# alvgaona/heart-sounds-segmentation

Measured on AMD Instinct MI355X. Metric: PCG windows/sec FSST (1 kHz, 2000-sample), higher is better.
Workload: dtype f32

## Files before the change

### heart_sounds_segmentation_amd/csrc/fsst_canon128.hpp

```cpp
#pragma once
#include "fsst_mfma128.hpp"

namespace hssfsst {

using h8 = _Float16 __attribute__((ext_vector_type(8)));
using u2 = unsigned __attribute__((ext_vector_type(2)));
using u4 = unsigned __attribute__((ext_vector_type(4)));
using lds_u2 = __attribute__((address_space(3))) u2;
using lds_u4 = __attribute__((address_space(3))) u4;

#define HSS_RARE_VMEM_DONE() __builtin_amdgcn_s_waitcnt(0x0f70)
constexpr int kCanonTileFrames = 64;
constexpr int kCanonRecs = 192;
constexpr int kCanonOpFloats = 16 * 64 * 4;
constexpr int kCanonAtabFloats = kCanonOpFloats + 4 * 128;
constexpr int kCanonLdsTabFloats = kCanonAtabFloats + 4 * 33 * 2;
constexpr int kCanonErrMul = 4;
constexpr int kCanonFlagWords = 8;
constexpr int kCanonTieWords = 32;

template <int KLO, int KC>
struct CanonCfg {
    static_assert(KC % 2 == 0 && KC >= 2 && KC <= 24 && KLO >= 0 && KLO + KC <= 32, "even band of <= 24 rows inside rows 0..31");
    static constexpr int NWIN = 128;
// ... 279 lines not shown
            if (mb) db = canon_decide(kB, dnb.y, dnb.x, tile.R2s, tile.eoff());
            const bool la = ma && (da.tie || da.row != kA), lb = mb && (db.tie || db.row != kB);
            if (ma && da.tie) { __hip_atomic_fetch_or(tb + (kA >> 1), 1u << (((kA & 1) << 4) + j), __ATOMIC_RELAXED, __HIP_MEMORY_SCOPE_WORKGROUP); flag[1] = 1; }
            if (mb && db.tie) { __hip_atomic_fetch_or(tb + (kB >> 1), 1u << (((kB & 1) << 4) + j), __ATOMIC_RELAXED, __HIP_MEMORY_SCOPE_WORKGROUP); flag[1] = 1; }
            if constexpr (STA) { if (la) *cellA = f2{0.0f, 0.0f}; }
            if constexpr (STB) { if (lb) *cellB = f2{0.0f, 0.0f}; }
            if (la && !da.tie) { if (canon_put<KLO, KC, s>(row0, kA, da.row, f2{a1.x, a2.x})) defer |= 1u << (2 * s); }
            if (lb && !db.tie) { if (canon_put<KLO, KC, s>(row0, kB, db.row, f2{b1.x, b2.x})) defer |= 1u << (2 * s + 1); }
        }
        if constexpr (s == 3) {
            if (__builtin_expect(visited && __builtin_amdgcn_ballot_w64(defer != 0u) != 0ull, 0)) {
                static_for<3>([&](auto TT) {
                    constexpr int t = decltype(TT)::value;
                    if (__builtin_amdgcn_ballot_w64((defer >> (2 * t)) & 3u) != 0ull) {
                        const f2 QA = zb[NT - 1 - t], QB = za[NT - 1 - t];
                        const f2 c1 = mix_re(za[t], QA), c2 = mix_im(za[t], QA), e1 = mix_re(zb[t], QB), e2 = mix_im(zb[t], QB);
                        const f2 dc = dn_second(c2, dn_first(c1, tiny)), de = dn_second(e2, dn_first(e1, tiny));
                        if ((defer >> (2 * t)) & 1u) {
                            const CanonMove d = canon_decide(rAi + RQ * t, dc.y, dc.x, tile.R2s, tile.eoff());
                            (void)canon_put<KLO, KC, 3>(row0, rAi + RQ * t, d.row, f2{c1.x, c2.x});
                        }
                        if ((defer >> (2 * t + 1)) & 1u) {
                            const CanonMove d = canon_decide(rBi + RQ * t, de.y, de.x, tile.R2s, tile.eoff());
                            (void)canon_put<KLO, KC, 3>(row0, rBi + RQ * t, d.row, f2{e1.x, e2.x});
                        }
                    }
                });
            }
        }
    });
    wave_sync();
    int f_ties = 0;
    if (visited) f_ties = flag[1];
    asm volatile("" : "+v"(f_ties));
    auto signal_sample = [&](int i) -> double {
        const int gi = tg + i - NWIN / 2;
        const float* xs;
        if constexpr (__is_pointer(XSig)) xs = xsig; else xs = xsig();
        return (gi >= 0 && gi < n) ? static_cast<double>(xs[gi]) : 0.0;
    };
    bool exact = false;
    if (__builtin_expect(__builtin_amdgcn_ballot_w64(mx > kExactTheta2 * tile.R2s) == 0ull && tile.R2s > 0.0f, 0)) {
        float e2 = 0.0f;
#pragma unroll
        for (int k = 0; k < 3; ++k) {
            const int i = lane_o + 64 * k;
            const u2 r = xrec[min(i, 142)];
            const float v = static_cast<float>(__builtin_bit_cast(_Float16, static_cast<unsigned short>(r.x & 0xffffu))) +
                            static_cast<float>(__builtin_bit_cast(_Float16, static_cast<unsigned short>(r.y & 0xffffu)));
            e2 = fmaf(i < 143 ? v : 0.0f, v, e2);
        }
        const float R2g = tile.r2s * __int_as_float(__builtin_amdgcn_readfirstlane(__float_as_int(piece_sums(e2, 0.0f, 0.0f, 0.0f))));
        exact = __builtin_amdgcn_ballot_w64(mx > kExactTheta2 * R2g) == 0ull && R2g > 0.0f;
    }
    if (__builtin_expect(exact, 0)) {
        for (int i = lane_o; i < 16 * C::LD; i += 64) own_base[i] = f2{0.0f, 0.0f};
        if (lane_o == 0) flag[1] = 0;
        wave_sync();
        resolve_bitmap<NWIN, true, true, true>(reinterpret_cast<unsigned*>(tq), signal_sample, own_base, C::LD, flag, KLO, KC, own_base, C::LD,
                                               C::COV0, C::COV0 + C::COVN, wtab, tw_lds, 1.0 / static_cast<double>(tile.inv), lane_o);
        wave_sync();
        HSS_RARE_VMEM_DONE();
    } else
    if (__builtin_expect(__builtin_amdgcn_readfirstlane(f_ties) != 0, 0)) {
        resolve_bitmap<NWIN, false, true, true>(reinterpret_cast<unsigned*>(tq), signal_sample, own_base, C::LD, flag, KLO, KC, own_base, C::LD, C::COV0, C::COV0 + C::COVN, wtab, tw_lds, 1.0 / static_cast<double>(tile.inv), lane_o);
        wave_sync();
        HSS_RARE_VMEM_DONE();
    }
}
template <int KLO, int KC>
__device__ __forceinline__ float canon_stats(const f2* own_base, int nvalid, float inv, int lane_o, f2& piv_out)
{
    using C = CanonCfg<KLO, KC>;
    const int g = (lane_o >> 4) & 3, j = lane_o & 15;
    const f2* src = own_base + j * C::LD + C::KOFF + g;
    const f2 pv0 = own_base[C::KOFF], pv1 = own_base[C::KOFF + KC / 2], pv2 = own_base[C::KOFF + KC - 1];
    const f2 piv = f2{pivot_med3(pv0.x, pv1.x, pv2.x), pivot_med3(pv0.y, pv1.y, pv2.y)};
    constexpr int NU = (KC + 3) / 4, UF = KC / 4;
    f2 v[NU];
#pragma unroll
    for (int u = 0; u < NU; ++u) v[u] = src[4 * u];
    f2 st_s = {0.0f, 0.0f}, st_q = {0.0f, 0.0f};
    if (__builtin_expect(nvalid == 16, 1)) {
#pragma unroll
        for (int u = 0; u < NU; ++u) {
            f2 d = v[u] - piv;
            if (u >= UF) { const bool ok = g + 4 * u < KC; d = f2{ok ? d.x : 0.0f, ok ? d.y : 0.0f}; }
            st_s += d; st_q = pk_fma(d, d, st_q);
        }
    } else {
        asm volatile("");
        const bool jv = j < nvalid;
#pragma unroll
        for (int u = 0; u < NU; ++u) {
            f2 d = v[u] - piv;
            const bool ok = jv && (g + 4 * u < KC);
            d = f2{ok ? d.x : 0.0f, ok ? d.y : 0.0f};
            st_s += d; st_q = pk_fma(d, d, st_q);
        }
    }
    float w = piece_sums(st_s.x, st_q.x, st_s.y, st_q.y);
    w *= inv;
    if ((lane_o >> 4) & 1) w *= inv;
    piv_out = piv * f2{inv, inv};
    return w;
}

template <int KLO, int KC, class Sink>
__device__ __forceinline__ void canon_image_to(const f2* own_base, const unsigned* ppk, float inv, int lane_o, Sink sink)
{
    unsigned obase = static_cast<unsigned>(reinterpret_cast<size_t>((lds_float*)reinterpret_cast<const float*>(own_base)));
    asm volatile("" : "+s"(obase));
    const f2 sc = {inv, inv};
    static_for<3>([&](auto I) {
        constexpr int i = decltype(I)::value;
        const unsigned pk = ppk[i * 64 + lane_o];
        const lds_float* q0 = (const lds_float*)static_cast<size_t>(obase + (pk & 0xffffu));
        const lds_float* q1 = (const lds_float*)static_cast<size_t>(obase + (pk >> 16));
        const f2 lo = f2{q0[0], q0[2]} * sc, hi = f2{q1[0], q1[2]} * sc;
        sink(i, f4{lo.x, lo.y, hi.x, hi.y});
    });
}
template <int KLO, int KC>
__device__ __forceinline__ void canon_image(const f2* own_base, const unsigned* ppk, float inv, int lane_o, f4 (&o)[3])
{
    canon_image_to<KLO, KC>(own_base, ppk, inv, lane_o, [&](int i, f4 v) { o[i] = v; });
}

template <int KLO, int KC>
__device__ __forceinline__ unsigned canon_store_offsets(int f)
{
    using C = CanonCfg<KLO, KC>;
    constexpr int Q = KC / 2;
    const int jj = min(f / Q, 15), c = 4 * (f - (f / Q) * Q);
    const int rowb = jj * C::LD + C::KOFF;
    const unsigned p0 = (c < KC) ? (rowb + c) * 8 : (rowb + c - KC) * 8 + 4;
    const unsigned p1 = (c + 2 < KC) ? (rowb + c + 2) * 8 : (rowb + c + 2 - KC) * 8 + 4;
    return p0 | (p1 << 16);
}

struct CanonParams {
    const float* x;
    float* out;
    float* partials;
    const float* atab;
    const double* wtab;
    const double* twtab;
    float r2scale_s;
    float inv_c;
    int n, mode, nsig, col0, ncols;
    long long xstride;
    Core128Regions reg;
    unsigned* status;
    const unsigned* gate;
    unsigned gate_val;
    const RaggedSignal* rsig;
    const int2* rchunk;
    int rnchunks;
};

constexpr int kCanonCtlFloats = 16 + 192;
constexpr int kCanonCtlFusedFloats = kCtlFusedFloats;

__device__ __forceinline__ void canon_fetch(const float* xsig, int n, int t0, int lane_o, float (&sreg)[3])
{
    const __amdgpu_buffer_rsrc_t rs = __builtin_amdgcn_make_buffer_rsrc(const_cast<float*>(xsig), 0, n * 4, 0x00020000);
#pragma unroll
    for (int k = 0; k < 3; ++k)
        sreg[k] = __builtin_bit_cast(float, __builtin_amdgcn_raw_buffer_load_b32(rs, (t0 + lane_o + 64 * k - 64) * 4, 0, 0));
}

template <int KLO, int KC, bool FUSED, bool RAGGED = false>
__global__ __launch_bounds__(64 * 16, 4) void fsst_canon_kernel(CanonParams p)
{
    static_assert(!(RAGGED && FUSED), "ragged lists: the two-launch kernel");
    using C = CanonCfg<KLO, KC>;
    constexpr int WPB = 16, K = KC, GPCF = kCanonTileFrames / 16;
    constexpr int ATAB = kCanonLdsTabFloats;
    constexpr int CTL = FUSED ? kCanonCtlFusedFloats : kCanonCtlFloats;
    extern __shared__ __attribute__((aligned(16))) float smem[];
    if (p.gate != nullptr && *p.gate != p.gate_val) return;
    int n = p.n;
    const int lane = threadIdx.x & 63;
    const int wv = __builtin_amdgcn_readfirstlane(threadIdx.x >> 6);
    float* atab = smem;
    int* next_q = reinterpret_cast<int*>(smem + ATAB);
    unsigned* done_a = reinterpret_cast<unsigned*>(smem + ATAB) + 1;
    unsigned* dead = done_a + 2;
    unsigned* ready = dead + 1;
    float4* fin_stats = reinterpret_cast<float4*>(smem + ATAB + 272);
    unsigned* cls_lds = reinterpret_cast<unsigned*>(smem + ATAB + 16);
    unsigned* ppk_lds = reinterpret_cast<unsigned*>(smem + ATAB + (FUSED ? 80 : 16));
    float* part_lds = smem + ATAB + 288;
    float* wbase = smem + ATAB + CTL + wv * C::wave_floats();
    u2* xrec = reinterpret_cast<u2*>(wbase);
    f2* own_base = reinterpret_cast<f2*>(wbase + 2 * kCanonRecs);
    int* flag = reinterpret_cast<int*>(own_base + 16 * C::LD);
    int* tq = flag + kCanonFlagWords;

    for (int i = threadIdx.x; i < ATAB; i += 64 * WPB) atab[i] = p.atab[i];
    int ncols = p.ncols, cend = p.col0 + p.ncols;
    if (lane < kCanonFlagWords) flag[lane] = 0;
    if (lane < kCanonTieWords) tq[lane] = 0;
    if (threadIdx.x < (FUSED ? 8 : 1)) next_q[threadIdx.x] = 0;
    if (wv == 0) {
        unsigned cls = 0u;
#pragma unroll
        for (int i = 0; i < 3; ++i) {
            const unsigned c = (4u * static_cast<unsigned>(lane + 64 * i)) % static_cast<unsigned>(2 * K);
            cls |= (c >= static_cast<unsigned>(K) ? 1u : 0u) << (2 * i);
            cls |= (c + 2 >= static_cast<unsigned>(K) ? 1u : 0u) << (2 * i + 1);
            ppk_lds[i * 64 + lane] = canon_store_offsets<KLO, KC>(lane + 64 * i);
        }
        if constexpr (FUSED) cls_lds[lane] = cls;
    }
    __syncthreads();

    const int nc0 = p.nsig * p.reg.npc[0];
    const int nc1 = nc0 + p.nsig * p.reg.npc[1];
    const int nchunks = nc1 + p.nsig * p.reg.npc[2];
    int ngroups = (ncols + 15) >> 4;
    const int nk = (FUSED && p.nsig > static_cast<int>(blockIdx.x)) ? (p.nsig - static_cast<int>(blockIdx.x) + static_cast<int>(gridDim.x) - 1) / static_cast<int>(gridDim.x) : 0;
    const int NC = (ngroups + GPCF - 1) / GPCF;
    const int lead = min(8, NC);
    const int nwork = FUSED ? 2 * NC * nk : RAGGED ? p.rnchunks : nchunks;
    auto draw = [&]() -> int {
        int q = 0;
        if (lane == 0) q = __hip_atomic_fetch_add(next_q, 1, __ATOMIC_RELAXED, __HIP_MEMORY_SCOPE_WORKGROUP);
        q = __builtin_amdgcn_readfirstlane(q);
        if constexpr (FUSED) return q < nwork ? q : nwork;
        const long long c = static_cast<long long>(blockIdx.x) + static_cast<long long>(q) * gridDim.x;
        return c < nwork ? static_cast<int>(c) : nwork;
    };
    int chunk = draw();
    f2 tiny = {1.0e-37f, 0.0f};
    asm volatile("" : "+s"(tiny));
    while (chunk < nwork) {
    long long b;
    int grp0, ngrp;
    long long ksig = 0;
    bool zpass = false;
    long long rxo = 0, roo = 0, rpo = 0;
    if constexpr (FUSED) {
        int c;
        if (chunk < NC) {
            ksig = 0; c = chunk;
        } else {
            const int u = chunk - NC;
            const int kk = 1 + u / (2 * NC), v = u - (kk - 1) * (2 * NC);
            if (kk < nk) {
                const int npairs = NC - lead;
                if (v < lead) { ksig = kk; c = v; }
                else if (v - lead < 2 * npairs) {
                    const int w = v - lead;
                    if (w & 1) { ksig = kk; c = lead + (w >> 1); }
                    else { ksig = kk - 1; c = w >> 1; zpass = true; }
                } else { ksig = kk - 1; c = npairs + (v - lead - 2 * npairs); zpass = true; }
            } else { ksig = nk - 1; c = v; zpass = true; }
        }
        b = static_cast<long long>(blockIdx.x) + ksig * gridDim.x;
        grp0 = c * GPCF;
        ngrp = min(GPCF, ngroups - grp0);
    } else if constexpr (RAGGED) {
        const int2 cd = p.rchunk[chunk];
        const RaggedSignal* rs = p.rsig + cd.x;
        rxo = rs->xoff; roo = rs->ooff; rpo = rs->poff;
        n = rs->n; ncols = n; cend = n; ngroups = (n + 15) >> 4;
        b = 0;
        grp0 = cd.y & ((1 << kRaggedGroupBits) - 1);
        ngrp = (cd.y >> kRaggedGroupBits) + 1;
    } else {
        const int rg = (chunk < nc0) ? 0 : (chunk < nc1) ? 1 : 2;
        const int local = chunk - ((rg == 0) ? 0 : (rg == 1) ? nc0 : nc1);
        const int npc = p.reg.npc[rg], gpc = p.reg.gpc[rg];
        b = local / npc;
        const int cidx = local - static_cast<int>(b) * npc;
        grp0 = p.reg.g0[rg] + cidx * gpc;
        ngrp = min(gpc, ngroups - grp0);
    }
    int lane_o = lane;
    asm volatile("" : "+v"(lane_o));
    if (FUSED && zpass) {
        const int sl = static_cast<int>(ksig) & 3;
        const unsigned epoch = static_cast<unsigned>(ksig) + 1u;
        constexpr int CC = 2 * K;
        float4* d4 = reinterpret_cast<float4*>(p.out + (b * static_cast<long long>(ncols) + grp0 * 16) * CC) + lane_o;
        constexpr int per = 8 * K;
        for (unsigned spins = 0;; ++spins) {
            unsigned have = 0;
            if (lane == 0) have = __hip_atomic_load(ready + sl, __ATOMIC_ACQUIRE, __HIP_MEMORY_SCOPE_WORKGROUP);
            if (__builtin_amdgcn_readfirstlane(have) == epoch) break;
            if (spins >= kSpinLimit || __hip_atomic_load(dead, __ATOMIC_RELAXED, __HIP_MEMORY_SCOPE_WORKGROUP)) {
                if (lane == 0) {
                    __hip_atomic_store((gu32*)(p.status), 2u, __ATOMIC_RELAXED, __HIP_MEMORY_SCOPE_SYSTEM);
                    __hip_atomic_store(dead, 1u, __ATOMIC_RELAXED, __HIP_MEMORY_SCOPE_WORKGROUP);
                }
                break;
            }
            __builtin_amdgcn_s_sleep(4);
        }
        __builtin_amdgcn_fence(__ATOMIC_ACQUIRE, "workgroup");
        const float4 st = fin_stats[sl];
        const unsigned cls = cls_lds[lane_o];
        const float4* base0 = reinterpret_cast<const float4*>(p.out + (b * static_cast<long long>(ncols) + grp0 * 16) * CC);
        auto glim = [&](int q) { return (q < ngrp) ? min(16, ncols - (grp0 + q) * 16) * (K >> 1) : 0; };
        {
            f4 o[GPCF][3];
#pragma unroll
            for (int q = 0; q < GPCF; ++q) {
                const int lim = glim(q);
#pragma unroll
                for (int i = 0; i < 3; ++i) {
                    const float4* src = (lane_o + 64 * i < lim) ? (d4 + q * per + 64 * i) : base0;
                    o[q][i] = __builtin_nontemporal_load(reinterpret_cast<const f4*>(src));
                }
            }
            f2 mu[3][2], rs[3][2];
#pragma unroll
            for (int i = 0; i < 3; ++i) {
                const bool im0 = (cls >> (2 * i)) & 1u, im1 = (cls >> (2 * i + 1)) & 1u;
                const float m0 = im0 ? st.z : st.x, r0 = im0 ? st.w : st.y;
                const float m1 = im1 ? st.z : st.x, r1 = im1 ? st.w : st.y;
                mu[i][0] = f2{m0, m0}; rs[i][0] = f2{r0, r0};
                mu[i][1] = f2{m1, m1}; rs[i][1] = f2{r1, r1};
            }
#pragma unroll
            for (int q = 0; q < GPCF; ++q) {
                const int lim = glim(q);
#pragma unroll
                for (int i = 0; i < 3; ++i) {
                    if (lane_o + 64 * i < lim) {
                        const f2 lo = (f2{o[q][i].x, o[q][i].y} - mu[i][0]) * rs[i][0];
                        const f2 hi = (f2{o[q][i].z, o[q][i].w} - mu[i][1]) * rs[i][1];
                        __builtin_nontemporal_store(f4{lo.x, lo.y, hi.x, hi.y}, reinterpret_cast<f4*>(d4 + q * per + 64 * i));
// ... 79 lines not shown
```

### heart_sounds_segmentation_amd/csrc/fsst_half.hpp

```cpp
#pragma once

#include "fsst_kernels.hpp"
#include "fsst_mfma128.hpp"

namespace hssfsst {

template <class OT>
__device__ __forceinline__ void half_store4(OT* dst, float a, float b, float c, float d)
{
    using o2 = OT __attribute__((ext_vector_type(2)));
    using w2 = unsigned __attribute__((ext_vector_type(2)));
    const w2 w = {__builtin_bit_cast(unsigned, __builtin_convertvector(f2{a, b}, o2)), __builtin_bit_cast(unsigned, __builtin_convertvector(f2{c, d}, o2))};
    *reinterpret_cast<w2*>(dst) = w;
}

template <class OT>
__global__ __launch_bounds__(256) void fsst_normalize_to_kernel(const float* in, OT* out, const float4* stats, const float* partials,
                                                                int nblk, int fpp, int n, int K, int nsignals, int slices,
                                                                const unsigned* gate = nullptr, unsigned gate_val = 0u)
{
    static_assert(sizeof(OT) == 2, "2-byte output elements");
    if (gate != nullptr && *gate != gate_val) return;
    __shared__ float4 st_sh;
    const int tid = threadIdx.x;
    const int C = 2 * K;
    const int total = n * C;
    const bool vec = (total & 3) == 0 && (reinterpret_cast<uintptr_t>(out) & 7) == 0;
    for (int unit = blockIdx.x; unit < nsignals * slices; unit += gridDim.x) {
        const int sig = unit / slices, sl = unit - sig * slices;
        float4 st;
        if (partials != nullptr) {
            if (tid < 64) {
                const float4 r = signal_stats(partials + static_cast<long long>(sig) * nblk * kPartFloats, nblk, fpp, n, K, tid);
                if (tid == 0) st_sh = r;
            }
            __syncthreads();
            st = st_sh;
            __syncthreads();
        } else {
            st = stats[sig];
        }
        const float m_re = st.x, i_re = st.y, m_im = st.z, i_im = st.w;
        const float* src = in + static_cast<long long>(sig) * total;
        OT* dst = out + static_cast<long long>(sig) * total;
        if (vec) {
            const float4* s4 = reinterpret_cast<const float4*>(src);
            const int tot4 = total >> 2;
            const int i0 = static_cast<int>(static_cast<long long>(tot4) * sl / slices);
            const int i1 = static_cast<int>(static_cast<long long>(tot4) * (sl + 1) / slices);
            int c = static_cast<int>((static_cast<unsigned>(i0 + tid) * 4u) % static_cast<unsigned>(C));
            const int dc = static_cast<int>(1024u % static_cast<unsigned>(C));
            const bool rowwrap = (C & 3) != 0;
#pragma unroll 4
            for (int i = i0 + tid; i < i1; i += 256) {
                const float4 v = s4[i];
                int c1 = c + 1, c2 = c + 2, c3 = c + 3;
                if (rowwrap) {
                    if (c1 >= C) c1 -= C;
                    if (c2 >= C) c2 -= C;
                    if (c3 >= C) c3 -= C;
                }
                half_store4<OT>(dst + 4ll * i,
                                (c < K) ? (v.x - m_re) * i_re : (v.x - m_im) * i_im,
                                (c1 < K) ? (v.y - m_re) * i_re : (v.y - m_im) * i_im,
                                (c2 < K) ? (v.z - m_re) * i_re : (v.z - m_im) * i_im,
                                (c3 < K) ? (v.w - m_re) * i_re : (v.w - m_im) * i_im);
                c += dc;
                if (c >= C) c -= C;
            }
        } else {
            const int i0 = static_cast<int>(static_cast<long long>(total) * sl / slices);
            const int i1 = static_cast<int>(static_cast<long long>(total) * (sl + 1) / slices);
            for (int i = i0 + tid; i < i1; i += 256) {
                const int c = i % C;
                const float v = src[i];
                dst[i] = static_cast<OT>((c < K) ? (v - m_re) * i_re : (v - m_im) * i_im);
            }
        }
    }
}

template <class OT>
__global__ __launch_bounds__(256) void fsst_ragged_normalize_to_kernel(const float* in, OT* out, const RaggedSignal* sig, const int* unit0,
                                                                       const float4* stats, int nsig, int K)
{
    static_assert(sizeof(OT) == 2, "2-byte output elements");
    const int tid = threadIdx.x;
    const int C = 2 * K;
    const bool vec = (reinterpret_cast<uintptr_t>(out) & 7) == 0;
    const int nunits = unit0[nsig];
    for (int u = blockIdx.x; u < nunits; u += gridDim.x) {
        int lo = 0, hi = nsig;
        while (hi - lo > 1) {
            const int mid = (lo + hi) >> 1;
            if (unit0[mid] <= u) lo = mid; else hi = mid;
        }
        const int s = lo;
        const RaggedSignal rs = sig[s];
        const float4 st = stats[s];
        const float m_re = st.x, i_re = st.y, m_im = st.z, i_im = st.w;
        const int a = static_cast<int>(rs.ooff & 3);
        const float* src = in + (rs.ooff - a);
        OT* dst = out + (rs.ooff - a);
        const int total = rs.n * C;
        const int q = static_cast<int>((static_cast<long long>(a) + total + 3) >> 2);
        const int slices = unit0[s + 1] - unit0[s], sl = u - unit0[s];
        const int i0 = static_cast<int>(static_cast<long long>(q) * sl / slices);
        const int i1 = static_cast<int>(static_cast<long long>(q) * (sl + 1) / slices);
        long long e = 4ll * (i0 + tid) - a;
        int c = static_cast<int>(e % C);
        if (c < 0) c += C;
        const int dc = 1024 % C;
        auto zs = [&](float v, int col) -> float { return (col < K) ? (v - m_re) * i_re : (v - m_im) * i_im; };
        auto wrap = [&](int col) -> int { if (col >= C) col -= C; if (col >= C) col -= C; return col; };
        for (int i = i0 + tid; i < i1; i += 256) {
            if (vec && e >= 0 && e + 4 <= total) {
                const float4 v = reinterpret_cast<const float4*>(src)[i];
                half_store4<OT>(dst + 4ll * i, zs(v.x, c), zs(v.y, wrap(c + 1)), zs(v.z, wrap(c + 2)), zs(v.w, wrap(c + 3)));
            } else {
                for (int k = 0; k < 4; ++k)
                    if (e + k >= 0 && e + k < total) dst[4ll * i + k] = static_cast<OT>(zs(src[4ll * i + k], wrap(c + k)));
            }
            e += 1024;
            c = wrap(c + dc);
        }
    }
}

}
```

### heart_sounds_segmentation_amd/csrc/fsst_kernels.hpp

```cpp
#pragma once
#include <hip/hip_runtime.h>

#include <utility>

namespace hssfsst {

constexpr int kModeRaw = 0, kModeAbs = 1, kModeStack = 2, kModeStackUnnorm = 3;

struct CoreParams {
    const float* x;
    float* out;
    float* partials;
    const float* ctab;
    int n;
    int klo;
    int K;
    int mode;
    int nblk;
    int col0;
    int ncols;
    int oneplane;
    const double* wtab;
    const double* twtab;
    float r2scale;
// ... 246 lines not shown
        const auto r = __builtin_amdgcn_permlane16_swap(v, v, false, false);
        const auto ri = __builtin_amdgcn_permlane16_swap(id, id, false, false);
        return ri[0] == (id ^ 16u) ? r[0] : r[1];
    } else {
        const auto r = __builtin_amdgcn_permlane32_swap(v, v, false, false);
        const auto ri = __builtin_amdgcn_permlane32_swap(id, id, false, false);
        return ri[0] == (id ^ 32u) ? r[0] : r[1];
    }
}
template <int OFF>
__device__ __forceinline__ double xor_lane_f64(double v, int lane)
{
    const long long b = __double_as_longlong(v);
    const unsigned lo = xor_lane_u32<OFF>(static_cast<unsigned>(b & 0xffffffffll), lane);
    const unsigned hi = xor_lane_u32<OFF>(static_cast<unsigned>(static_cast<unsigned long long>(b) >> 32), lane);
    return __longlong_as_double(static_cast<long long>((static_cast<unsigned long long>(hi) << 32) | lo));
}
__device__ __forceinline__ float4 stats_finish_pre(double acc, double it, double it1, int lane)
{
    { const double o = xor_lane_f64<4>(acc, lane);  acc = (lane & 4) ? (o + acc) : (acc + o); }
    { const double o = xor_lane_f64<8>(acc, lane);  acc = (lane & 8) ? (o + acc) : (acc + o); }
    { const double o = xor_lane_f64<16>(acc, lane); acc = (lane & 16) ? (o + acc) : (acc + o); }
    { const double o = xor_lane_f64<32>(acc, lane); acc = (lane & 32) ? (o + acc) : (acc + o); }
    auto from_lane = [&](int l) {
        const long long b = __double_as_longlong(acc);
        const int lo = __builtin_amdgcn_readlane(static_cast<int>(b & 0xffffffffll), l);
        const int hi = __builtin_amdgcn_readlane(static_cast<int>(b >> 32), l);
        return __longlong_as_double((static_cast<long long>(hi) << 32) | static_cast<unsigned>(lo));
    };
    const double sx_re = from_lane(0), sxx_re = from_lane(1), sx_im = from_lane(2), sxx_im = from_lane(3);
    const double mr = sx_re * it, mi = sx_im * it;
    const double vr = fma(-sx_re, mr, sxx_re) * it1, vi = fma(-sx_im, mi, sxx_im) * it1;
    return make_float4(static_cast<float>(mr), 1.0f / sqrtf(static_cast<float>(vr)),
                       static_cast<float>(mi), 1.0f / sqrtf(static_cast<float>(vi)));
}
__device__ __forceinline__ float4 stats_finish_lead(double acc, double it, double it1, int lane)
{
    auto halves = [](double v, unsigned& lo, unsigned& hi) {
        const unsigned long long b = static_cast<unsigned long long>(__double_as_longlong(v));
        lo = static_cast<unsigned>(b); hi = static_cast<unsigned>(b >> 32);
    };
    auto join = [](unsigned lo, unsigned hi) { return __longlong_as_double(static_cast<long long>((static_cast<unsigned long long>(hi) << 32) | lo)); };
    unsigned lo, hi;
    {
        const int from = __builtin_amdgcn_readfirstlane(__builtin_amdgcn_update_dpp(0, lane, 0x124, 0xf, 0xf, false));
        halves(acc, lo, hi);
        unsigned plo, phi;
        if (from == 4) {
            plo = static_cast<unsigned>(__builtin_amdgcn_update_dpp(0, static_cast<int>(lo), 0x124, 0xf, 0xf, false));
            phi = static_cast<unsigned>(__builtin_amdgcn_update_dpp(0, static_cast<int>(hi), 0x124, 0xf, 0xf, false));
        } else {
            plo = static_cast<unsigned>(__builtin_amdgcn_update_dpp(0, static_cast<int>(lo), 0x12c, 0xf, 0xf, false));
            phi = static_cast<unsigned>(__builtin_amdgcn_update_dpp(0, static_cast<int>(hi), 0x12c, 0xf, 0xf, false));
        }
        acc = acc + join(plo, phi);
    }
    {
        halves(acc, lo, hi);
        const unsigned plo = static_cast<unsigned>(__builtin_amdgcn_update_dpp(0, static_cast<int>(lo), 0x128, 0xf, 0xf, false));
        const unsigned phi = static_cast<unsigned>(__builtin_amdgcn_update_dpp(0, static_cast<int>(hi), 0x128, 0xf, 0xf, false));
        acc = acc + join(plo, phi);
    }
    {
        halves(acc, lo, hi);
        const auto rl = __builtin_amdgcn_permlane16_swap(lo, lo, false, false);
        const auto rh = __builtin_amdgcn_permlane16_swap(hi, hi, false, false);
        acc = acc + join(rl[1], rh[1]);
    }
    {
        halves(acc, lo, hi);
        const auto rl = __builtin_amdgcn_permlane32_swap(lo, lo, false, false);
        const auto rh = __builtin_amdgcn_permlane32_swap(hi, hi, false, false);
        acc = acc + join(rl[1], rh[1]);
    }
    auto from_lane = [&](int l) {
        const long long b = __double_as_longlong(acc);
        const int l0 = __builtin_amdgcn_readlane(static_cast<int>(b & 0xffffffffll), l);
        const int h0 = __builtin_amdgcn_readlane(static_cast<int>(b >> 32), l);
        return __longlong_as_double((static_cast<long long>(h0) << 32) | static_cast<unsigned>(l0));
    };
    const double sx_re = from_lane(0), sxx_re = from_lane(1), sx_im = from_lane(2), sxx_im = from_lane(3);
    const double mr = sx_re * it, mi = sx_im * it;
    const double vr = fma(-sx_re, mr, sxx_re) * it1, vi = fma(-sx_im, mi, sxx_im) * it1;
    return make_float4(static_cast<float>(mr), 1.0f / sqrtf(static_cast<float>(vr)),
                       static_cast<float>(mi), 1.0f / sqrtf(static_cast<float>(vi)));
}
__device__ __forceinline__ float4 stats_finish(double acc, double total, int lane)
{
    return stats_finish_pre(acc, 1.0 / total, 1.0 / (total - 1.0), lane);
}
template <class BlockSum>
__device__ __forceinline__ float4 stats_from_blocks(int nblocks, double total, BlockSum block_sum, int lane)
{
    const int q = lane & 3;
    double acc = 0.0;
    for (int blk = lane >> 2; blk < nblocks; blk += 16) acc += block_sum(blk, q);
    return stats_finish(acc, total, lane);
}

template <int STRIDE = kPartFloats>
__device__ __forceinline__ float4 signal_stats(const float* part, int nparts, int fpp, int ncols, int K, int lane)
{
    const int nblocks = (nparts + kStatBlock - 1) / kStatBlock;
    return stats_from_blocks(nblocks, static_cast<double>(K) * static_cast<double>(ncols), [&](int blk, int q) {
        double s = 0.0;
        const int g1 = min(nparts, (blk + 1) * kStatBlock);
        for (int g = blk * kStatBlock; g < g1; ++g) {
            const float* pp = part + static_cast<long long>(g) * STRIDE;
            const double cnt = static_cast<double>(min(fpp, ncols - fpp * g)) * static_cast<double>(K);
            const int h = q >> 1;
            s += piece_moment(q, static_cast<double>(pp[2 * h]), static_cast<double>(pp[2 * h + 1]),
                              static_cast<double>(pp[4 + h]), cnt);
        }
        return s;
    }, lane);
}

__device__ __forceinline__ float piece_sums(float s_re, float q_re, float s_im, float q_im)
{
    const auto r1 = __builtin_amdgcn_permlane32_swap(__float_as_uint(s_re), __float_as_uint(s_im), false, false);
    const float u = __uint_as_float(r1[0]) + __uint_as_float(r1[1]);
    const auto r2 = __builtin_amdgcn_permlane32_swap(__float_as_uint(q_re), __float_as_uint(q_im), false, false);
    const float v = __uint_as_float(r2[0]) + __uint_as_float(r2[1]);
    const auto r3 = __builtin_amdgcn_permlane16_swap(__float_as_uint(u), __float_as_uint(v), false, false);
    float w = __uint_as_float(r3[0]) + __uint_as_float(r3[1]);
    w += __uint_as_float(__builtin_amdgcn_update_dpp(0, __float_as_uint(w), 0x128, 0xf, 0xf, false));
    w += __uint_as_float(__builtin_amdgcn_update_dpp(0, __float_as_uint(w), 0x124, 0xf, 0xf, false));
    w += __uint_as_float(__builtin_amdgcn_update_dpp(0, __float_as_uint(w), 0x122, 0xf, 0xf, false));
    w += __uint_as_float(__builtin_amdgcn_update_dpp(0, __float_as_uint(w), 0x121, 0xf, 0xf, false));
    return w;
}

__device__ __forceinline__ float pivot_med3(float a, float b, float c) { return __builtin_amdgcn_fmed3f(a, b, c); }

__device__ __forceinline__ void store_partial(float* part, float w, float p_re, float p_im)
{
    const int lane = threadIdx.x & 63;
    part[lane >> 4] = w;
    part[4 + (lane & 1)] = (lane & 1) ? p_im : p_re;
}

constexpr float kDcTheta = 0.99f;
struct TileEnergy { float E, S1, C; bool dcdom; };
__device__ __forceinline__ TileEnergy tile_energy(float e2, float s1, float cnt)
{
    const float w = piece_sums(e2, s1, cnt, 0.0f);
    const float E = __int_as_float(__builtin_amdgcn_readlane(__float_as_int(w), 0));
    const float S1 = __int_as_float(__builtin_amdgcn_readlane(__float_as_int(w), 16));
    const float C = __int_as_float(__builtin_amdgcn_readlane(__float_as_int(w), 32));
    return TileEnergy{E, S1, C, E > 0.0f && S1 * S1 >= kDcTheta * C * E};
}

__global__ __launch_bounds__(64) void fsst_stats_kernel(const float* partials, float4* stats, int nparts, int fpp,
                                                        int n, int K, const unsigned* gate = nullptr, unsigned gate_val = 0u)
{
    if (gate != nullptr && *gate != gate_val) return;
    const long long b = blockIdx.x;
    const float4 st = signal_stats(partials + b * nparts * kPartFloats, nparts, fpp, n, K, threadIdx.x & 63);
    if (threadIdx.x == 0) stats[b] = st;
}

template <int R, int TILE>
__global__ __launch_bounds__(TILE, 2) void fsst_core_kernel(CoreParams p)
{
    constexpr int NWIN = 32 * R;
    constexpr int XS = ((TILE + NWIN - 1 + 3) / 4) * 4;
    constexpr int LD = TILE + 1;
    extern __shared__ __attribute__((aligned(16))) float smem[];
    float* xs = smem;
    float* own = smem + XS;

    const int tid = threadIdx.x;
    const int blk = blockIdx.x % p.nblk;
    const long long b = blockIdx.x / p.nblk;
    const int t0 = p.col0 + blk * TILE;
    const int n = p.n;
    const int ncols = p.ncols, tr0 = t0 - p.col0;
    const int K = p.K;
    const float* xsig = p.x + b * p.xstride;

    float e2 = 0.0f, s1 = 0.0f, cnt = 0.0f;
    for (int i = tid; i < TILE + NWIN - 1; i += TILE) {
        const int g = t0 + i - NWIN / 2;
        const bool in = (g >= 0 && g < n);
        const float v = in ? xsig[g] : 0.0f;
        xs[i] = v;
        e2 = fmaf(v, v, e2); s1 += v; cnt += in ? 1.0f : 0.0f;
    }
    static_assert(TILE == 64, "tile_energy reduces one wave");
    const TileEnergy te = tile_energy(e2, s1, cnt);
    const float R2 = p.r2scale * te.E;
    const bool oneplane = p.oneplane != 0;
    float* disp = oneplane ? own : own + 2 * K * LD;
    for (int c = 0; c < 2 * K; ++c) disp[c * LD + tid] = 0.0f;
    __syncthreads();

    const Scatter<LD> sc{own + tid, disp + tid, p.klo, K, oneplane, xs + tid, p.wtab, p.twtab, R2};
    const float* myx = xs + tid;
    ctab_ptr tab = (ctab_ptr)p.ctab;
    packed_class<R, false, LD>(tab, myx, sc);
    if constexpr (R >= 2) packed_class<R, true, LD>(tab + (R / 2) * 32 * 4 * R, myx, sc);
    if constexpr (R >= 4 && R <= 8) {
        static_for<R / 2 - 1>([&](auto RR) {
            constexpr int r = decltype(RR)::value + 1;
            pair_class<R, LD>(tab + r * 32 * 4 * R, r, myx, sc);
        });
    } else if constexpr (R > 8) {
        for (int r = 1; r < R / 2; ++r) pair_class<R, LD>(tab + r * 32 * 4 * R, r, myx, sc);
    }
    __syncthreads();
    if (!oneplane) {
        for (int c = 0; c < 2 * K; ++c) own[c * LD + tid] += disp[c * LD + tid];
    }
    __syncthreads();
    float* acc = own;
    {
        float mxc = 0.0f;
        for (int k = 0; k < K; ++k) { const float re = acc[k * LD + tid], im = acc[(K + k) * LD + tid]; mxc = fmaxf(mxc, fmaf(re, re, im * im)); }
        if ((__builtin_amdgcn_ballot_w64(mxc > 1.0e-4f * R2) == 0ull || te.dcdom) && R2 > 0.0f) {
            for (int c = 0; c < 2 * K; ++c) acc[c * LD + tid] = 0.0f;
            const int klo = p.klo;
            for (int kp = 0; kp <= NWIN / 2; ++kp) {
                double vr = 0.0, vi = 0.0, dr = 0.0, di = 0.0;
#pragma unroll 4
                for (int nn = 0; nn < NWIN; ++nn) {
                    const double x = static_cast<double>(xs[tid + nn]);
                    const double2 wd = reinterpret_cast<const double2*>(p.wtab)[nn];
                    const double2 cs = reinterpret_cast<const double2*>(p.twtab)[(kp * nn) & (NWIN - 1)];
                    const double xw = x * wd.x, xd = x * wd.y;
                    vr = fma(xw, cs.x, vr); vi = fma(-xw, cs.y, vi);
                    dr = fma(xd, cs.x, dr); di = fma(-xd, cs.y, di);
                }
                double shift = (dr * vi - di * vr) / (vr * vr + vi * vi);
                if (!(fabs(shift) <= 1.0e6)) shift = 0.0;
                const double a = static_cast<double>(kp) + shift;
                const double r = (a >= 0.0) ? floor(a + 0.5) : -floor(0.5 - a);
                const int row = static_cast<int>(static_cast<long long>(r)) & (NWIN - 1);
                const double sg = (kp & 1) ? -1.0 : 1.0;
                const float re = static_cast<float>(vr * sg), im = static_cast<float>(vi * sg);
                const int idx = row - klo;
                if (static_cast<unsigned>(idx) < static_cast<unsigned>(K)) { acc[idx * LD + tid] += re; acc[(K + idx) * LD + tid] += im; }
                if (kp != 0 && kp != NWIN / 2) {
                    const int idm = ((NWIN - row) & (NWIN - 1)) - klo;
                    if (static_cast<unsigned>(idm) < static_cast<unsigned>(K)) { acc[idm * LD + tid] += re; acc[(K + idm) * LD + tid] -= im; }
                }
            }
        }
    }

    const int valid = min(TILE, p.col0 + ncols - t0);
    if (p.mode == kModeRaw) {
        if (tid < valid) {
            float2* dst = reinterpret_cast<float2*>(p.out) + (b * K) * static_cast<long long>(ncols) + tr0 + tid;
            for (int k = 0; k < K; ++k)
                dst[static_cast<long long>(k) * ncols] = make_float2(acc[k * LD + tid], acc[(K + k) * LD + tid]);
        }
        return;
    }
    const int C = (p.mode == kModeAbs) ? K : 2 * K;
    float* dst = p.out + (b * static_cast<long long>(ncols) + tr0) * C;
    const int total = valid * C;
    int tt = tid / C, c = tid - tt * C;
    const int dtt = TILE / C, dc = TILE - dtt * C;
    static_assert(TILE == 64, "one wave per tile: the statistics partial is a single-wave reduction");
    const float p_re = pivot_med3(acc[0], acc[(K >> 1) * LD], acc[(K - 1) * LD]);
    const float p_im = pivot_med3(acc[K * LD], acc[(K + (K >> 1)) * LD], acc[(2 * K - 1) * LD]);
    float s_re = 0.0f, q_re = 0.0f, s_im = 0.0f, q_im = 0.0f;
    for (int e = tid; e < total; e += TILE) {
        float val;
        if (p.mode == kModeAbs) {
            const float re = acc[c * LD + tt], im = acc[(K + c) * LD + tt];
            val = sqrtf(fmaf(re, re, im * im));
        } else {
            val = acc[c * LD + tt];
            if (c < K) { const float d = val - p_re; s_re += d; q_re = fmaf(d, d, q_re); }
            else       { const float d = val - p_im; s_im += d; q_im = fmaf(d, d, q_im); }
        }
        dst[e] = val;
        c += dc; tt += dtt;
        if (c >= C) { c -= C; ++tt; }
    }
    if (p.mode != kModeStack) return;
    const float w = piece_sums(s_re, q_re, s_im, q_im);
    store_partial(p.partials + (b * p.nblk + blk) * kPartFloats, w, p_re, p_im);
}

__global__ __launch_bounds__(256) void fsst_normalize_kernel(float* out, const float4* stats, const float* partials,
                                                             int nblk, int fpp, int n, int K, int nsignals, int slices,
                                                             const unsigned* gate = nullptr, unsigned gate_val = 0u)
{
    if (gate != nullptr && *gate != gate_val) return;
    __shared__ float4 st_sh;
    const int tid = threadIdx.x;
    const int C = 2 * K;
    const int total = n * C;
    for (int unit = blockIdx.x; unit < nsignals * slices; unit += gridDim.x) {
        const int sig = unit / slices, sl = unit - sig * slices;
        float4 st;
        if (partials != nullptr) {
            if (tid < 64) {
                const float4 r = signal_stats(partials + static_cast<long long>(sig) * nblk * kPartFloats, nblk, fpp, n, K, tid);
                if (tid == 0) st_sh = r;
            }
            __syncthreads();
            st = st_sh;
            __syncthreads();
        } else {
            st = stats[sig];
        }
        const float m_re = st.x, i_re = st.y, m_im = st.z, i_im = st.w;
        float* base = out + static_cast<long long>(sig) * total;
        if ((total & 3) == 0) {
            float4* b4 = reinterpret_cast<float4*>(base);
            const int tot4 = total >> 2;
            const int i0 = static_cast<int>(static_cast<long long>(tot4) * sl / slices);
            const int i1 = static_cast<int>(static_cast<long long>(tot4) * (sl + 1) / slices);
            int c = static_cast<int>((static_cast<unsigned>(i0 + tid) * 4u) % static_cast<unsigned>(C));
            const int dc = static_cast<int>(1024u % static_cast<unsigned>(C));
            const bool rowwrap = (C & 3) != 0;
#pragma unroll 4
            for (int i = i0 + tid; i < i1; i += 256) {
                float4 v = b4[i];
                int c1 = c + 1, c2 = c + 2, c3 = c + 3;
                if (rowwrap) {
                    if (c1 >= C) c1 -= C;
                    if (c2 >= C) c2 -= C;
                    if (c3 >= C) c3 -= C;
                }
                v.x = (c < K) ? (v.x - m_re) * i_re : (v.x - m_im) * i_im;
                v.y = (c1 < K) ? (v.y - m_re) * i_re : (v.y - m_im) * i_im;
                v.z = (c2 < K) ? (v.z - m_re) * i_re : (v.z - m_im) * i_im;
                v.w = (c3 < K) ? (v.w - m_re) * i_re : (v.w - m_im) * i_im;
                b4[i] = v;
                c += dc;
                if (c >= C) c -= C;
            }
        } else {
            const int i0 = static_cast<int>(static_cast<long long>(total) * sl / slices);
            const int i1 = static_cast<int>(static_cast<long long>(total) * (sl + 1) / slices);
            for (int i = i0 + tid; i < i1; i += 256) {
                const int c = i % C;
                const float v = base[i];
                base[i] = (c < K) ? (v - m_re) * i_re : (v - m_im) * i_im;
            }
        }
    }
}

constexpr int kMomThreads = 1024;
constexpr int kMomPieceFrames = 16;
struct PlainLoad4 { __device__ float4 operator()(const float4* q) const { return *q; } };
struct AgentLoad4 {
    __device__ float4 operator()(const float4* q) const
    {
        const unsigned long long* u = reinterpret_cast<const unsigned long long*>(q);
        const unsigned long long a = __hip_atomic_load(u, __ATOMIC_RELAXED, __HIP_MEMORY_SCOPE_AGENT);
        const unsigned long long b = __hip_atomic_load(u + 1, __ATOMIC_RELAXED, __HIP_MEMORY_SCOPE_AGENT);
        return make_float4(__uint_as_float(static_cast<unsigned>(a)), __uint_as_float(static_cast<unsigned>(a >> 32)),
                           __uint_as_float(static_cast<unsigned>(b)), __uint_as_float(static_cast<unsigned>(b >> 32)));
    }
};
__device__ __forceinline__ void mom_acc(double (&a)[4], float f, bool imag)
{
    const double v = static_cast<double>(f);
    if (imag) { a[2] += v; a[3] = fma(v, v, a[3]); } else { a[0] += v; a[1] = fma(v, v, a[1]); }
}
__device__ __forceinline__ void mom_acc4(double (&a)[4], float4 v, int f, int C, int K)
{
    int c = static_cast<int>((4u * static_cast<unsigned>(f)) % static_cast<unsigned>(C));
    int c1 = c + 1, c2 = c + 2, c3 = c + 3;
    if (c1 >= C) c1 -= C;
    if (c2 >= C) c2 -= C;
    if (c3 >= C) c3 -= C;
    mom_acc(a, v.x, c >= K); mom_acc(a, v.y, c1 >= K); mom_acc(a, v.z, c2 >= K); mom_acc(a, v.w, c3 >= K);
}
__device__ inline void piece_moments(const float* pb, int L, int C, int K, int lane, double (&t)[4])
{
    double a[4] = {0.0, 0.0, 0.0, 0.0};
    const bool wide = (reinterpret_cast<uintptr_t>(pb) & 15) == 0;
    for (int f = lane; 4 * f < L; f += 64) {
        if (wide && 4 * f + 3 < L) mom_acc4(a, *reinterpret_cast<const float4*>(pb + 4 * f), f, C, K);
        else
            for (int u = 0; u < 4; ++u) {
                const int e = 4 * f + u;
                if (e < L) mom_acc(a, pb[e], (e % C) >= K);
            }
    }
#pragma unroll
    for (int e = 0; e < 4; ++e) t[e] = wave_sum(a[e]);
}
template <class Piece>
__device__ inline void moments_from_pieces(int npieces, int lane, Piece piece, double (&out)[4])
{
    double a[4] = {0.0, 0.0, 0.0, 0.0};
    for (int q = lane; q < npieces; q += 64)
#pragma unroll
        for (int e = 0; e < 4; ++e) a[e] += piece(q, e);
#pragma unroll
    for (int e = 0; e < 4; ++e) out[e] = wave_sum(a[e]);
}
__device__ inline void chunk_moments(const float* base, int n, int C, int K, int tid, double (*sh)[4], double out[4])
{
    const int lane = tid & 63, w = tid >> 6;
    const int npieces = (n + kMomPieceFrames - 1) / kMomPieceFrames;
    double a[4] = {0.0, 0.0, 0.0, 0.0};
    for (int q = w; q < npieces; q += kMomThreads / 64) {
        double t[4];
        piece_moments(base + static_cast<long long>(q) * kMomPieceFrames * C, min(kMomPieceFrames, n - q * kMomPieceFrames) * C, C, K, lane, t);
        if (lane == (q & 63))
#pragma unroll
            for (int e = 0; e < 4; ++e) a[e] += t[e];
    }
    if ((lane & 15) == w)
#pragma unroll
        for (int e = 0; e < 4; ++e) sh[lane][e] = a[e];
    __syncthreads();
#pragma unroll
    for (int e = 0; e < 4; ++e) out[e] = wave_sum(sh[lane][e]);
}

__device__ inline float2 merge_state(double* st, double s, double q, double nb)
{
    const double mean_b = s / nb;
    const double m2_b = q - s * mean_b;
    const double na = st[0], mean_a = st[1], m2_a = st[2];
    const double nn = na + nb;
    const double delta = mean_b - mean_a;
    const double mean_n = mean_a + delta * (nb / nn);
    const double m2_n = m2_a + m2_b + delta * delta * (na * nb / nn);
    st[0] = nn; st[1] = mean_n; st[2] = m2_n;
    return make_float2(static_cast<float>(mean_n), 1.0f / static_cast<float>(sqrt(m2_n / (nn - 1.0))));
}

__global__ __launch_bounds__(kMomThreads) void fsst_moments_merge_kernel(const float* feats, double* state, int n, int K)
{
    __shared__ double sh[64][4];
    const long long b = blockIdx.x;
    const int tid = threadIdx.x;
    const int total = n * 2 * K;
    double m[4];
    chunk_moments(feats + b * static_cast<long long>(total), n, 2 * K, K, tid, sh, m);
    if (tid < 2) merge_state(state + b * 6 + tid * 3, m[2 * tid], m[2 * tid + 1], static_cast<double>(K) * static_cast<double>(n));
}

// ... 112 lines not shown
```

### heart_sounds_segmentation_amd/csrc/fsst_team16.hpp

```cpp
#pragma once
#include "fsst_mfma128.hpp"
#include "fsst_canon128.hpp"

namespace hssfsst {

using gu64 = __attribute__((address_space(1))) unsigned long long;

constexpr int kT16PartFloats = 6;
constexpr int kT16BlockWords = 8;
constexpr int kT16MaxBlocks = kFusedMaxGroups / kStatBlock;
constexpr int kT16SlotWords = kT16MaxBlocks * kT16BlockWords;
constexpr int kT16MaxCpc = 8;
constexpr int kT16MaxSlots = 64;
constexpr int kT16StatFloats = 12;
constexpr int t16_ctl_base(int slots) { return 16 + 64 + 192 + 2 * slots + kT16StatFloats * slots; }
constexpr int t16_ctl_floats(int pslots, int slots) { return t16_ctl_base(slots) + pslots * (kT16MaxCpc * kT16PartFloats + 2); }
template <int KLO, int KC>
constexpr int t16_room() { return 160 * 1024 / 4 - kCanonLdsTabFloats - 16 * CanonCfg<KLO, KC>::wave_floats(); }
template <int KLO, int KC>
constexpr int t16_slots() { return t16_room<KLO, KC>() >= t16_ctl_floats(16, kT16MaxSlots) ? kT16MaxSlots : kT16MaxSlots / 2; }
template <int KLO, int KC>
constexpr int t16_pslots()
{
    constexpr int room = t16_room<KLO, KC>(), sl = t16_slots<KLO, KC>();
    return room >= t16_ctl_floats(32, sl) ? 32 : room >= t16_ctl_floats(16, sl) ? 16 : 0;
}

struct Team16Params {
    const float* x;
    float* out;
    const float* atab;
    const double* wtab;
    const double* twtab;
    unsigned long long* mail;
    unsigned* status;
    float r2scale_s;
    float inv_c;
    int n, nsig, col0, ncols;
    long long xstride;
    int team;
    int cpc_shift;
    int slots;
    unsigned seq;
    unsigned spin_ticks;
    unsigned* arrive;
    unsigned arrive_base;
    unsigned* abort_word;
    unsigned* fallbacks;
    unsigned launch;
    unsigned* done;
    unsigned done_base;
    unsigned* host_done;
    double inv_total, inv_total1;
};


constexpr int kT16HeldBase = 104;
#define HSS_T16_PAIRS(X) X(0, 104, 105) X(1, 106, 107) X(2, 108, 109) X(3, 110, 111) X(4, 112, 113) X(5, 114, 115) \
                         X(6, 116, 117) X(7, 118, 119) X(8, 120, 121) X(9, 122, 123) X(10, 124, 125) X(11, 126, 127)
template <int P>
__device__ __forceinline__ void held_put(f2 a, f2 b)
{
#define HSS_T16_PUT(N, LO, HI) if constexpr (P == N) asm volatile("v_pk_mul_f32 v[" #LO ":" #HI "], %0, %1" :: "v"(a), "v"(b) : "v" #LO, "v" #HI);
    HSS_T16_PAIRS(HSS_T16_PUT)
#undef HSS_T16_PUT
}
template <int P>
__device__ __forceinline__ f2 held_zscore(f2 m)
{
    f2 d, e;
#define HSS_T16_ZS(N, LO, HI) if constexpr (P == N) asm volatile("v_pk_add_f32 %0, v[" #LO ":" #HI "], %1 op_sel:[0,0] op_sel_hi:[1,0] neg_lo:[0,1] neg_hi:[0,1]" : "=v"(d) : "v"(m));
    HSS_T16_PAIRS(HSS_T16_ZS)
#undef HSS_T16_ZS
    asm("v_pk_mul_f32 %0, %1, %2 op_sel:[0,1] op_sel_hi:[1,1]" : "=v"(e) : "v"(d), "v"(m));
    return e;
}

template <class OT>
__device__ __forceinline__ void team16_store4(char* dst, f2 lo, f2 hi)
{
    static_assert(sizeof(OT) == 2, "2-byte output elements");
    using o2 = OT __attribute__((ext_vector_type(2)));
    using w2 = unsigned __attribute__((ext_vector_type(2)));
    const w2 w = {__builtin_bit_cast(unsigned, __builtin_convertvector(lo, o2)), __builtin_bit_cast(unsigned, __builtin_convertvector(hi, o2))};
    __builtin_nontemporal_store(w, reinterpret_cast<w2*>(dst));
}

template <int KLO, int KC, int WPB, int DEPTH, class OT = float>
__global__ __launch_bounds__(64 * WPB, WPB / 4) __attribute__((amdgpu_num_vgpr(52))) void fsst_team16_kernel(Team16Params p)
{
    constexpr int OB = static_cast<int>(sizeof(OT));
    using C = CanonCfg<KLO, KC>;
    static_assert(WPB % 4 == 0 && DEPTH >= 1 && DEPTH <= 2, "whole waves per SIMD; two held groups (v104 .. v127)");
    static_assert(DEPTH == 2, "the kernel is compiled for 104 allocatable registers + 24 fixed ones");
    constexpr int K = KC, ATAB = kCanonLdsTabFloats;
    extern __shared__ __attribute__((aligned(16))) float smem[];
    const int n = p.n;
    const int lane = threadIdx.x & 63;
    const int wv = __builtin_amdgcn_readfirstlane(threadIdx.x >> 6);
    float* atab = smem;
    int* next_q = reinterpret_cast<int*>(smem + ATAB);
    unsigned* dead = reinterpret_cast<unsigned*>(smem + ATAB) + 1;
    unsigned* cls_lds = reinterpret_cast<unsigned*>(smem + ATAB + 16);
    unsigned* ppk_lds = reinterpret_cast<unsigned*>(smem + ATAB + 80);
    unsigned* ready = reinterpret_cast<unsigned*>(smem + ATAB + 272);
    constexpr int MS = t16_slots<KLO, KC>(), PSLOTS = t16_pslots<KLO, KC>();
    unsigned* claim = ready + MS;
    float4* fin = reinterpret_cast<float4*>(smem + ATAB + 272 + 2 * MS);
    static_assert(PSLOTS >= 16, "the CU's own partials need LDS beside the wave regions");
    float* part_lds = smem + ATAB + t16_ctl_base(MS);
    int* pcnt_lds = reinterpret_cast<int*>(part_lds + PSLOTS * kT16MaxCpc * kT16PartFloats);
    float* wbase = smem + ATAB + t16_ctl_floats(PSLOTS, MS) + wv * C::wave_floats();
    u2* xrec = reinterpret_cast<u2*>(wbase);
    f2* own_base = reinterpret_cast<f2*>(wbase + 2 * kCanonRecs);
    int* flag = reinterpret_cast<int*>(own_base + 16 * C::LD);
    int* tq = flag + kCanonFlagWords;

    unsigned arrived = 0u;
    if (threadIdx.x == 64) arrived = __hip_atomic_fetch_add(p.arrive, 1u, __ATOMIC_RELAXED, __HIP_MEMORY_SCOPE_AGENT) - p.arrive_base;
    for (int i = threadIdx.x; i < ATAB; i += 64 * WPB) atab[i] = p.atab[i];
    if (lane < kCanonFlagWords) flag[lane] = 0;
    if (lane < kCanonTieWords) tq[lane] = 0;
    if (threadIdx.x < 16 && threadIdx.x != 2) next_q[threadIdx.x] = 0;
    for (int i = threadIdx.x; i < 2 * MS; i += 64 * WPB) ready[i] = 0u;
    if (threadIdx.x < 2 * PSLOTS) pcnt_lds[threadIdx.x] = 0;
    if (threadIdx.x == 64) next_q[2] = static_cast<int>(arrived);
    if (wv == 0) {
        unsigned cofs = 0u;
#pragma unroll
        for (int i = 0; i < 3; ++i) {
            const unsigned c = (4u * static_cast<unsigned>(lane + 64 * i)) % static_cast<unsigned>(2 * K);
            const unsigned nim = (c >= static_cast<unsigned>(K) ? 1u : 0u) + (c + 2 >= static_cast<unsigned>(K) ? 1u : 0u);
            cofs |= (16u * nim) << (8 * i);
            ppk_lds[i * 64 + lane] = canon_store_offsets<KLO, KC>(lane + 64 * i);
        }
        cls_lds[lane] = cofs;
    }
    __syncthreads();

    using kparams = const __attribute__((address_space(4))) Team16Params;
    kparams* const kp_ = (kparams*)__builtin_amdgcn_kernarg_segment_ptr();
    auto P = [&]() -> kparams* { kparams* q = kp_; asm volatile("" : "+s"(q)); return q; };

    auto aborted = [&]() -> bool {
        return __hip_atomic_load(P()->abort_word, __ATOMIC_RELAXED, __HIP_MEMORY_SCOPE_AGENT) == P()->launch;
    };
    auto gave_up = [&]() {
        if (lane == 0) {
            __hip_atomic_store(P()->abort_word, P()->launch, __ATOMIC_RELAXED, __HIP_MEMORY_SCOPE_AGENT);
            __hip_atomic_store((gu32*)(P()->fallbacks), P()->launch, __ATOMIC_RELAXED, __HIP_MEMORY_SCOPE_SYSTEM);
            __hip_atomic_store(dead, 1u, __ATOMIC_RELAXED, __HIP_MEMORY_SCOPE_WORKGROUP);
        }
    };
    auto is_dead = [&]() -> bool { return __hip_atomic_load(dead, __ATOMIC_RELAXED, __HIP_MEMORY_SCOPE_WORKGROUP) != 0u; };
    auto leave = [&]() { asm volatile("s_endpgm" ::: "memory"); };
    auto expired = [&](unsigned since) -> bool {
        return static_cast<unsigned>(wall_clock64()) - since > P()->spin_ticks || is_dead() || aborted();
    };

    const int virt = __builtin_amdgcn_readfirstlane(next_q[2]);
    if (static_cast<unsigned>(virt) >= gridDim.x) { gave_up(); return; }
    const unsigned abort_seen = __hip_atomic_load(P()->abort_word, __ATOMIC_RELAXED, __HIP_MEMORY_SCOPE_AGENT);
    const int T = p.team, cpcs = p.cpc_shift, cpc = 1 << cpcs;
    const int member = virt & (T - 1), team = virt / T;
    const int nteams = static_cast<int>(gridDim.x) / T;
    const int nk = (p.nsig > team) ? (p.nsig - team + nteams - 1) / nteams : 0;
    const int nwork = nk << cpcs;
    const int ncols = p.ncols, cend = p.col0 + p.ncols;
    const int G = (ncols + 15) >> 4;
    const int cg0 = p.col0 >> 4;
    const int smask = p.slots - 1;
    constexpr int nwords = kT16SlotWords;
    gu64* mail = (gu64*)(p.mail) + static_cast<size_t>(team) * static_cast<size_t>(p.slots) * nwords;
    const int nblocks = (G + kStatBlock - 1) / kStatBlock;
    const unsigned sig_bytes = static_cast<unsigned>(ncols) * (2 * K * OB);

    f2 tiny = {1.0e-37f, 0.0f};
    asm volatile("" : "+s"(tiny));

    float sreg[3];
    bool d_valid = false, saw_dead = false;
    int ko_d = 0, g_d = 0, q_last = -1;
    int ask_qi = 0x7fffffff;
    unsigned ask_dd = 0u;
    auto draw_ask = [&](int after_ko) {
        ask_qi = 0x7fffffff;
        ask_dd = 0u;
        const bool known = after_ko < 0 || ((q_last + 1) >> cpcs) > after_ko;
        if (lane == 0) {
            const bool go = known || (__hip_atomic_load(next_q, __ATOMIC_RELAXED, __HIP_MEMORY_SCOPE_WORKGROUP) >> cpcs) > after_ko;
            if (go) ask_qi = __hip_atomic_fetch_add(next_q, 1, __ATOMIC_RELAXED, __HIP_MEMORY_SCOPE_WORKGROUP);
            ask_dd = __hip_atomic_load(dead, __ATOMIC_RELAXED, __HIP_MEMORY_SCOPE_WORKGROUP);
        }
    };
    auto draw_take = [&]() {
        int qi = __builtin_amdgcn_readfirstlane(ask_qi);
        const unsigned dd = ask_dd;
        saw_dead = __builtin_amdgcn_readfirstlane(dd) != 0u;
        d_valid = false;
        while (qi < nwork) {
            q_last = qi;
            ko_d = qi >> cpcs;
            g_d = (((member + ko_d) & (T - 1)) << cpcs) + (qi & (cpc - 1));
            if (g_d < G) { d_valid = true; break; }
            if (lane == 0) qi = __hip_atomic_fetch_add(next_q, 1, __ATOMIC_RELAXED, __HIP_MEMORY_SCOPE_WORKGROUP);
            qi = __builtin_amdgcn_readfirstlane(qi);
        }
        if (d_valid) {
            int lane_o = lane;
            asm volatile("" : "+v"(lane_o));
            const float* xsig = P()->x + static_cast<unsigned long long>(static_cast<unsigned>(team + ko_d * nteams)) * static_cast<unsigned>(P()->xstride);
            canon_fetch(xsig, n, ((g_d + cg0) & ~3) * 16, lane_o, sreg);
        }
    };
    auto draw = [&](int after_ko) { draw_ask(after_ko); draw_take(); };

    auto stats_ready = [&](int ko) -> bool {
        unsigned have = 0u;
        if (lane == 0) have = __hip_atomic_load(ready + (ko & smask), __ATOMIC_ACQUIRE, __HIP_MEMORY_SCOPE_WORKGROUP);
        return static_cast<unsigned>(__builtin_amdgcn_readfirstlane(have)) == static_cast<unsigned>(ko) + 1u;
    };
    auto try_claim = [&](int ko) -> bool {
        unsigned mine = 0u;
        const unsigned epoch = static_cast<unsigned>(ko) + 1u;
        if (lane == 0) mine = __hip_atomic_fetch_max(claim + (ko & smask), epoch, __ATOMIC_RELAXED, __HIP_MEMORY_SCOPE_WORKGROUP) < epoch ? 1u : 0u;
        return __builtin_amdgcn_readfirstlane(mine) != 0u;
    };

    auto blocks_to_stats = [&](int ko, unsigned t0, int lane_r) __attribute__((always_inline)) -> float4 {
        const unsigned tag = (P()->seq << 16) | (static_cast<unsigned>(ko) & 0xffffu);
        const gu64* slot = mail + static_cast<size_t>(ko & smask) * nwords;
        const int blk0 = lane_r >> 2;
        unsigned need = (blk0 < nblocks ? 1u : 0u) | (blk0 + 16 < nblocks ? 2u : 0u);
        double sb[2] = {0.0, 0.0};
        for (unsigned polls = 0;; ++polls) {
#pragma unroll
            for (int rb = 0; rb < 2; ++rb)
                if ((need >> rb) & 1u) {
                    const gu64* q = slot + 2 * (lane_r + 64 * rb);
                    const unsigned long long hi = __hip_atomic_load(q, __ATOMIC_RELAXED, __HIP_MEMORY_SCOPE_AGENT);
                    const unsigned long long lo = __hip_atomic_load(q + 1, __ATOMIC_RELAXED, __HIP_MEMORY_SCOPE_AGENT);
                    if (static_cast<unsigned>(hi >> 32) == tag && static_cast<unsigned>(lo >> 32) == tag) {
                        sb[rb] = __longlong_as_double(static_cast<long long>((hi << 32) | (lo & 0xffffffffull)));
                        need &= ~(1u << rb);
                    }
                }
            if (__builtin_amdgcn_ballot_w64(need != 0u) == 0ull) break;
            if ((polls & 7u) == 7u && expired(t0)) { gave_up(); leave(); }
            __builtin_amdgcn_s_sleep(8);
        }
        double acc = 0.0;
        if (blk0 < nblocks) acc += sb[0];
        if (blk0 + 16 < nblocks) acc += sb[1];
        static_assert(kT16MaxBlocks <= 32, "a lane sums at most two blocks");
        return stats_finish_lead(acc, P()->inv_total, P()->inv_total1, lane_r);
    };
    auto resolve_owned = [&](int ko, unsigned t0, int lane_r) __attribute__((always_inline)) {
        __builtin_amdgcn_s_setprio(3);
        float4 r;
        r = blocks_to_stats(ko, t0, lane_r);
        if (lane == 0) {
            float4* f3 = fin + 3 * (ko & smask);
            f3[0] = make_float4(r.x, r.y, r.x, r.y);
            f3[1] = make_float4(r.x, r.y, r.z, r.w);
            f3[2] = make_float4(r.z, r.w, r.z, r.w);
            __hip_atomic_store(ready + (ko & smask), static_cast<unsigned>(ko) + 1u, __ATOMIC_RELEASE, __HIP_MEMORY_SCOPE_WORKGROUP);
        }
        wave_sync();
        __builtin_amdgcn_s_setprio(0);
    };
    auto signal_statistics = [&](int ko) {
        if (stats_ready(ko)) return;
        int lane_r = lane;
        asm volatile("" : "+v"(lane_r));
        const unsigned t0 = static_cast<unsigned>(wall_clock64());
        for (unsigned spins = 0;; ++spins) {
            if ((spins & 15u) == 0u && try_claim(ko)) {
                resolve_owned(ko, t0, lane_r); return;
            }
            if ((spins & 31u) == 31u && expired(t0)) { gave_up(); leave(); }
            if (is_dead()) leave();
            __builtin_amdgcn_s_sleep(4);
            if (stats_ready(ko)) return;
        }
    };

    auto emit_held = [&](auto SL, int ko_h, int g_h) {
        constexpr int sl = decltype(SL)::value;
        int lane_r = lane;
        asm volatile("" : "+v"(lane_r));
        __builtin_amdgcn_fence(__ATOMIC_ACQUIRE, "workgroup");
        const unsigned cofs = cls_lds[lane_r];
        const char* tb = reinterpret_cast<const char*>(fin + 3 * (ko_h & smask));
        char* obase = reinterpret_cast<char*>(P()->out) + static_cast<unsigned long long>(static_cast<unsigned>(team + ko_h * nteams)) * sig_bytes +
                      static_cast<unsigned>(g_h * (16 * 2 * K * OB));
        const unsigned voff = static_cast<unsigned>(lane_r) * (4u * OB);
        const int nvalid = min(16, ncols - g_h * 16);
        auto put = [&](auto I) {
            constexpr int i = decltype(I)::value;
            const float4 tt = *reinterpret_cast<const float4*>(tb + ((cofs >> (8 * i)) & 0xffu));
            const f2 lo = held_zscore<6 * sl + 2 * i>(f2{tt.x, tt.y});
            const f2 hi = held_zscore<6 * sl + 2 * i + 1>(f2{tt.z, tt.w});
            if constexpr (OB == 4) __builtin_nontemporal_store(f4{lo.x, lo.y, hi.x, hi.y}, reinterpret_cast<f4*>(obase + (voff + 1024u * static_cast<unsigned>(i))));
            else team16_store4<OT>(obase + (voff + (256u * OB) * static_cast<unsigned>(i)), lo, hi);
        };
        if (__builtin_expect(nvalid == 16, 1)) {
            static_for<3>([&](auto I) {
                constexpr int i = decltype(I)::value;
                if constexpr (64 * (i + 1) <= 8 * K) put(I);
                else if constexpr (64 * i < 8 * K) { if (lane_r + 64 * i < 8 * K) put(I); }
            });
        } else {
            asm volatile("");
            const int lim = nvalid * (K >> 1);
            static_for<3>([&](auto I) { if (lane_r + 64 * decltype(I)::value < lim) put(I); });
        }
    };

// ... 29 lines not shown
        {
            const int lag = (d_valid ? ko_d : ko + 2) - ko;
            if (lag >= 2) __builtin_amdgcn_s_setprio(2); else if (lag == 1) __builtin_amdgcn_s_setprio(1); else __builtin_amdgcn_s_setprio(0);
        }
        canon_group<KLO, KC, 2, true>(xrec + ((g + cg0) & 3) * 16, atab, own_base, flag, tq, P()->wtab, P()->twtab, tile, tiny, lane_o,
                                           [&]() -> const float* { return P()->x + static_cast<unsigned long long>(b) * static_cast<unsigned>(P()->xstride); }, n, tg, P()->atab + kCanonAtabFloats);
        const float inv_cur = tile.inv;
        const int ko_cur = ko, g_cur = g;
        c_valid = false;
        HSS_RARE_VMEM_DONE();
        if (d_valid) land();
        {
            const int nvalid = min(16, cend - tg);
            f2 piv;
            const float w = canon_stats<KLO, KC>(own_base, nvalid, inv_cur, lane_o, piv);
            const int pos = g_cur & (cpc - 1);
            const int ps = ko_cur & (PSLOTS - 1);
            float* pe = part_lds + (ps * kT16MaxCpc + pos) * kT16PartFloats;
            const unsigned pa = static_cast<unsigned>(reinterpret_cast<size_t>((lds_float*)pe)) + (static_cast<unsigned>(lane_o) >> 4) * 4u;
            const unsigned pcnt_a = static_cast<unsigned>(reinterpret_cast<size_t>((__attribute__((address_space(3))) int*)(pcnt_lds + 2 * ps + (pos >> 2))));
            int before = 0;
            const bool known = ((q_last + 1) >> cpcs) > ko_cur;
            if (__builtin_expect(known, 1)) {
                const unsigned nq_a = static_cast<unsigned>(reinterpret_cast<size_t>((__attribute__((address_space(3))) int*)next_q));
                unsigned one = 1u, before_v, qi_v, dd_v;
                unsigned long long keep;
                asm volatile("s_mov_b64 %0, exec\n\ts_mov_b32 exec_lo, 0x00010001\n\ts_mov_b32 exec_hi, 0x00010001\n\tds_write_b32 %4, %5\n\t"
                             "s_mov_b64 exec, 1\n\tds_write_b64 %4, %6 offset:16\n\t"
                             "ds_add_rtn_u32 %1, %7, %9\n\tds_add_rtn_u32 %2, %8, %9\n\tds_read_b32 %3, %8 offset:4\n\t"
                             "s_mov_b64 exec, %0\n\ts_waitcnt lgkmcnt(0)"
                             : "=&s"(keep), "=&v"(before_v), "=&v"(qi_v), "=&v"(dd_v)
                             : "v"(pa), "v"(w), "v"(piv), "v"(pcnt_a), "v"(nq_a), "v"(one) : "memory");
                before = static_cast<int>(before_v);
                ask_qi = static_cast<int>(qi_v);
                ask_dd = dd_v;
                wave_sync();
            } else {
                unsigned long long keep;
                asm volatile("s_mov_b64 %0, exec\n\ts_mov_b32 exec_lo, 0x00010001\n\ts_mov_b32 exec_hi, 0x00010001\n\tds_write_b32 %1, %2\n\t"
                             "s_mov_b64 exec, 1\n\tds_write_b64 %1, %3 offset:16\n\ts_mov_b64 exec, %0"
                             : "=&s"(keep) : "v"(pa), "v"(w), "v"(piv) : "memory");
                wave_sync();
                if (lane == 0) before = __hip_atomic_fetch_add(pcnt_lds + 2 * ps + (pos >> 2), 1, __ATOMIC_RELAXED, __HIP_MEMORY_SCOPE_WORKGROUP);
                draw_ask(ko_cur);
            }
            const int blk = g_cur >> 2, bfirst = blk << 2;
            const int expect = min(kStatBlock, G - bfirst);
            if (__builtin_amdgcn_readfirstlane(before) + 1 == expect) {
                __builtin_amdgcn_s_setprio(3);
                if (lane == 0) __hip_atomic_store(pcnt_lds + 2 * ps + (pos >> 2), 0, __ATOMIC_RELAXED, __HIP_MEMORY_SCOPE_WORKGROUP);
                wave_sync();
                int lane_b = lane;
                asm volatile("" : "+v"(lane_b));
                const int q = lane_b & 3, h = q >> 1, pc = (lane_b >> 2) & 3;
                const float* pb = part_lds + (ps * kT16MaxCpc + (pos & ~3) + pc) * kT16PartFloats;
                const double cnt = static_cast<double>(min(16, ncols - 16 * (bfirst + pc))) * static_cast<double>(K);
                const double mom = piece_moment(q, static_cast<double>(pb[2 * h]), static_cast<double>(pb[2 * h + 1]), static_cast<double>(pb[4 + h]), cnt);
                auto from_row = [&](int ctrl) -> double {
                    const long long b = __double_as_longlong(mom);
                    unsigned lo, hi;
                    if (ctrl == 4) { lo = __builtin_amdgcn_update_dpp(0u, static_cast<unsigned>(b), 0x104, 0xf, 0xf, true); hi = __builtin_amdgcn_update_dpp(0u, static_cast<unsigned>(b >> 32), 0x104, 0xf, 0xf, true); }
                    else if (ctrl == 8) { lo = __builtin_amdgcn_update_dpp(0u, static_cast<unsigned>(b), 0x108, 0xf, 0xf, true); hi = __builtin_amdgcn_update_dpp(0u, static_cast<unsigned>(b >> 32), 0x108, 0xf, 0xf, true); }
                    else { lo = __builtin_amdgcn_update_dpp(0u, static_cast<unsigned>(b), 0x10c, 0xf, 0xf, true); hi = __builtin_amdgcn_update_dpp(0u, static_cast<unsigned>(b >> 32), 0x10c, 0xf, 0xf, true); }
                    return __longlong_as_double(static_cast<long long>((static_cast<unsigned long long>(hi) << 32) | lo));
                };
                double sbk = 0.0;
                sbk += mom;
                if (expect > 1) sbk += from_row(4);
                if (expect > 2) sbk += from_row(8);
                if (expect > 3) sbk += from_row(12);
                const unsigned tag = (P()->seq << 16) | (static_cast<unsigned>(ko_cur) & 0xffffu);
                const unsigned long long bits = static_cast<unsigned long long>(__double_as_longlong(sbk));
                gu64* e = mail + static_cast<size_t>(ko_cur & smask) * nwords + (blk * 4 + q) * 2;
                if (lane_b < 4) {
                    __hip_atomic_store(e, (static_cast<unsigned long long>(tag) << 32) | (bits >> 32), __ATOMIC_RELAXED, __HIP_MEMORY_SCOPE_AGENT);
                    __hip_atomic_store(e + 1, (static_cast<unsigned long long>(tag) << 32) | (bits & 0xffffffffull), __ATOMIC_RELAXED, __HIP_MEMORY_SCOPE_AGENT);
                }
                __builtin_amdgcn_s_setprio(0);
            }
        }
        draw_take();
        auto move_in = [&](const f2* src_plane, float inv_src, int ko_src, int g_src) {
            int ko_o = 0, g_o = 0;
            static_for<DEPTH>([&](auto S) { if (slot == decltype(S)::value) { ko_o = ko_hs[decltype(S)::value]; g_o = g_hs[decltype(S)::value]; } });
            const bool full = nheld == DEPTH;
            int lane_r = lane;
            asm volatile("" : "+v"(lane_r));
            const unsigned cofs = cls_lds[lane_r];
            const unsigned pk0 = ppk_lds[lane_r], pk1 = ppk_lds[64 + lane_r], pk2 = ppk_lds[128 + lane_r];
            const unsigned have = __hip_atomic_load(ready + (ko_o & smask), __ATOMIC_RELAXED, __HIP_MEMORY_SCOPE_WORKGROUP);
            if (full) {
                if (static_cast<unsigned>(__builtin_amdgcn_readfirstlane(static_cast<int>(have))) != static_cast<unsigned>(ko_o) + 1u) signal_statistics(ko_o);
            } else ++nheld;
            __builtin_amdgcn_fence(__ATOMIC_ACQUIRE, "workgroup");
            unsigned obase = static_cast<unsigned>(reinterpret_cast<size_t>((lds_float*)reinterpret_cast<const float*>(src_plane)));
            asm volatile("" : "+s"(obase));
            auto cell = [&](unsigned off) -> f2 {
                const lds_float* q = (const lds_float*)static_cast<size_t>(obase + off);
                return f2{q[0], q[2]};
            };
            const f2 lo0 = cell(pk0 & 0xffffu), hi0 = cell(pk0 >> 16), lo1 = cell(pk1 & 0xffffu), hi1 = cell(pk1 >> 16),
                     lo2 = cell(pk2 & 0xffffu), hi2 = cell(pk2 >> 16);
            const f2 sc = {inv_src, inv_src};
            static_for<DEPTH>([&](auto S) {
                constexpr int sl = decltype(S)::value;
                if (slot == sl) {
                    if (full) {
                        const char* tb = reinterpret_cast<const char*>(fin + 3 * (ko_o & smask));
                        const float4 t0 = *reinterpret_cast<const float4*>(tb + (cofs & 0xffu));
                        const float4 t1 = *reinterpret_cast<const float4*>(tb + ((cofs >> 8) & 0xffu));
                        const float4 t2 = *reinterpret_cast<const float4*>(tb + ((cofs >> 16) & 0xffu));
                        char* ob = reinterpret_cast<char*>(P()->out) + static_cast<unsigned long long>(static_cast<unsigned>(team + ko_o * nteams)) * sig_bytes +
                                   static_cast<unsigned>(g_o * (16 * 2 * K * OB));
                        const unsigned voff = static_cast<unsigned>(lane_r) * (4u * OB);
                        const int nvalid = min(16, ncols - g_o * 16);
                        auto put = [&](auto I, float4 tt) {
                            constexpr int i = decltype(I)::value;
                            const f2 l = held_zscore<6 * sl + 2 * i>(f2{tt.x, tt.y});
                            const f2 h = held_zscore<6 * sl + 2 * i + 1>(f2{tt.z, tt.w});
                            if constexpr (OB == 4) __builtin_nontemporal_store(f4{l.x, l.y, h.x, h.y}, reinterpret_cast<f4*>(ob + (voff + 1024u * static_cast<unsigned>(i))));
                            else team16_store4<OT>(ob + (voff + (256u * OB) * static_cast<unsigned>(i)), l, h);
                        };
                        const float4 tts[3] = {t0, t1, t2};
                        if (__builtin_expect(nvalid == 16, 1)) {
                            static_for<3>([&](auto I) {
                                constexpr int i = decltype(I)::value;
                                if constexpr (64 * (i + 1) <= 8 * K) put(I, tts[i]);
                                else if constexpr (64 * i < 8 * K) { if (lane_r + 64 * i < 8 * K) put(I, tts[i]); }
                            });
                        } else {
                            asm volatile("");
                            const int lim = nvalid * (K >> 1);
                            static_for<3>([&](auto I) { if (lane_r + 64 * decltype(I)::value < lim) put(I, tts[decltype(I)::value]); });
                        }
                    }
                    held_put<6 * sl + 0>(lo0, sc); held_put<6 * sl + 1>(hi0, sc);
                    held_put<6 * sl + 2>(lo1, sc); held_put<6 * sl + 3>(hi1, sc);
                    held_put<6 * sl + 4>(lo2, sc); held_put<6 * sl + 5>(hi2, sc);
                    ko_hs[sl] = ko_src; g_hs[sl] = g_src;
                }
            });
            slot = (slot + 1 == DEPTH) ? 0 : slot + 1;
        };
        move_in(own_base, inv_cur, ko_cur, g_cur);
        wave_sync();
    }
    for (int i = 0; i < nheld; ++i) {
        const int so = (slot + DEPTH - nheld + i) % DEPTH;
        static_for<DEPTH>([&](auto S) {
            constexpr int sl = decltype(S)::value;
            if (so == sl) { signal_statistics(ko_hs[sl]); emit_held(S, ko_hs[sl], g_hs[sl]); }
        });
    }
    if (P()->host_done != nullptr) {
        __builtin_amdgcn_fence(__ATOMIC_RELEASE, "workgroup");
        unsigned last = 0u;
        if (lane == 0) last = __hip_atomic_fetch_add(next_q + 3, 1, __ATOMIC_RELAXED, __HIP_MEMORY_SCOPE_WORKGROUP) == WPB - 1 ? 1u : 0u;
        if (__builtin_amdgcn_readfirstlane(last) != 0u) {
            __builtin_amdgcn_fence(__ATOMIC_ACQUIRE, "workgroup");
            __builtin_amdgcn_fence(__ATOMIC_RELEASE, "");
            if (lane == 0) {
                const unsigned before = __hip_atomic_fetch_add(P()->done, 1u, __ATOMIC_RELAXED, __HIP_MEMORY_SCOPE_AGENT) - P()->done_base;
                if (before + 1u == gridDim.x) {
                    __builtin_amdgcn_fence(__ATOMIC_SEQ_CST, "");
                    __hip_atomic_store((gu32*)(P()->host_done), P()->launch, __ATOMIC_RELAXED, __HIP_MEMORY_SCOPE_SYSTEM);
                }
            }
        }
    }
}

}
```

### heart_sounds_segmentation_amd/csrc/hssfsst.hip

```cpp
#include "../../include/hssfsst.h"

#include <hip/hip_runtime.h>

#include <algorithm>
#include <cmath>
#include <cstdarg>
#include <cstdio>
#include <cstring>
#include <chrono>
#include <mutex>
#include <dlfcn.h>
#include <cstdlib>
#include <array>
#include <atomic>
#include <memory>
#include <new>
#include <thread>
#include <vector>
#include <type_traits>

#include "fsst_kernels.hpp"
#include "fsst_mfma128.hpp"
#include "fsst_canon128.hpp"
#include "fsst_team16.hpp"
// ... 94 lines not shown
    if (device < 0 || device >= ndev) return fail(HSSFSST_EINVAL, "%s: device %d out of range [0,%d)", what, device, ndev);
    return 0;
}

int spline_knot_slopes(const double* w, int n, double* s)
{
    if (n < 1) return HSSFSST_EINVAL;
    if (n == 1) { s[0] = 0.0; return 0; }
    if (n == 2) { s[0] = s[1] = w[1] - w[0]; return 0; }
    if (n == 3) {
        const double d0 = w[1] - w[0], d1 = w[2] - w[1];
        s[0] = d0 - 0.5 * (d1 - d0); s[1] = 0.5 * (d0 + d1); s[2] = d1 + 0.5 * (d1 - d0);
        return 0;
    }
    std::vector<double> dl(n, 0.0), d(n, 0.0), du(n, 0.0), du2(n, 0.0), b(n, 0.0);
    d[0] = 1.0; du[0] = 2.0; b[0] = (5.0 * (w[1] - w[0]) + (w[2] - w[1])) / 2.0;
    for (int i = 1; i < n - 1; ++i) {
        dl[i] = 1.0; d[i] = 4.0; du[i] = 1.0; b[i] = 3.0 * (w[i + 1] - w[i - 1]);
    }
    dl[n - 1] = 2.0; d[n - 1] = 1.0;
    b[n - 1] = (5.0 * (w[n - 1] - w[n - 2]) + (w[n - 2] - w[n - 3])) / 2.0;
    for (int i = 0; i < n - 1; ++i) {
        if (std::fabs(d[i]) >= std::fabs(dl[i + 1])) {
            if (d[i] == 0.0) return HSSFSST_EINVAL;
            const double f = dl[i + 1] / d[i];
            d[i + 1] -= f * du[i];
            if (i + 2 < n) du[i + 1] -= f * du2[i];
            b[i + 1] -= f * b[i];
        } else {
            const double f = d[i] / dl[i + 1];
            const double di = dl[i + 1], dui = d[i + 1], du2i = (i + 2 < n) ? du[i + 1] : 0.0;
            const double bi = b[i + 1];
            d[i + 1] = du[i] - f * dui;
            if (i + 2 < n) du[i + 1] = du2[i] - f * du2i;
            b[i + 1] = b[i] - f * bi;
            d[i] = di; du[i] = dui; du2[i] = du2i; b[i] = bi;
        }
    }
    if (d[n - 1] == 0.0) return HSSFSST_EINVAL;
    s[n - 1] = b[n - 1] / d[n - 1];
    s[n - 2] = (b[n - 2] - du[n - 2] * s[n - 1]) / d[n - 2];
    for (int i = n - 3; i >= 0; --i) s[i] = (b[i] - du[i] * s[i + 1] - du2[i] * s[i + 2]) / d[i];
    return 0;
}

void band_rows(int nwin, double fs, double f_lo, double f_hi, int* klo, int* K)
{
    const int nf = nwin / 2 + 1;
    const double res = fs / static_cast<double>(nwin);
    int first = -1, cnt = 0;
    for (int k = 0; k < nf; ++k) {
        double fk = res * k;
        if ((nwin % 2) == 0 && k == nwin / 2) fk = fs / 2.0;
        const float f32 = static_cast<float>(fk);
        if (f32 >= static_cast<float>(f_lo) && f32 <= static_cast<float>(f_hi)) {
            if (first < 0) first = k;
            ++cnt;
        }
    }
    *klo = first < 0 ? 0 : first;
    *K = cnt;
}

constexpr int kTile = 64;
constexpr int kFpw128 = 64;

template <class T>
struct DevBuf {
    T* p = nullptr;
    size_t cap = 0;
    DevBuf() = default;
    DevBuf(const DevBuf&) = delete;
    DevBuf& operator=(const DevBuf&) = delete;
    ~DevBuf() { if (p) (void)hipFree(p); }
    T* get() const { return p; }
    int grow(size_t need)
    {
        if (need <= cap) return 0;
        if (p) { HIP_TRY(hipFree(p)); p = nullptr; cap = 0; }
        void* v = nullptr;
        const hipError_t e = hipMalloc(&v, need * sizeof(T));
        if (e != hipSuccess) return fail(HSSFSST_ENOMEM, "hipMalloc(%zu B): %s", need * sizeof(T), hipGetErrorString(e));
        p = static_cast<T*>(v);
        cap = need;
        return 0;
    }
    int upload(const T* host, size_t n)
    {
        if (int rc = grow(n)) return rc;
        HIP_TRY(hipMemcpy(p, host, n * sizeof(T), hipMemcpyHostToDevice));
        return 0;
    }
};

template <class T>
struct PinnedBuf {
    T* h = nullptr;
    T* d = nullptr;
    size_t cap = 0;
    bool mapped = true;
    PinnedBuf() = default;
    explicit PinnedBuf(bool mapped_) : mapped(mapped_) {}
    PinnedBuf(const PinnedBuf&) = delete;
    PinnedBuf& operator=(const PinnedBuf&) = delete;
    ~PinnedBuf() { if (h) (void)hipHostFree(h); }
    int grow(size_t need, size_t es)
    {
        if (need <= cap) return 0;
        if (h) { HIP_TRY(hipHostFree(h)); h = nullptr; d = nullptr; cap = 0; }
        size_t c = need + need / 2;
        if (mapped) for (c = size_t(1) << 12; c < need; c *= 2) {}
        void* hp = nullptr;
        HIP_TRY(hipHostMalloc(&hp, c * es, mapped ? hipHostMallocMapped : hipHostMallocDefault));
        void* dp = nullptr;
        const hipError_t e = mapped ? hipHostGetDevicePointer(&dp, hp, 0) : hipSuccess;
        if (e != hipSuccess) {
            (void)hipHostFree(hp);
            return fail(HSSFSST_EHIP, "hipHostGetDevicePointer: %s", hipGetErrorString(e));
        }
        h = static_cast<T*>(hp); d = static_cast<T*>(dp); cap = c;
        return 0;
    }
};

constexpr size_t kPinPoolMax = 64;

}

struct hssfsst_plan {
    int device = -1;
    int nwin = 0, R = 0, nf = 0, klo = 0, K = 0, mode = 0;
    int out_dtype = HSSFSST_DTYPE_F32;
    size_t out_es = sizeof(float);
    DevBuf<float> d_f32;
    double fs = 0.0;
    DevBuf<float> d_ctab;
    DevBuf<float> d_dtab;
    int dft = 0;
    float r2scale = 0.0f;
    DevBuf<double> d_wtab;
    DevBuf<float> d_atab;
    int rq = 0;
    DevBuf<float> d_atab16;
    float canon_inv_c = 0.0f;
    float canon_r2s = 0.0f;
    int canon_slots = 0;
    int nt = 16;
    DevBuf<float> d_partials;
    unsigned* d_status = nullptr;
    volatile unsigned* h_status = nullptr;
    DevBuf<unsigned long long> d_mail;
    unsigned team_seq = 0;
    DevBuf<unsigned> d_arrive; unsigned arrive_total = 0;
    unsigned done_total = 0;
    unsigned team_launch = 0;
    volatile unsigned* h_fallback = nullptr; unsigned* d_fallback = nullptr;
    unsigned seen_fallback = 0; int fallbacks = 0;
    int giveups_in_a_row = 0, team_pause = 0;
    int team16_cus = 0;
    char last_kernel[112] = "";
    int last_fused = 0;
    int zpath_pref = 0;
    int last_zpath = 0;
    int core128_slots = 0;
    int ragged_slots = 0;
    int stream_slots = 0;
    DevBuf<unsigned> d_stream_arrive;
    DevBuf<double> d_stream_pieces;
    int fused_slots = 0;
    DevBuf<float> d_stats;
    DevBuf<float> d_xstage, d_ostage;
    PinnedBuf<float> xpin, opin;
    struct PoolBuf { PinnedBuf<float> buf; bool used = false; };
    std::array<PoolBuf, kPinPoolMax> pin_pool;
    std::mutex pin_mu;
    DevBuf<long long> d_starts;
    DevBuf<float> d_frames;
    DevBuf<unsigned char> d_rtab;
    PinnedBuf<unsigned char> h_rtab{false};
    size_t rtab_bytes = 0;
    std::vector<long long> rkey;
    size_t rtab_unit = 0, rtab_chunk = 0;
    long long rtab_nchunks = 0, rtab_nunits = 0;
    hipEvent_t rtab_ev = nullptr;
    int timing_every = 0;
    unsigned timing_seq = 0;
    std::vector<hipEvent_t> ev;
    size_t ev_used = 0;
    std::vector<int> ev_chunks;
};

namespace {

constexpr int kMaxLdsBytes = 160 * 1024;
template <class Kern>
int allow_full_lds(Kern kern, int device, std::atomic<unsigned long long>& done)
{
    const unsigned long long bit = 1ull << (device & 63);
    if (done.load(std::memory_order_acquire) & bit) return 0;
    HIP_TRY(hipFuncSetAttribute(reinterpret_cast<const void*>(kern), hipFuncAttributeMaxDynamicSharedMemorySize, kMaxLdsBytes));
    done.fetch_or(bit, std::memory_order_release);
    return 0;
}

template <class Kern>
int resident_blocks(const hssfsst_plan* pl, int& cache, Kern kern, int threads, size_t lds, bool whole_cus)
{
    if (cache != 0) return 0;
    int per_cu = 0, cus = 0;
    HIP_TRY(hipOccupancyMaxActiveBlocksPerMultiprocessor(&per_cu, reinterpret_cast<const void*>(kern), threads, lds));
    HIP_TRY(hipDeviceGetAttribute(&cus, hipDeviceAttributeMultiprocessorCount, pl->device));
    cache = whole_cus ? ((per_cu >= 1 && cus >= 1) ? cus : -1) : std::max(per_cu, 1) * std::max(cus, 1);
    return 0;
}

struct ExecCtx {
    hipStream_t st = nullptr;
    int zpref = HSSFSST_ZPATH_AUTO;
    bool host_waits = false;
    bool want_done_word = false;
    const unsigned* gate = nullptr; unsigned gate_val = 0;
    unsigned team_launch = 0;
    unsigned flagged_launch = 0;
    bool fused = false;
    int zpath = 0;
    char kernel[sizeof(hssfsst_plan::last_kernel)] = "";
    bool timing = false;
    bool timing_closed = false;
};

void name_kernel(char (&name)[sizeof(hssfsst_plan::last_kernel)], int waves, long long grid, const char* fmt, ...)
{
    va_list ap;
    va_start(ap, fmt);
    const int k = vsnprintf(name, sizeof(name), fmt, ap);
    va_end(ap);
    if (k > 0 && static_cast<size_t>(k) < sizeof(name))
        snprintf(name + k, sizeof(name) - static_cast<size_t>(k), " [%d waves/block, grid %lld]", waves, grid);
}

void exec_report(hssfsst_plan* p, const ExecCtx& cx)
{
    std::memcpy(p->last_kernel, cx.kernel, sizeof(p->last_kernel));
    p->last_fused = (cx.fused || cx.team_launch != 0u) ? 1 : 0;
    p->last_zpath = cx.zpath;
}

int out_floats_per_sample(const hssfsst_plan* p) { return p->mode == HSSFSST_MODE_ABS ? p->K : 2 * p->K; }

template <int R>
int launch_core(hssfsst_plan* pl, ExecCtx& cx, hssfsst::CoreParams cp, long long nblocks)
{
    constexpr int NWIN = 32 * R;
    constexpr int XS = ((kTile + NWIN - 1 + 3) / 4) * 4;
    size_t lds = (static_cast<size_t>(XS) + static_cast<size_t>(4 * pl->K) * (kTile + 1)) * sizeof(float);
    cp.oneplane = 0;
    if (lds > 40 * 1024) {
        lds = (static_cast<size_t>(XS) + static_cast<size_t>(2 * pl->K) * (kTile + 1)) * sizeof(float);
        cp.oneplane = 1;
    }
    if (lds > 160 * 1024) return fail(HSSFSST_EUNSUPPORTED, "LDS request %zu B exceeds 160 KiB", lds);
    auto kern = hssfsst::fsst_core_kernel<R, kTile>;
    static std::atomic<unsigned long long> lds_ok{0};
    if (int rc = allow_full_lds(kern, pl->device, lds_ok)) return rc;
    name_kernel(cx.kernel, 1, nblocks, "fsst_core_kernel<%d, %d>", R, kTile);
    hipLaunchKernelGGL(kern, dim3(static_cast<unsigned>(nblocks)), dim3(kTile), lds, cx.st, cp);
    HIP_TRY(hipGetLastError());
    return 0;
}

inline size_t core128_lds_bytes(const hssfsst_plan* pl, int rq, int nt, int wpb, bool pair)
{
    const size_t regions = pair ? wpb / 2 : wpb;
    return (hssfsst::core128_atab_floats(rq, nt) + hssfsst::kCtlFloats + regions *
            (static_cast<size_t>(hssfsst::wave_lds_floats(kFpw128, pl->klo, pl->K, rq, nt)) + (pair ? hssfsst::kPairFloats : 0))) * sizeof(float);
}

int ensure_status(hssfsst_plan* pl);
template <int NT, int RQ, bool FAST, int WPB, int S1C = -1, bool PAIR = false, bool RAGGED = false>
int launch_core128_wpb(hssfsst_plan* pl, ExecCtx& cx, const hssfsst::Core128Params& cp, int64_t nchunks)
{
    size_t lds = core128_lds_bytes(pl, RQ, NT, WPB, PAIR);
    auto kern = hssfsst::fsst_core128_kernel<NT, RQ, kFpw128, FAST, WPB, S1C, false, false, PAIR, RAGGED>;
    static std::atomic<unsigned long long> lds_ok{0};
    if (int rc = allow_full_lds(kern, pl->device, lds_ok)) return rc;
    int& slots = RAGGED ? pl->ragged_slots : pl->core128_slots;
    if (int rc = resident_blocks(pl, slots, kern, 64 * WPB, lds, false)) return rc;
    int64_t blocks = nchunks;
    if (blocks > slots) blocks = slots;
    name_kernel(cx.kernel, WPB, blocks, "fsst_core128_kernel<%d, %d, %d, %s, %d, %d, false%s%s>", NT, RQ, kFpw128, FAST ? "true" : "false", WPB, S1C,
                PAIR ? ", pairs" : "", RAGGED ? ", ragged" : "");
    if constexpr (PAIR) {
        if (int rcs = ensure_status(pl)) return rcs;
        hssfsst::Core128Params cq = cp;
        cq.status = pl->d_status;
        hipLaunchKernelGGL(kern, dim3(static_cast<unsigned>(blocks)), dim3(64 * WPB), lds, cx.st, cq);
    } else
    hipLaunchKernelGGL(kern, dim3(static_cast<unsigned>(blocks)), dim3(64 * WPB), lds, cx.st, cp);
    HIP_TRY(hipGetLastError());
    return 0;
}

template <int NT, int RQ, int WPB, bool PAIR>
int launch_stream(hssfsst_plan* pl, float* tape_at, long long tape_len, const float* x_new_dev, long long x_stride, int channels, int chunk,
                  float* out, double* state, float* mirror, hipStream_t st)
{
    const int ngroups = (chunk + 15) / 16;
    const hssfsst::Core128Regions reg = hssfsst::core128_regions(ngroups, channels);
    if (!(reg.npc[0] == 0 && reg.npc[1] == 0 && reg.gpc[2] == 1)) return 0;
    const size_t lds = core128_lds_bytes(pl, RQ, NT, WPB, PAIR);
    if (lds > kMaxLdsBytes) return 0;
    auto kern = hssfsst::fsst_core128_kernel<NT, RQ, kFpw128, true, WPB, -1, false, true, PAIR>;
    static std::atomic<unsigned long long> lds_ok{0};
    if (int rc = allow_full_lds(kern, pl->device, lds_ok)) return rc;
    if (int rc = resident_blocks(pl, pl->stream_slots, kern, 64 * WPB, lds, false)) return rc;
    if (state && pl->d_stream_arrive.cap < static_cast<size_t>(channels)) {
        if (int rc = pl->d_stream_arrive.grow(static_cast<size_t>(channels))) return rc;
        HIP_TRY(hipMemsetAsync(pl->d_stream_arrive.get(), 0, static_cast<size_t>(channels) * sizeof(unsigned), st));
    }
    if (state) {
        if (int rc = pl->d_stream_pieces.grow(static_cast<size_t>(channels) * ngroups * 4)) return rc;
    }
    if (int rcs = ensure_status(pl)) return rcs;
    int bpc = pl->stream_slots / channels;
    if (bpc > ngroups) bpc = ngroups;
    if (bpc < 1) bpc = 1;
    hssfsst::Core128Params cp{};
    cp.x = tape_at; cp.xstride = tape_len; cp.out = out; cp.partials = nullptr; cp.atab = pl->d_atab.get();
    cp.wtab = pl->d_wtab.get(); cp.twtab = pl->d_wtab.get() + 2 * pl->nwin; cp.r2scale = pl->r2scale;
    cp.n = pl->nwin - 1 + chunk; cp.klo = pl->klo; cp.K = pl->K; cp.mode = pl->mode; cp.nsig = channels;
    cp.col0 = pl->nwin / 2; cp.ncols = chunk; cp.reg = reg;
    cp.xnew = x_new_dev; cp.xnew_stride = x_stride; cp.hist = pl->nwin - 1; cp.bpc = bpc; cp.state = state; cp.arrive = pl->d_stream_arrive.get(); cp.pieces = pl->d_stream_pieces.get(); cp.mirror = mirror;
    const long long grid = static_cast<long long>(channels) * bpc;
    cp.status = pl->d_status;
    name_kernel(pl->last_kernel, WPB, grid, "fsst_core128_kernel<%d, %d, %d, true, %d, -1, false, stream%s>", NT, RQ, kFpw128, WPB, PAIR ? ", pairs" : "");
    hipLaunchKernelGGL(kern, dim3(static_cast<unsigned>(grid)), dim3(64 * WPB), lds, st, cp);
    HIP_TRY(hipGetLastError());
    return 1;
}

template <int S1C>
int launch_fused128(hssfsst_plan* pl, ExecCtx& cx, hssfsst::Core128Params cp, int64_t batch, int ngroups)
{
    constexpr int WPB = 16;
    if (ngroups > hssfsst::kFusedMaxGroups || (ngroups + kFpw128 / 16 - 1) / (kFpw128 / 16) < hssfsst::kFusedMinChunks) return 0;
    const size_t lds = (hssfsst::core128_atab_floats(8, 16) + hssfsst::kCtlFusedFloats + static_cast<size_t>(WPB) *
                        hssfsst::wave_lds_floats(kFpw128, pl->klo, pl->K, 8, 16)) * sizeof(float);
    if (lds > static_cast<size_t>(kMaxLdsBytes)) return 0;
    auto kern = hssfsst::fsst_core128_kernel<16, 8, kFpw128, true, WPB, S1C, true>;
    static std::atomic<unsigned long long> lds_ok{0};
    if (int rc = allow_full_lds(kern, pl->device, lds_ok)) return rc;
    if (int rc = resident_blocks(pl, pl->fused_slots, kern, 64 * WPB, lds, true)) return rc;
    if (pl->fused_slots < 1) return 0;
    const int64_t grid = pl->fused_slots;
    const int64_t rounds = (batch + grid - 1) / grid;
    if (batch < grid || rounds * grid * 100 > batch * 112) return 0;
    if (int rcs = ensure_status(pl)) return rcs;
    cp.status = pl->d_status;
    name_kernel(cx.kernel, WPB, grid, "fsst_core128_kernel<16, 8, %d, true, %d, %d, true>", kFpw128, WPB, S1C);
    hipLaunchKernelGGL(kern, dim3(static_cast<unsigned>(grid)), dim3(64 * WPB), lds, cx.st, cp);
    HIP_TRY(hipGetLastError());
    return 1;
}

template <int NT, int RQ, int WPB, int S1C>
int launch_fused_general(hssfsst_plan* pl, ExecCtx& cx, hssfsst::Core128Params cp, int64_t batch, int ngroups)
{
    if (ngroups > hssfsst::kFusedMaxGroups || (ngroups + kFpw128 / 16 - 1) / (kFpw128 / 16) < hssfsst::kFusedMinChunks) return 0;
    if (((static_cast<long long>(cp.ncols) * 2 * pl->K) & 3) != 0 || (reinterpret_cast<uintptr_t>(cp.out) & 15) != 0) return 0;
    const size_t lds = (hssfsst::core128_atab_floats(RQ, NT) + hssfsst::kCtlFloats + static_cast<size_t>(WPB) *
                        hssfsst::wave_lds_floats(kFpw128, pl->klo, pl->K, RQ, NT)) * sizeof(float);
    if (lds > static_cast<size_t>(kMaxLdsBytes)) return 0;
    auto kern = hssfsst::fsst_core128_kernel<NT, RQ, kFpw128, false, WPB, S1C, true>;
    static std::atomic<unsigned long long> lds_ok{0};
    if (int rc = allow_full_lds(kern, pl->device, lds_ok)) return rc;
    if (int rc = resident_blocks(pl, pl->fused_slots, kern, 64 * WPB, lds, true)) return rc;
    if (pl->fused_slots < 1) return 0;
    const int64_t grid = pl->fused_slots;
    const int64_t rounds = (batch + grid - 1) / grid;
    if (batch < grid || rounds * grid * 100 > batch * 112) return 0;
    if (int rcs = ensure_status(pl)) return rcs;
    cp.status = pl->d_status;
    name_kernel(cx.kernel, WPB, grid, "fsst_core128_kernel<%d, %d, %d, false, %d, %d, true>", NT, RQ, kFpw128, WPB, S1C);
    hipLaunchKernelGGL(kern, dim3(static_cast<unsigned>(grid)), dim3(64 * WPB), lds, cx.st, cp);
    HIP_TRY(hipGetLastError());
    return 1;
}

int ensure_status(hssfsst_plan* pl)
{
    if (pl->d_status) return 0;
    void* h = nullptr;
    HIP_TRY(hipHostMalloc(&h, sizeof(unsigned), hipHostMallocMapped));
    *static_cast<volatile unsigned*>(h) = 0u;
    void* d = nullptr;
    HIP_TRY(hipHostGetDevicePointer(&d, h, 0));
    pl->h_status = static_cast<volatile unsigned*>(h);
    pl->d_status = static_cast<unsigned*>(d);
    return 0;
}

int ensure_team_words(hssfsst_plan* pl, hipStream_t st)
{
    if (pl->d_arrive.get()) return 0;
    if (int rc = pl->d_arrive.grow(4)) return rc;
    HIP_TRY(hipMemsetAsync(pl->d_arrive.get(), 0, 4 * sizeof(unsigned), st));
    pl->arrive_total = 0;
    pl->done_total = 0;
    void* h = nullptr;
    HIP_TRY(hipHostMalloc(&h, 4 * sizeof(unsigned), hipHostMallocMapped));
    for (int i = 0; i < 4; ++i) static_cast<volatile unsigned*>(h)[i] = 0u;
    void* d = nullptr;
    HIP_TRY(hipHostGetDevicePointer(&d, h, 0));
    pl->h_fallback = static_cast<volatile unsigned*>(h);
    pl->d_fallback = static_cast<unsigned*>(d);
    return 0;
}

template <int KLO, int KC, int WPB, int DEPTH, class OT>
constexpr auto team16_kernel()
{
    return &hssfsst::fsst_team16_kernel<KLO, KC, WPB, DEPTH, OT>;
}
template <class OT>
constexpr const char* out_type_suffix() { return sizeof(OT) == 4 ? "" : std::is_same<OT, _Float16>::value ? ", f16" : ", bf16"; }

template <int KLO, int KC, int WPB, int DEPTH, class OT = float>
int launch_team16(hssfsst_plan* pl, ExecCtx& cx, const hssfsst::Core128Params& cp, int64_t batch, int ngroups, void* hout = nullptr)
{
    using namespace hssfsst;
    hipStream_t st = cx.st;
    if constexpr (sizeof(OT) == 2) {
        if (hout == nullptr || (reinterpret_cast<uintptr_t>(hout) & 7) != 0) return 0;
    }
    const int G = ngroups;
    if (G < 1 || G > kFusedMaxGroups) return 0;
    constexpr int PSLOTS = t16_pslots<KLO, KC>();
    constexpr int MS = t16_slots<KLO, KC>();
    size_t lds = (kCanonLdsTabFloats + t16_ctl_floats(PSLOTS, MS) + static_cast<size_t>(WPB) * CanonCfg<KLO, KC>::wave_floats()) * sizeof(float);
    if (lds > static_cast<size_t>(kMaxLdsBytes)) return 0;
    if (lds < 84 * 1024) lds = 84 * 1024;
    auto kern = team16_kernel<KLO, KC, WPB, DEPTH, OT>();
    static std::atomic<unsigned long long> lds_ok{0};
    if (int rc = allow_full_lds(kern, pl->device, lds_ok)) return rc;
    if (int rc = resident_blocks(pl, pl->team16_cus, kern, 64 * WPB, lds, true)) return rc;
    if (pl->team16_cus < 1) return 0;
    int T = 1;
    while ((WPB / 2) * T < G) T *= 2;
    if (T > pl->team16_cus || T > 64) return 0;
    int cpc = 1, cpc_shift = 0;
    while (cpc * T < G) { cpc *= 2; ++cpc_shift; }
    if (cpc > WPB || cpc > kT16MaxCpc || G / T < 1) return 0;
    if (cpc < 4 && T > 1) return 0;
    int nteams = pl->team16_cus / T;
    if (batch < nteams) nteams = static_cast<int>(batch);
    const int grid = nteams * T;
    if ((batch + nteams - 1) / nteams > 65535) return 0;
    if (cp.xstride < 1 || cp.xstride > 0x7fffffffLL || batch > 0x7fffffffLL) return 0;
    const int held_pos = WPB * (DEPTH + 3);
    const int lead = (held_pos + G / T - 1) / (G / T) + 1;
    int slots = 8;
    while (slots < 2 * lead + 2) slots *= 2;
    if (slots > MS) return 0;
    if (lead + 1 > PSLOTS) return 0;
    int rc;
    if ((rc = ensure_status(pl)) != 0) return rc;
    const size_t words = static_cast<size_t>(nteams) * slots * kT16SlotWords;
    if (words > pl->d_mail.cap) {
        if ((rc = pl->d_mail.grow(words)) != 0) return rc;
        HIP_TRY(hipMemsetAsync(pl->d_mail.get(), 0, pl->d_mail.cap * sizeof(unsigned long long), st));
        pl->team_seq = 0;
    }
    if (++pl->team_seq > 0xffffu) {
        HIP_TRY(hipMemsetAsync(pl->d_mail.get(), 0, pl->d_mail.cap * sizeof(unsigned long long), st));
        pl->team_seq = 1;
    }
    Team16Params tp{};
    tp.x = cp.x; tp.out = sizeof(OT) == 4 ? cp.out : static_cast<float*>(hout); tp.atab = pl->d_atab16.get(); tp.wtab = cp.wtab; tp.twtab = cp.twtab;
    tp.mail = pl->d_mail.get(); tp.status = pl->d_status; tp.r2scale_s = pl->canon_r2s; tp.inv_c = pl->canon_inv_c;
    tp.n = cp.n; tp.nsig = cp.nsig; tp.col0 = cp.col0; tp.ncols = cp.ncols; tp.xstride = cp.xstride;
    tp.team = T; tp.cpc_shift = cpc_shift; tp.slots = slots; tp.seq = pl->team_seq;
    {
        const double total = static_cast<double>(KC) * static_cast<double>(cp.ncols);
        tp.inv_total = 1.0 / total; tp.inv_total1 = 1.0 / (total - 1.0);
    }
    tp.spin_ticks = 500u * 100u;
    if ((rc = ensure_team_words(pl, st)) != 0) return rc;
    if (++pl->team_launch == 0u) pl->team_launch = 1u;
    tp.abort_word = pl->d_arrive.get() + 1; tp.fallbacks = pl->d_fallback; tp.launch = pl->team_launch;
    const bool force_fallback = debug_switches().team_force_fallback;
    if (force_fallback) {
        HIP_TRY(hipMemcpyAsync(pl->d_arrive.get() + 1, &pl->team_launch, sizeof(unsigned), hipMemcpyHostToDevice, st));
        HIP_TRY(hipMemcpyAsync(pl->d_fallback, &pl->team_launch, sizeof(unsigned), hipMemcpyHostToDevice, st));
    }
    tp.arrive = pl->d_arrive.get(); tp.arrive_base = pl->arrive_total;
    pl->arrive_total += static_cast<unsigned>(grid);
    if (cx.want_done_word && !force_fallback) {
        tp.done = pl->d_arrive.get() + 2; tp.done_base = pl->done_total; tp.host_done = pl->d_fallback + 2;
        pl->done_total += static_cast<unsigned>(grid);
        cx.flagged_launch = pl->team_launch;
    }
    name_kernel(cx.kernel, WPB, grid, "fsst_team16_kernel<%d, %d, %d, %d%s> teams of %d", KLO, KC, WPB, DEPTH, out_type_suffix<OT>(), T);
    hipLaunchKernelGGL(kern, dim3(static_cast<unsigned>(grid)), dim3(64 * WPB), lds, st, tp);
    HIP_TRY(hipGetLastError());
    cx.team_launch = pl->team_launch;
    return 1;
}

constexpr int kCanonBands[][2] = {{4, 22}, {2, 24}};
constexpr int kCanonKlo = kCanonBands[0][0], kCanonK = kCanonBands[0][1];

int canon_band(const hssfsst_plan* pl)
{
    if (debug_switches().no_canon || !pl->d_atab16.get() || pl->nwin != 128) return -1;
    if (!(pl->mode == HSSFSST_MODE_STACK || pl->mode == HSSFSST_MODE_STACK_UNNORM)) return -1;
    for (int i = 0; i < static_cast<int>(sizeof(kCanonBands) / sizeof(kCanonBands[0])); ++i)
        if (pl->klo == kCanonBands[i][0] && pl->K == kCanonBands[i][1]) return i;
    return -1;
}
bool plan_is_canon(const hssfsst_plan* pl) { return canon_band(pl) >= 0; }
template <class F>
int canon_dispatch(const hssfsst_plan* pl, F&& f)
{
    switch (canon_band(pl)) {
    case 0: return f(std::integral_constant<int, kCanonBands[0][0]>{}, std::integral_constant<int, kCanonBands[0][1]>{});
    case 1: return f(std::integral_constant<int, kCanonBands[1][0]>{}, std::integral_constant<int, kCanonBands[1][1]>{});
    default: return fail(HSSFSST_EINVAL, "canon_dispatch: not a canonical-class plan");
    }
}

hssfsst::CanonParams canon_params(const hssfsst_plan* pl, const ExecCtx& cx, const hssfsst::Core128Params& cp)
{
    hssfsst::CanonParams q{};
    q.x = cp.x; q.out = cp.out; q.partials = cp.partials; q.atab = pl->d_atab16.get(); q.wtab = cp.wtab; q.twtab = cp.twtab;
    q.r2scale_s = pl->canon_r2s; q.inv_c = pl->canon_inv_c;
    q.n = cp.n; q.mode = cp.mode; q.nsig = cp.nsig; q.col0 = cp.col0; q.ncols = cp.ncols; q.xstride = cp.xstride; q.reg = cp.reg;
    q.status = cp.status;
    q.gate = cx.gate; q.gate_val = cx.gate_val;
    return q;
}

template <int KLO, int KC, bool RAGGED = false>
int launch_canon_band(hssfsst_plan* pl, ExecCtx& cx, const hssfsst::Core128Params& cp, int64_t nchunks)
{
    constexpr int WPB = 16;
    const size_t lds = (hssfsst::kCanonLdsTabFloats + hssfsst::kCanonCtlFloats + static_cast<size_t>(WPB) * hssfsst::CanonCfg<KLO, KC>::wave_floats()) * sizeof(float);
    static_assert((hssfsst::kCanonLdsTabFloats + hssfsst::kCanonCtlFloats + 16 * hssfsst::CanonCfg<KLO, KC>::wave_floats()) * sizeof(float) <= 160 * 1024, "16 wave regions must fit");
    auto kern = hssfsst::fsst_canon_kernel<KLO, KC, false, RAGGED>;
    static std::atomic<unsigned long long> lds_ok{0};
    if (int rc = allow_full_lds(kern, pl->device, lds_ok)) return rc;
    int& slots = RAGGED ? pl->ragged_slots : pl->canon_slots;
    if (int rc = resident_blocks(pl, slots, kern, 64 * WPB, lds, false)) return rc;
    int64_t blocks = nchunks < slots ? nchunks : slots;
    if (cx.gate != nullptr && blocks > 64) blocks = 64;
    if (cx.gate == nullptr) name_kernel(cx.kernel, WPB, blocks, "fsst_canon_kernel<%d, %d, false%s>", KLO, KC, RAGGED ? ", ragged" : "");
    hssfsst::CanonParams q = canon_params(pl, cx, cp);
    if constexpr (RAGGED) { q.rsig = cp.rsig; q.rchunk = cp.rchunk; q.rnchunks = cp.rnchunks; }
    hipLaunchKernelGGL(kern, dim3(static_cast<unsigned>(blocks)), dim3(64 * WPB), lds, cx.st, q);
    HIP_TRY(hipGetLastError());
    return 0;
}
int launch_canon(hssfsst_plan* pl, ExecCtx& cx, const hssfsst::Core128Params& cp, int64_t nchunks)
{
    return canon_dispatch(pl, [&](auto KL, auto KN) { return launch_canon_band<decltype(KL)::value, decltype(KN)::value>(pl, cx, cp, nchunks); });
}

template <int KLO, int KC>
int launch_canon_fused_band(hssfsst_plan* pl, ExecCtx& cx, hssfsst::Core128Params cp, int64_t batch, int ngroups)
{
    const bool gated = cx.gate != nullptr;
    constexpr int WPB = 16, GPC = hssfsst::kCanonTileFrames / 16;
    if (ngroups > hssfsst::kFusedMaxGroups || (ngroups + GPC - 1) / GPC < hssfsst::kFusedMinChunks) return 0;
    constexpr size_t lds = (hssfsst::kCanonLdsTabFloats + hssfsst::kCanonCtlFusedFloats + static_cast<size_t>(WPB) * hssfsst::CanonCfg<KLO, KC>::wave_floats()) * sizeof(float);
    if constexpr (lds > static_cast<size_t>(kMaxLdsBytes)) return 0;
    else {
    auto kern = hssfsst::fsst_canon_kernel<KLO, KC, true>;
    static std::atomic<unsigned long long> lds_ok{0};
    if (int rc = allow_full_lds(kern, pl->device, lds_ok)) return rc;
    if (int rc = resident_blocks(pl, pl->fused_slots, kern, 64 * WPB, lds, true)) return rc;
    if (pl->fused_slots < 1) return 0;
    int64_t grid = pl->fused_slots;
    const int64_t rounds = (batch + grid - 1) / grid;
    if (gated) grid = batch < 64 ? batch : 64;
    else if (batch < grid || rounds * grid * 100 > batch * 112) return 0;
    if (int rcs = ensure_status(pl)) return rcs;
    cp.status = pl->d_status;
    if (!gated) name_kernel(cx.kernel, WPB, grid, "fsst_canon_kernel<%d, %d, true>", KLO, KC);
    hipLaunchKernelGGL(kern, dim3(static_cast<unsigned>(grid)), dim3(64 * WPB), lds, cx.st, canon_params(pl, cx, cp));
    HIP_TRY(hipGetLastError());
    return 1;
    }
}
int launch_canon_fused(hssfsst_plan* pl, ExecCtx& cx, const hssfsst::Core128Params& cp, int64_t batch, int ngroups)
{
    return canon_dispatch(pl, [&](auto KL, auto KN) { return launch_canon_fused_band<decltype(KL)::value, decltype(KN)::value>(pl, cx, cp, batch, ngroups); });
}

constexpr int kTeamGiveUps = 4, kTeamPause = 256;
void note_team_outcome(hssfsst_plan* p, bool gave_up)
{
    if (!gave_up) { p->giveups_in_a_row = 0; return; }
    if (++p->giveups_in_a_row >= kTeamGiveUps) { p->giveups_in_a_row = 0; p->team_pause = kTeamPause; }
}

int plan_next_event(hssfsst_plan* p, hipEvent_t* out_ev)
{
    if (p->ev.size() <= p->ev_used) {
        hipEvent_t e2 = nullptr;
        HIP_TRY(hipEventCreate(&e2));
        p->ev.push_back(e2);
    }
    *out_ev = p->ev[p->ev_used++];
    return 0;
}

void timing_begin(hssfsst_plan* p, ExecCtx& cx)
{
    cx.timing = p->timing_every > 0 && (p->timing_seq++ % static_cast<unsigned>(p->timing_every)) == 0u;
}
int timing_event(hssfsst_plan* p, const ExecCtx& cx)
{
    if (!cx.timing) return 0;
    hipEvent_t evt = nullptr;
    if (int rc = plan_next_event(p, &evt)) return rc;
    HIP_TRY(hipEventRecord(evt, cx.st));
    return 0;
}
int timing_core_done(hssfsst_plan* p, const ExecCtx& cx)
{
    return cx.timing_closed ? 0 : timing_event(p, cx);
}
int timing_end(hssfsst_plan* p, const ExecCtx& cx, bool one_kernel)
{
    if (!cx.timing) return 0;
    if (!one_kernel)
        if (int rc = timing_event(p, cx)) return rc;
    p->ev_chunks.push_back(one_kernel ? -1 : 1);
    return 0;
}

template <class F>
void half_dispatch(const hssfsst_plan* p, void* out, F&& f)
{
    if (p->out_dtype == HSSFSST_DTYPE_F16) f(static_cast<_Float16*>(out));
    else f(static_cast<__bf16*>(out));
}

template <bool RAGGED>
int launch_core128_plain(hssfsst_plan* pl, ExecCtx& cx, const hssfsst::Core128Params& cp, int64_t nchunks, bool fast, bool canon)
{
    const int rq = pl->rq, nt = pl->nt;
    const size_t fixed = (hssfsst::core128_atab_floats(rq, nt) + hssfsst::kCtlFloats) * sizeof(float);
    const size_t per_wave = static_cast<size_t>(hssfsst::wave_lds_floats(kFpw128, pl->klo, pl->K, rq, nt)) * sizeof(float);
    const size_t room = 160 * 1024;
    if (nt == 16 && rq == 8) {
        if (fast && canon) return launch_core128_wpb<16, 8, true, 16, 3, false, RAGGED>(pl, cx, cp, nchunks);
        if (fast) return launch_core128_wpb<16, 8, true, 16, -1, false, RAGGED>(pl, cx, cp, nchunks);
        if (fixed + 16 * per_wave <= room) return launch_core128_wpb<16, 8, false, 16, -1, false, RAGGED>(pl, cx, cp, nchunks);
        if (fixed + 8 * per_wave <= room) return launch_core128_wpb<16, 8, false, 8, -1, false, RAGGED>(pl, cx, cp, nchunks);
        if (fixed + 4 * per_wave <= room) return launch_core128_wpb<16, 8, false, 4, -1, false, RAGGED>(pl, cx, cp, nchunks);
    } else if (nt == 16 && rq == 16) {
        if (fast && fixed + 8 * per_wave <= room) return launch_core128_wpb<16, 16, true, 8, -1, false, RAGGED>(pl, cx, cp, nchunks);
        if (!fast && canon && fixed + 8 * per_wave <= room) return launch_core128_wpb<16, 16, false, 8, 3, false, RAGGED>(pl, cx, cp, nchunks);
        if (!fast && fixed + 8 * per_wave <= room) return launch_core128_wpb<16, 16, false, 8, -1, false, RAGGED>(pl, cx, cp, nchunks);
        if (!fast && fixed + 4 * per_wave <= room) return launch_core128_wpb<16, 16, false, 4, -1, false, RAGGED>(pl, cx, cp, nchunks);
        if (fast && fixed + 4 * per_wave <= room) return launch_core128_wpb<16, 16, true, 4, -1, false, RAGGED>(pl, cx, cp, nchunks);
    } else {
        if (!debug_switches().no_pair) {
            if (fast && core128_lds_bytes(pl, 16, 32, 8, true) <= room) return launch_core128_wpb<32, 16, true, 8, -1, true, RAGGED>(pl, cx, cp, nchunks);
            if (!fast && core128_lds_bytes(pl, 16, 32, 8, true) <= room) return launch_core128_wpb<32, 16, false, 8, -1, true, RAGGED>(pl, cx, cp, nchunks);
            if (!fast && core128_lds_bytes(pl, 16, 32, 6, true) <= room) return launch_core128_wpb<32, 16, false, 6, -1, true, RAGGED>(pl, cx, cp, nchunks);
            if (!fast && core128_lds_bytes(pl, 16, 32, 4, true) <= room) return launch_core128_wpb<32, 16, false, 4, -1, true, RAGGED>(pl, cx, cp, nchunks);
        }
        if (fast && fixed + 8 * per_wave <= room) return launch_core128_wpb<32, 16, true, 8, -1, false, RAGGED>(pl, cx, cp, nchunks);
        if (!fast && fixed + 8 * per_wave <= room) return launch_core128_wpb<32, 16, false, 8, -1, false, RAGGED>(pl, cx, cp, nchunks);
        if (!fast && fixed + 6 * per_wave <= room) return launch_core128_wpb<32, 16, false, 6, -1, false, RAGGED>(pl, cx, cp, nchunks);
        if (fast && fixed + 4 * per_wave <= room) return launch_core128_wpb<32, 16, true, 4, -1, false, RAGGED>(pl, cx, cp, nchunks);
        if (!fast && fixed + 4 * per_wave <= room) return launch_core128_wpb<32, 16, false, 4, -1, false, RAGGED>(pl, cx, cp, nchunks);
        if (!fast && fixed + 3 * per_wave <= room) return launch_core128_wpb<32, 16, false, 3, -1, false, RAGGED>(pl, cx, cp, nchunks);
        if (!fast && fixed + 2 * per_wave <= room) return launch_core128_wpb<32, 16, false, 2, -1, false, RAGGED>(pl, cx, cp, nchunks);
        if (fast && fixed + 2 * per_wave <= room) return launch_core128_wpb<32, 16, true, 2, -1, false, RAGGED>(pl, cx, cp, nchunks);
    }
    return fail(HSSFSST_EUNSUPPORTED, "LDS request %zu B per wave exceeds the 160 KiB budget", per_wave);
}

enum class Team { No, Paused, Yes };
Team team_wanted(const hssfsst_plan* pl, int zpref, int col0, int ncols, bool team_only)
{
    if (!plan_is_canon(pl) || (col0 & 15) != 0 || debug_switches().no_team || zpref == HSSFSST_ZPATH_ONE_CU || zpref == HSSFSST_ZPATH_TWO_LAUNCH)
        return Team::No;
    if (pl->team_pause > 0 && !team_only) return Team::Paused;
    return (ncols + 15) / 16 <= hssfsst::kFusedMaxGroups ? Team::Yes : Team::No;
}

int launch_core128(hssfsst_plan* pl, ExecCtx& cx, const float* dx, long long xstride, float* dout, float* partials, int n, int col0,
                   int ncols, int64_t batch, bool try_fused, void* hout = nullptr)
{
    const bool half = hout != nullptr;
    hssfsst::Core128Params cp{};
    cp.xstride = xstride;
    cp.x = dx; cp.out = dout; cp.partials = partials; cp.atab = pl->d_atab.get();
    cp.wtab = pl->d_wtab.get(); cp.twtab = pl->d_wtab.get() + 2 * pl->nwin; cp.r2scale = pl->r2scale;
    cp.n = n; cp.klo = pl->klo; cp.K = pl->K; cp.mode = pl->mode; cp.nsig = static_cast<int>(batch);
    cp.col0 = col0; cp.ncols = ncols;
    cp.reg = hssfsst::core128_regions((ncols + 15) / 16, batch);
    const int64_t nchunks = batch * hssfsst::core128_chunks_per_signal(cp.reg);
    const bool fast = (pl->mode == HSSFSST_MODE_STACK || pl->mode == HSSFSST_MODE_STACK_UNNORM) &&
                      (pl->K & 1) == 0 && pl->K <= 24;
    const int rq = pl->rq, nt = pl->nt;
    const size_t fixed = (hssfsst::core128_atab_floats(rq, nt) + hssfsst::kCtlFloats) * sizeof(float);
    const size_t per_wave = static_cast<size_t>(hssfsst::wave_lds_floats(kFpw128, pl->klo, pl->K, rq, nt)) * sizeof(float);
    const size_t room = 160 * 1024;
    const bool canon = hssfsst::own_s0(pl->klo, rq) == 0 && hssfsst::own_s1(pl->klo, pl->K, rq) == 3;
    const bool canon16 = fast && nt == 16 && rq == 8 && plan_is_canon(pl) && (col0 & 15) == 0;
    if (try_fused && fast && nt == 16 && rq == 8 && pl->mode == HSSFSST_MODE_STACK) {
        const int ngroups = (ncols + 15) / 16;
        const bool team_only = debug_switches().team_only || cx.zpref == HSSFSST_ZPATH_TEAM;
        int rc = 0;
        const Team team = team_wanted(pl, cx.zpref, col0, ncols, team_only);
        if (team == Team::Paused) --pl->team_pause;
        if (team == Team::Yes) {
            rc = canon_dispatch(pl, [&](auto KL, auto KN) {
                constexpr int kl = decltype(KL)::value, kn = decltype(KN)::value;
                if (pl->out_dtype == HSSFSST_DTYPE_F16) return launch_team16<kl, kn, 16, 2, _Float16>(pl, cx, cp, batch, ngroups, hout);
                if (pl->out_dtype == HSSFSST_DTYPE_BF16) return launch_team16<kl, kn, 16, 2, __bf16>(pl, cx, cp, batch, ngroups, hout);
                return launch_team16<kl, kn, 16, 2>(pl, cx, cp, batch, ngroups);
            });
            if (rc == 1) {
                cx.zpath = 2;
                if (int rce = timing_event(pl, cx)) return rce;
                cx.timing_closed = cx.timing;
                if (cx.host_waits) {
                    cx.fused = true;
                    return 0;
                }
                cx.gate = pl->d_arrive.get() + 1; cx.gate_val = cx.team_launch;
                const int rc1 = half ? 0 : launch_canon_fused(pl, cx, cp, batch, ngroups);
                if (rc1 < 0) return rc1;
                if (rc1 == 1) { cx.fused = true; return 0; }
                return launch_canon(pl, cx, cp, nchunks);
            }
            if (rc < 0) return rc;
        }
        if (!team_only && !half) {
            rc = canon16 ? launch_canon_fused(pl, cx, cp, batch, ngroups)
                 : canon ? launch_fused128<3>(pl, cx, cp, batch, ngroups) : launch_fused128<-1>(pl, cx, cp, batch, ngroups);
        }
        if (rc < 0) return rc;
        if (rc == 1) { cx.fused = true; cx.zpath = 1; return 0; }
    }
    if (try_fused && !half && !fast && rq == 8 && nt == 16 && pl->mode == HSSFSST_MODE_STACK && cx.zpref != HSSFSST_ZPATH_TEAM &&
        fixed + 16 * per_wave <= room) {
        const int rc = launch_fused_general<16, 8, 16, -1>(pl, cx, cp, batch, (ncols + 15) / 16);
        if (rc < 0) return rc;
        if (rc == 1) { cx.fused = true; cx.zpath = 1; return 0; }
    }
    if (try_fused && !half && !fast && rq == 16 && pl->mode == HSSFSST_MODE_STACK && cx.zpref != HSSFSST_ZPATH_TEAM) {
        const int ngroups = (ncols + 15) / 16;
        int rc = 0;
        if (nt == 16 && fixed + 8 * per_wave <= room)
            rc = canon ? launch_fused_general<16, 16, 8, 3>(pl, cx, cp, batch, ngroups) : launch_fused_general<16, 16, 8, -1>(pl, cx, cp, batch, ngroups);
        if (rc < 0) return rc;
        if (rc == 1) { cx.fused = true; cx.zpath = 1; return 0; }
    }
    if (canon16) return launch_canon(pl, cx, cp, nchunks);
    return launch_core128_plain<false>(pl, cx, cp, nchunks, fast, canon);
}

}

extern "C" {

int hssfsst_version(void) { return HSSFSST_VERSION; }
const char* hssfsst_last_error(void) { return g_err; }

int hssfsst_device_count(void)
{
    int n = 0;
    if (hipGetDeviceCount(&n) != hipSuccess) { (void)hipGetLastError(); return 0; }
    return n;
}

int hssfsst_dtwin(const double* window, int nwin, double fs, double* dwindow)
{
    if (!window || !dwindow || nwin < 1 || !(fs > 0.0)) return fail(HSSFSST_EINVAL, "hssfsst_dtwin: bad argument");
    const int rc = spline_knot_slopes(window, nwin, dwindow);
    if (rc != 0) return fail(rc, "hssfsst_dtwin: singular spline system");
    const double scale = fs / (2.0 * M_PI);
    for (int i = 0; i < nwin; ++i) dwindow[i] *= scale;
    return 0;
}

int hssfsst_band(int nwin, double fs, double f_lo, double f_hi, int* klo, int* K)
{
    if (nwin < 1 || !(fs > 0.0) || !klo || !K) return fail(HSSFSST_EINVAL, "hssfsst_band: bad argument");
    band_rows(nwin, fs, f_lo, f_hi, klo, K);
    return 0;
}

double hssfsst_update_mean(double m, double x, int64_t k) { return m + (x - m) / static_cast<double>(k); }

double hssfsst_update_variance(double x, double m, double var, int64_t k)
{
    const double delta = x - m;
    return var + delta * (x - (m + delta / static_cast<double>(k)));
}

int hssfsst_plan_create(hssfsst_plan** out, int device, int nwin, const double* window, double fs,
                        int has_band, double f_lo, double f_hi, int mode)
{
    return hssfsst_plan_create_ex(out, device, nwin, window, fs, has_band, f_lo, f_hi, mode, HSSFSST_DTYPE_F32);
}

int hssfsst_plan_create_ex(hssfsst_plan** out, int device, int nwin, const double* window, double fs,
                           int has_band, double f_lo, double f_hi, int mode, int out_dtype)
{
    if (!out) return fail(HSSFSST_EINVAL, "plan_create: out is NULL");
    *out = nullptr;
    if (!window || nwin < 1 || !(fs > 0.0) || mode < 0 || mode > HSSFSST_MODE_STACK_UNNORM)
        return fail(HSSFSST_EINVAL, "plan_create: bad argument (nwin=%d fs=%g mode=%d)", nwin, fs, mode);
    if (out_dtype != HSSFSST_DTYPE_F32 && out_dtype != HSSFSST_DTYPE_F16 && out_dtype != HSSFSST_DTYPE_BF16)
        return fail(HSSFSST_EINVAL, "plan_create: output dtype %d is not HSSFSST_DTYPE_F32 / F16 / BF16", out_dtype);
    if (out_dtype != HSSFSST_DTYPE_F32 && mode != HSSFSST_MODE_STACK)
        return fail(HSSFSST_EINVAL, "plan_create: half-precision output (dtype %d) is for HSSFSST_MODE_STACK only, not mode %d", out_dtype, mode);
    if (nwin > 65535) return fail(HSSFSST_EUNSUPPORTED, "plan_create: window length %d exceeds 65535", nwin);
    const bool force_dft = debug_switches().force_dft;
    const bool radix_len = nwin == 32 || nwin == 64 || nwin == 128 || nwin == 256 || nwin == 512;
    if (int rc = check_device("plan_create", device)) return rc;
    DEVICE_SCOPE(device);

    std::unique_ptr<hssfsst_plan> p(new (std::nothrow) hssfsst_plan());
    if (!p) return fail(HSSFSST_ENOMEM, "plan_create: host allocation failed");
    p->device = device; p->nwin = nwin; p->R = nwin / 32; p->nf = nwin / 2 + 1; p->mode = mode; p->fs = fs;
    p->out_dtype = out_dtype; p->out_es = out_dtype == HSSFSST_DTYPE_F32 ? sizeof(float) : 2;
    if (has_band) band_rows(nwin, fs, f_lo, f_hi, &p->klo, &p->K);
    else { p->klo = 0; p->K = p->nf; }

    std::vector<double> dwb(nwin);
    int rc = spline_knot_slopes(window, nwin, dwb.data());
    if (rc != 0) return fail(rc, "plan_create: singular spline system");
    for (int i = 0; i < nwin; ++i) dwb[i] *= static_cast<double>(nwin) / (2.0 * M_PI);

    p->dft = (!radix_len || force_dft) ? 1 : 0;
    const int R = p->dft ? 2 : p->R;
    const int ncls = R / 2 + 1;
    std::vector<float> tab(static_cast<size_t>(ncls) * 32 * 4 * R, 0.0f);
    if (!p->dft)
    for (int r = 0; r < ncls; ++r) {
        const bool packed = (r == 0) || (2 * r == R);
        for (int n = 0; n < 32; ++n) {
            float* row = tab.data() + (static_cast<size_t>(r) * 32 + n) * 4 * R;
            for (int q = 0; q < R; ++q) {
                const double ang = -2.0 * M_PI * (static_cast<double>(r) * q / R + static_cast<double>(r) * n / nwin);
                const double c = std::cos(ang), s = std::sin(ang);
                const double wv = window[n + 32 * q], dv = dwb[n + 32 * q];
                if (packed) {
                    row[q] = static_cast<float>(0.5 * (wv * c - dv * s));
                    row[R + q] = static_cast<float>(0.5 * (wv * s + dv * c));
                } else {
                    row[q] = static_cast<float>(wv * c);
                    row[R + q] = static_cast<float>(wv * s);
                    row[2 * R + q] = static_cast<float>(dv * c);
                    row[3 * R + q] = static_cast<float>(dv * s);
                }
            }
        }
    }
    if ((rc = p->d_ctab.upload(tab.data(), tab.size())) != 0) return rc;
    {
        std::vector<double> wt(static_cast<size_t>(4) * nwin);
        double cmax2 = 0.0;
        for (int i = 0; i < nwin; ++i) cmax2 = std::fmax(cmax2, 0.25 * (window[i] * window[i] + dwb[i] * dwb[i]));
        p->r2scale = static_cast<float>(4.0 * nwin * cmax2);
        for (int i = 0; i < nwin; ++i) {
            wt[2 * i] = window[i]; wt[2 * i + 1] = dwb[i];
            const double ang = 2.0 * M_PI * static_cast<double>(i) / static_cast<double>(nwin);
            wt[2 * nwin + 2 * i] = std::cos(ang); wt[2 * nwin + 2 * i + 1] = std::sin(ang);
        }
        if (nwin == 128 || nwin == 256 || nwin == 512) {
            const int nt = (nwin == 512) ? 32 : 16, rq = nwin / nt, npass = rq / 8, kst = rq / 4;
            wt.resize(static_cast<size_t>(4) * nwin + static_cast<size_t>(hssfsst::fold64_doubles(rq, nt)));
            for (int pz = 0; pz < npass; ++pz)
                for (int n = 0; n < nt; ++n)
                    for (int ks = 0; ks < kst; ++ks)
                        for (int l = 0; l < 64; ++l) {
                            const int i = l & 15, q = (l >> 4) + 4 * ks;
                            const int gg = i & 3, sub = i >> 2, m = 4 * pz + gg;
                            const int r = (sub < 2) ? m : (m ? rq - m : rq / 2);
                            const double ang = -2.0 * M_PI * (static_cast<double>(r) * q / rq + static_cast<double>(r) * n / nwin);
                            const double c = std::cos(ang), sn = std::sin(ang);
                            const double sg = (r & 1) ? -0.5 : 0.5;
                            const double wv = window[n + nt * q], dv = dwb[n + nt * q];
                            wt[static_cast<size_t>(4) * nwin + (((pz * nt + n) * kst) + ks) * 64 + l] =
// ... 386 lines not shown
        const size_t pw = static_cast<size_t>(hssfsst::dft_wave_lds_floats(dp.nk4, p->K, cand)) * sizeof(float);
        int w = static_cast<int>(static_cast<size_t>(kMaxLdsBytes) / pw);
        if (w > 8) w = 8;
        if (w < 1) continue;
        int per_cu = static_cast<int>(static_cast<size_t>(kMaxLdsBytes) / (pw * w)) * w;
        if (per_cu > 32) per_cu = 32;
        if (per_cu >= 16) { G = cand; best_waves = per_cu; break; }
        if (per_cu > best_waves) { G = cand; best_waves = per_cu; }
    }
    if (ncols <= 16) G = 1;
    const size_t per_wave = static_cast<size_t>(hssfsst::dft_wave_lds_floats(dp.nk4, p->K, G)) * sizeof(float);
    int waves = static_cast<int>(static_cast<size_t>(kMaxLdsBytes) / per_wave);
    if (waves > 8) waves = 8;
    if (waves < 1) return fail(HSSFSST_EUNSUPPORTED, "exec: LDS request %zu B per wave exceeds 160 KiB", per_wave);
    const int ntiles = (ncols + 16 * G - 1) / (16 * G);
    dp.nitems = static_cast<long long>(batch) * ntiles;
    long long blocks = (dp.nitems + waves - 1) / waves;
    if (blocks > 256 * 64) blocks = 256 * 64;
    auto launch = [&](auto kern) -> int {
        static std::atomic<unsigned long long> lds_ok{0};
        if (int r2 = allow_full_lds(kern, p->device, lds_ok)) return r2;
        name_kernel(cx.kernel, waves, blocks, "fsst_dft_kernel<%d>", G);
        hipLaunchKernelGGL(kern, dim3(static_cast<unsigned>(blocks)), dim3(64 * waves), per_wave * waves, cx.st, dp);
        return (hipGetLastError() == hipSuccess) ? 0 : fail(HSSFSST_EHIP, "exec: fsst_dft_kernel launch failed");
    };
    return (G == 4) ? launch(hssfsst::fsst_dft_kernel<4>) : (G == 2) ? launch(hssfsst::fsst_dft_kernel<2>) : launch(hssfsst::fsst_dft_kernel<1>);
}

static int finish_pinned_exec(hssfsst_plan* p, const ExecCtx& cx, bool* redo)
{
    bool seen = false;
    const unsigned fl = cx.flagged_launch;
    if (fl != 0u && p->h_fallback) {
        const auto t0 = std::chrono::steady_clock::now();
        for (unsigned it = 0;; ++it) {
            if (p->h_fallback[2] == fl) { seen = true; break; }
            if (p->h_fallback[0] == fl) break;
            if ((it & 255u) == 255u && std::chrono::steady_clock::now() - t0 > std::chrono::microseconds(2000)) break;
            __builtin_ia32_pause();
        }
        std::atomic_thread_fence(std::memory_order_acquire);
    }
    if (!seen) {
        HIP_TRY(hipStreamSynchronize(cx.st));
        if (fl != 0u) {
            HIP_TRY(hipMemsetAsync(p->d_arrive.get() + 2, 0, sizeof(unsigned), cx.st));
            p->done_total = 0;
        }
    }
    if (cx.host_waits && cx.team_launch != 0u) {
        const bool gave = p->h_fallback && p->h_fallback[0] == cx.team_launch;
        note_team_outcome(p, gave);
        if (gave) { *redo = true; return 0; }
    }
    if (seen) {
        if (p->h_status && *p->h_status != 0u) {
            const unsigned code = *p->h_status;
            *p->h_status = 0u;
            return fail(HSSFSST_EHIP, "fused z-score: a wait inside the kernel gave up (code %u); results of that exec are invalid", code);
        }
    } else if (p->d_status) return hssfsst_plan_check(p);
    return 0;
}

static int exec_impl(hssfsst_plan* p, const float* x, int64_t batch, int n, int64_t x_stride, const long long* d_starts,
                     size_t x_len, int col0, int ncols, int x_on_device, float* out, int out_on_device, void* stream, float* pin_d = nullptr,
                     bool redo = false)
{
    if (!p || !x || !out || batch < 0 || n < 1 || col0 < 0 || ncols < 1 || col0 > n - ncols || x_stride < 1)
        return fail(HSSFSST_EINVAL, "exec: bad argument (batch=%lld n=%d stride=%lld col0=%d ncols=%d)",
                    static_cast<long long>(batch), n, static_cast<long long>(x_stride), col0, ncols);
    if (batch == 0 || p->K == 0) return 0;
    hipStream_t st = static_cast<hipStream_t>(stream);
    DEVICE_SCOPE(p->device);
    int rc;
    if ((rc = take_pending_status(p, "exec")) != 0) return rc;
    ExecCtx cx;
    cx.st = st;
    cx.zpref = redo ? HSSFSST_ZPATH_ONE_CU : p->zpath_pref;
    const int ofps = out_floats_per_sample(p);
    const bool use128 = (p->d_atab.get() != nullptr);
    const int fpp = (use128 || p->dft) ? 16 : kTile;
    const int nblk = (ncols + fpp - 1) / fpp;
    const long long nblocks = static_cast<long long>(batch) * nblk;
    if (nblocks > 0x7fffffffLL) return fail(HSSFSST_EINVAL, "exec: batch*tiles = %lld exceeds the grid limit; split the batch", nblocks);
    if (static_cast<long long>(n) * 2 * p->nf >= 0x7fffffffLL) return fail(HSSFSST_EINVAL, "exec: signal too long (n = %d)", n);
    const size_t nx = d_starts ? x_len : static_cast<size_t>(batch > 0 ? batch - 1 : 0) * static_cast<size_t>(x_stride) + n;
    const size_t no = static_cast<size_t>(batch) * ncols * ofps;
    const size_t es = p->out_es, no_f = (no * es + sizeof(float) - 1) / sizeof(float);
    const bool half = es != sizeof(float);

    const float* dx = x;
    float* dout = out;
    const bool tiny_in = !x_on_device && nx <= (static_cast<size_t>(1) << 16);
    const bool tiny_out = tiny_in && !out_on_device && no_f <= (static_cast<size_t>(1) << 21) &&
                          (p->mode != HSSFSST_MODE_STACK || team_wanted(p, cx.zpref, col0, ncols, cx.zpref == HSSFSST_ZPATH_TEAM) == Team::Yes);
    auto pin = [&](PinnedBuf<float>& b, size_t need) -> int {
        if (b.h && b.cap < need) HIP_TRY(hipStreamSynchronize(st));
        return b.grow(need, sizeof(float));
    };
    if (tiny_in) {
        if ((rc = pin(p->xpin, nx)) != 0) return rc;
        std::memcpy(p->xpin.h, x, nx * sizeof(float));
        dx = p->xpin.d;
    } else if (!x_on_device) {
        if ((rc = stage_input(p, x, nx, &dx, st)) != 0) return rc;
    }
    if (d_starts) {
        const size_t nd = static_cast<size_t>(batch) * n;
        if ((rc = p->d_frames.grow(nd)) != 0) return rc;
        const long long quads = (static_cast<long long>(n) + 3) / 4;
        long long blocks = (static_cast<long long>(batch) * quads + 255) / 256;
        if (blocks > 65536) blocks = 65536;
        hipLaunchKernelGGL(hssfsst::fsst_gather_frames_kernel, dim3(static_cast<unsigned>(blocks)), dim3(256), 0, st,
                           dx, d_starts, p->d_frames.get(), static_cast<long long>(batch), n);
        HIP_TRY(hipGetLastError());
        dx = p->d_frames.get();
        x_stride = n;
    }
    if (pin_d && !tiny_out) return 1;
    if (tiny_out) {
        if (pin_d) dout = pin_d;
        else {
            if ((rc = pin(p->opin, no_f)) != 0) return rc;
            dout = p->opin.d;
        }
        cx.host_waits = cx.zpref != HSSFSST_ZPATH_ONE_CU && !d_starts;
    }
    float* kout = nullptr;
    if ((rc = exec_buffers(p, no, !tiny_out && !out_on_device, static_cast<size_t>(nblocks), batch, &dout, &kout)) != 0) return rc;

    timing_begin(p, cx);
    cx.want_done_word = cx.host_waits && !cx.timing;
    hssfsst::CoreParams cp;
    cp.x = dx; cp.out = kout; cp.partials = p->d_partials.get(); cp.ctab = p->d_ctab.get();
    cp.n = n; cp.klo = p->klo; cp.K = p->K; cp.mode = p->mode; cp.nblk = nblk; cp.col0 = col0; cp.ncols = ncols; cp.xstride = x_stride;
    cp.wtab = p->d_wtab.get(); cp.twtab = p->d_wtab.get() + 2 * p->nwin; cp.r2scale = p->r2scale;
    if ((rc = timing_event(p, cx)) != 0) return rc;
    const bool no_fused = debug_switches().no_fused;
    if (p->dft) {
        rc = launch_dft(p, cx, dx, kout, batch, n, x_stride, col0, ncols);
    } else if (use128) {
        rc = launch_core128(p, cx, dx, x_stride, kout, cp.partials, n, col0, ncols, batch, !no_fused && cx.zpref != HSSFSST_ZPATH_TWO_LAUNCH,
                            half ? dout : nullptr);
    } else switch (p->R) {
        case 1: rc = launch_core<1>(p, cx, cp, nblocks); break;
        case 2: rc = launch_core<2>(p, cx, cp, nblocks); break;
        case 4: rc = launch_core<4>(p, cx, cp, nblocks); break;
        case 8: rc = launch_core<8>(p, cx, cp, nblocks); break;
        case 16: rc = launch_core<16>(p, cx, cp, nblocks); break;
        default: rc = fail(HSSFSST_EUNSUPPORTED, "exec: unsupported radix %d", p->R);
    }
    if (rc != 0) return rc;
    if ((rc = timing_core_done(p, cx)) != 0) return rc;
    if (p->mode == HSSFSST_MODE_STACK && !cx.fused) {
        float4* stats = reinterpret_cast<float4*>(p->d_stats.get());
        int64_t zgrid = 4096;
        int slices = 1;
        if (batch < 1024) {
            slices = static_cast<int>(1024 / batch);
            if (slices > 32) slices = 32;
        }
        if (zgrid > batch * slices) zgrid = batch * slices;
        const bool fused = slices == 1 && zgrid == batch && batch >= 512;
        if (!fused)
            hipLaunchKernelGGL(hssfsst::fsst_stats_kernel, dim3(static_cast<unsigned>(batch)), dim3(64), 0, st,
                               cp.partials, stats, nblk, fpp, ncols, p->K, cx.gate, cx.gate_val);
        if (half)
            half_dispatch(p, dout, [&](auto* o) {
                hipLaunchKernelGGL(hssfsst::fsst_normalize_to_kernel<std::remove_pointer_t<decltype(o)>>, dim3(static_cast<unsigned>(zgrid)), dim3(256), 0, st,
                                   kout, o, stats, fused ? cp.partials : nullptr, nblk, fpp, ncols, p->K, static_cast<int>(batch), slices,
                                   cx.gate, cx.gate_val);
            });
        else
            hipLaunchKernelGGL(hssfsst::fsst_normalize_kernel, dim3(static_cast<unsigned>(zgrid)), dim3(256), 0, st,
                               kout, stats, fused ? cp.partials : nullptr, nblk, fpp, ncols, p->K, static_cast<int>(batch), slices,
                               cx.gate, cx.gate_val);
        HIP_TRY(hipGetLastError());
    }
    exec_report(p, cx);
    if ((rc = timing_end(p, cx, p->last_fused != 0)) != 0) return rc;
    if (tiny_out) {
        bool gave_up = false;
        if ((rc = finish_pinned_exec(p, cx, &gave_up)) != 0) return rc;
        if (gave_up)
            return exec_impl(p, x, batch, n, x_stride, d_starts, x_len, col0, ncols, x_on_device, out, out_on_device, stream, nullptr, true);
        if (!pin_d) std::memcpy(out, p->opin.h, no * es);
    } else return exec_finish(p, out, dout, no * es, x_on_device, out_on_device, st);
    return 0;
}

int hssfsst_exec_frames(hssfsst_plan* p, const float* x, int64_t batch, int n, int64_t x_stride, int col0, int ncols,
                        int x_on_device, float* out, int out_on_device, void* stream)
{
    return exec_impl(p, x, batch, n, x_stride, nullptr, 0, col0, ncols, x_on_device, out, out_on_device, stream);
}

int hssfsst_exec_pinned(hssfsst_plan* p, const float* x, int n, float** out)
{
    if (!p || !x || !out || n < 1) return fail(HSSFSST_EINVAL, "exec_pinned: bad argument");
    *out = nullptr;
    if (p->K == 0) return 1;
    DEVICE_SCOPE(p->device);
    const size_t no = static_cast<size_t>(n) * out_floats_per_sample(p);
    hssfsst_plan::PoolBuf* b = nullptr;
    {
        std::lock_guard<std::mutex> lock(p->pin_mu);
        for (auto& c : p->pin_pool) if (!c.used && c.buf.cap >= no) { b = &c; break; }
        if (!b) {
            for (auto& c : p->pin_pool) if (!c.used) { b = &c; break; }
            if (!b) return 1;
            if (int rc = b->buf.grow(no, p->out_es)) return rc;
        }
        b->used = true;
    }
    const int rc = exec_impl(p, x, 1, n, static_cast<int64_t>(n), nullptr, 0, 0, n, 0, b->buf.h, 0, nullptr, b->buf.d);
    if (rc != 0) {
        std::lock_guard<std::mutex> lock(p->pin_mu);
        b->used = false;
        return rc;
    }
    *out = b->buf.h;
    return 0;
}

int hssfsst_pinned_release(hssfsst_plan* p, float* buf)
{
    if (!p || !buf) return fail(HSSFSST_EINVAL, "pinned_release: bad argument");
    std::lock_guard<std::mutex> lock(p->pin_mu);
    for (auto& c : p->pin_pool) if (c.buf.h == buf) { c.used = false; return 0; }
    return fail(HSSFSST_EINVAL, "pinned_release: not a buffer of this plan's pool");
}

int hssfsst_exec_list(hssfsst_plan* p, const float* x, int64_t x_len, const int64_t* starts, int starts_on_device,
                      int64_t batch, int n, int x_on_device, float* out, int out_on_device, void* stream)
{
    if (!p || !x || !starts || !out || batch < 0 || n < 1 || x_len < n)
        return fail(HSSFSST_EINVAL, "exec_list: bad argument (batch=%lld n=%d x_len=%lld)", static_cast<long long>(batch), n,
                    static_cast<long long>(x_len));
    if (batch == 0 || p->K == 0) return 0;
    static_assert(sizeof(long long) == sizeof(int64_t), "frame starts are 64-bit");
    const long long* d_starts = reinterpret_cast<const long long*>(starts);
    if (!starts_on_device) {
        for (int64_t b = 0; b < batch; ++b)
            if (starts[b] < 0 || starts[b] > x_len - n)
                return fail(HSSFSST_EINVAL, "exec_list: frame %lld starts at %lld, outside [0, %lld]", static_cast<long long>(b),
                            static_cast<long long>(starts[b]), static_cast<long long>(x_len - n));
        DEVICE_SCOPE(p->device);
        int rc;
        if ((rc = p->d_starts.grow(static_cast<size_t>(batch))) != 0) return rc;
        HIP_TRY(hipMemcpyAsync(p->d_starts.get(), starts, static_cast<size_t>(batch) * sizeof(long long), hipMemcpyHostToDevice,
                               static_cast<hipStream_t>(stream)));
        d_starts = p->d_starts.get();
    }
    return exec_impl(p, x, batch, n, 1, d_starts, static_cast<size_t>(x_len), 0, n, x_on_device, out, out_on_device, stream);
}

int hssfsst_exec_ragged(hssfsst_plan* p, const float* x, int64_t x_len, const int64_t* starts, const int64_t* lens, int64_t batch,
                        int x_on_device, float* out, int out_on_device, void* stream)
{
    if (batch < 0 || batch > 0x7fffffffLL) return fail(HSSFSST_EINVAL, "exec_ragged: batch = %lld", static_cast<long long>(batch));
    if (batch > 0 && (!x || !starts || !lens || !out))
        return fail(HSSFSST_EINVAL, "exec_ragged: NULL %s", !x ? "x" : !starts ? "starts" : !lens ? "lens" : "out");
    for (int64_t i = 0; i < batch; ++i) {
        if (lens[i] < 1) return fail(HSSFSST_EINVAL, "exec_ragged: signal %lld has length %lld", static_cast<long long>(i), static_cast<long long>(lens[i]));
        if (starts[i] < 0 || x_len < lens[i] || starts[i] > x_len - lens[i])
            return fail(HSSFSST_EINVAL, "exec_ragged: signal %lld ([%lld, %lld + %lld)) lies outside x[0, %lld)", static_cast<long long>(i),
                        static_cast<long long>(starts[i]), static_cast<long long>(starts[i]), static_cast<long long>(lens[i]),
                        static_cast<long long>(x_len));
    }
    if (!p) return fail(HSSFSST_EINVAL, "exec_ragged: plan is NULL");
    for (int64_t i = 0; i < batch; ++i)
        if (lens[i] >= (0x7fffffffLL + 2 * p->nf - 1) / (2 * p->nf))
            return fail(HSSFSST_EINVAL, "exec_ragged: signal %lld too long (n = %lld)", static_cast<long long>(i), static_cast<long long>(lens[i]));
    if (batch == 0 || p->K == 0) return 0;
    const int ofps = out_floats_per_sample(p);
    if (p->d_atab.get() == nullptr) {
        long long off = 0;
        for (int64_t i = 0; i < batch; ++i) {
            const int n = static_cast<int>(lens[i]);
            float* o = reinterpret_cast<float*>(reinterpret_cast<char*>(out) + static_cast<size_t>(off) * ofps * p->out_es);
            if (int rc = exec_impl(p, x + starts[i], 1, n, n, nullptr, 0, 0, n, x_on_device, o, out_on_device, stream)) return rc;
            off += n;
        }
        return 0;
    }
    hipStream_t st = static_cast<hipStream_t>(stream);
    DEVICE_SCOPE(p->device);
    int rc;
    if ((rc = take_pending_status(p, "exec")) != 0) return rc;
    long long xlo = starts[0], xhi = starts[0] + lens[0];
    for (int64_t i = 1; i < batch; ++i) {
        xlo = std::min<long long>(xlo, starts[i]);
        xhi = std::max<long long>(xhi, starts[i] + lens[i]);
    }
    if (x_on_device) xlo = 0;
    long long cols = 0, groups = 0;
    for (int64_t i = 0; i < batch; ++i) { cols += lens[i]; groups += (lens[i] + 15) / 16; }
    const size_t no = static_cast<size_t>(cols) * ofps;
    const bool half = p->out_es != sizeof(float);

    const size_t sig_bytes = static_cast<size_t>(batch) * sizeof(hssfsst::RaggedSignal);
    bool same = p->d_rtab.get() != nullptr && p->rkey.size() == static_cast<size_t>(2 * batch);
    for (int64_t i = 0; same && i < batch; ++i) same = p->rkey[2 * i] == lens[i] && p->rkey[2 * i + 1] == starts[i] - xlo;
    if (!same) {
        if (p->rtab_ev) HIP_TRY(hipEventSynchronize(p->rtab_ev));
        std::vector<int> ng(static_cast<size_t>(batch));
        for (int64_t i = 0; i < batch; ++i) ng[i] = static_cast<int>((lens[i] + 15) / 16);
        std::vector<int2> chunks;
        hssfsst::core128_ragged_chunks(ng.data(), batch, chunks);
        if (chunks.size() >= 0x7fffffffull) return fail(HSSFSST_EINVAL, "exec_ragged: %zu chunks exceed the launch limit; split the list", chunks.size());
        p->rtab_unit = (sig_bytes + 15) & ~size_t(15);
        p->rtab_chunk = (p->rtab_unit + static_cast<size_t>(batch + 1) * sizeof(int) + 15) & ~size_t(15);
        p->rtab_bytes = p->rtab_chunk + chunks.size() * sizeof(int2);
        if ((rc = p->h_rtab.grow(p->rtab_bytes, 1)) != 0) return rc;
        std::memset(p->h_rtab.h, 0, p->rtab_chunk);
        auto* rs = reinterpret_cast<hssfsst::RaggedSignal*>(p->h_rtab.h);
        int* unit0 = reinterpret_cast<int*>(p->h_rtab.h + p->rtab_unit);
        long long o = 0, g = 0, u = 0;
        p->rkey.resize(static_cast<size_t>(2 * batch));
        for (int64_t i = 0; i < batch; ++i) {
            rs[i].xoff = starts[i] - xlo; rs[i].ooff = o * ofps; rs[i].poff = g * hssfsst::kPartFloats;
            rs[i].n = static_cast<int>(lens[i]); rs[i].pad = 0;
            unit0[i] = static_cast<int>(u);
            u += (lens[i] * 2 * p->K + hssfsst::kRaggedUnitFloats - 1) / hssfsst::kRaggedUnitFloats;
            o += lens[i]; g += ng[i];
            p->rkey[2 * i] = lens[i]; p->rkey[2 * i + 1] = starts[i] - xlo;
        }
        unit0[batch] = static_cast<int>(u);
        std::memcpy(p->h_rtab.h + p->rtab_chunk, chunks.data(), chunks.size() * sizeof(int2));
        p->rtab_nchunks = static_cast<long long>(chunks.size());
        p->rtab_nunits = u;
        if ((rc = p->d_rtab.grow(p->rtab_bytes)) != 0) { p->rkey.clear(); return rc; }
        if (!p->rtab_ev) HIP_TRY(hipEventCreateWithFlags(&p->rtab_ev, hipEventDisableTiming));
        HIP_TRY(hipMemcpyAsync(p->d_rtab.get(), p->h_rtab.h, p->rtab_bytes, hipMemcpyHostToDevice, st));
        HIP_TRY(hipEventRecord(p->rtab_ev, st));
    }
    const auto* d_rsig = reinterpret_cast<const hssfsst::RaggedSignal*>(p->d_rtab.get());
    const int* d_unit0 = reinterpret_cast<const int*>(p->d_rtab.get() + p->rtab_unit);
    const int2* d_chunks = reinterpret_cast<const int2*>(p->d_rtab.get() + p->rtab_chunk);

    const float* dx = x;
    float* dout = out;
    float* kout = nullptr;
    if (!x_on_device && (rc = stage_input(p, x + xlo, static_cast<size_t>(xhi - xlo), &dx, st)) != 0) return rc;
    if ((rc = exec_buffers(p, no, !out_on_device, static_cast<size_t>(groups), batch, &dout, &kout)) != 0) return rc;

    ExecCtx cx;
    cx.st = st;
    timing_begin(p, cx);
    if ((rc = timing_event(p, cx)) != 0) return rc;
    hssfsst::Core128Params cp{};
    cp.x = dx; cp.out = kout; cp.partials = p->d_partials.get(); cp.atab = p->d_atab.get();
    cp.wtab = p->d_wtab.get(); cp.twtab = p->d_wtab.get() + 2 * p->nwin; cp.r2scale = p->r2scale;
    cp.n = 1; cp.klo = p->klo; cp.K = p->K; cp.mode = p->mode; cp.nsig = static_cast<int>(std::min<int64_t>(batch, 0x7fffffff));
    cp.col0 = 0; cp.ncols = 1; cp.xstride = 0;
    cp.rsig = d_rsig; cp.rchunk = d_chunks; cp.rnchunks = static_cast<int>(p->rtab_nchunks);
    const bool fast = (p->mode == HSSFSST_MODE_STACK || p->mode == HSSFSST_MODE_STACK_UNNORM) && (p->K & 1) == 0 && p->K <= 24;
    const bool canon = hssfsst::own_s0(p->klo, p->rq) == 0 && hssfsst::own_s1(p->klo, p->K, p->rq) == 3;
    if (fast && p->nt == 16 && p->rq == 8 && plan_is_canon(p))
        rc = canon_dispatch(p, [&](auto KL, auto KN) { return launch_canon_band<decltype(KL)::value, decltype(KN)::value, true>(p, cx, cp, p->rtab_nchunks); });
    else
        rc = launch_core128_plain<true>(p, cx, cp, p->rtab_nchunks, fast, canon);
    if (rc != 0) return rc;
    if ((rc = timing_core_done(p, cx)) != 0) return rc;
    if (p->mode == HSSFSST_MODE_STACK) {
        float4* stats = reinterpret_cast<float4*>(p->d_stats.get());
        hipLaunchKernelGGL(hssfsst::fsst_ragged_stats_kernel, dim3(static_cast<unsigned>(batch)), dim3(64), 0, st, p->d_partials.get(), d_rsig, stats, p->K);
        const long long zgrid = std::min<long long>(p->rtab_nunits, 65536);
        if (half)
            half_dispatch(p, dout, [&](auto* o) {
                hipLaunchKernelGGL(hssfsst::fsst_ragged_normalize_to_kernel<std::remove_pointer_t<decltype(o)>>, dim3(static_cast<unsigned>(zgrid)), dim3(256), 0, st,
                                   kout, o, d_rsig, d_unit0, stats, static_cast<int>(batch), p->K);
            });
        else
            hipLaunchKernelGGL(hssfsst::fsst_ragged_normalize_kernel, dim3(static_cast<unsigned>(zgrid)), dim3(256), 0, st, dout, d_rsig, d_unit0,
                               stats, static_cast<int>(batch), p->K);
        HIP_TRY(hipGetLastError());
    }
    exec_report(p, cx);
    if ((rc = timing_end(p, cx, false)) != 0) return rc;
    return exec_finish(p, out, dout, no * p->out_es, x_on_device, out_on_device, st);
}

int hssfsst_moments_merge(hssfsst_plan* p, const float* feats, int64_t batch, int n, double* state, void* stream)
{
    if (!p || !feats || !state || batch < 0 || n < 1) return fail(HSSFSST_EINVAL, "moments_merge: bad argument");
    if (batch == 0 || p->K == 0) return 0;
    if (batch > 0x7fffffffLL || static_cast<long long>(n) * 2 * p->K >= 0x7fffffffLL) return fail(HSSFSST_EINVAL, "moments_merge: too large");
    DEVICE_SCOPE(p->device);
    hipLaunchKernelGGL(hssfsst::fsst_moments_merge_kernel, dim3(static_cast<unsigned>(batch)), dim3(hssfsst::kMomThreads), 0,
                       static_cast<hipStream_t>(stream), feats, state, n, p->K);
    HIP_TRY(hipGetLastError());
    return 0;
}

}

struct hssfsst_resample_plan {
    int device = -1;
    int64_t n = 0, num = 0;
    int M1 = 1, M2 = 1, Mt = 1;
    DevBuf<double2> d_tab;
    const double2 *c1 = nullptr, *B1 = nullptr, *c2 = nullptr, *B2 = nullptr, *tw = nullptr;
    DevBuf<unsigned char> d_x, d_y;
    DevBuf<long long> d_lab, d_starts;
    DevBuf<double2> d_work;
    bool ragged = false;
    DevBuf<double2> d_tw; int tw_M = 0;
    DevBuf<unsigned char> d_desc;
    std::vector<unsigned char> h_desc;
    hipEvent_t desc_ev = nullptr;
};

namespace {

constexpr int64_t kRsMaxLen = int64_t(1) << 26;
constexpr size_t kRsWorkBytes = size_t(256) << 20;

int pow2_at_least(int64_t v)
{
    int m = 1;
    while (m < v) m <<= 1;
    return m;
}

void bluestein_tables(int64_t N, int M, double sgn, hssfsst::resample_detail::cd* c, hssfsst::resample_detail::cd* B)
{
    using hssfsst::resample_detail::cd;
    std::vector<cd> w(static_cast<size_t>(N)), b(static_cast<size_t>(M), cd(0.0, 0.0));
    for (int64_t m = 0; m < N; ++m) {
        const int64_t r = (m * m) % (2 * N);
        const double ang = sgn * M_PI * static_cast<double>(r) / static_cast<double>(N);
        w[static_cast<size_t>(m)] = cd(std::cos(ang), std::sin(ang));
        c[m] = std::conj(w[static_cast<size_t>(m)]);
    }
    b[0] = w[0];
    for (int64_t m = 1; m < N; ++m) b[static_cast<size_t>(m)] = b[static_cast<size_t>(M - m)] = w[static_cast<size_t>(m)];
    hssfsst::resample_detail::fft_pow2(b, false);
    int lg = 0;
    while ((1 << lg) < M) ++lg;
    for (int j = 0; j < M; ++j) {
        int r = 0;
        for (int k = 0; k < lg; ++k) r |= ((j >> k) & 1) << (lg - 1 - k);
        B[j] = b[static_cast<size_t>(r)] / static_cast<double>(M);
    }
}

int rs_launch_check(const char* what)
{
    const hipError_t e = hipGetLastError();
    if (e != hipSuccess) return fail(HSSFSST_EHIP, "resample_exec: launch of %s failed: %s", what, hipGetErrorString(e));
    return 0;
}

unsigned rs_grid(long long total) { return static_cast<unsigned>((total + hssfsst::kRsThreads - 1) / hssfsst::kRsThreads); }

int rs_check_dtypes(const char* what, int x_dtype, const void* y, int y_dtype)
{
    if ((x_dtype != HSSFSST_DTYPE_F32 && x_dtype != HSSFSST_DTYPE_F64) || (y && y_dtype != HSSFSST_DTYPE_F32 && y_dtype != HSSFSST_DTYPE_F64))
        return fail(HSSFSST_EINVAL, "%s: unknown dtype (x %d, y %d)", what, x_dtype, y_dtype);
    return 0;
}

template <class Args>
int rs_stage(hssfsst_resample_plan* p, Args& a, const void* x, size_t x_bytes, int x_on_device, void* y, size_t ysz, int64_t* labels,
             size_t nout, int out_on_device, hipStream_t st)
{
    int rc;
    a.x = x;
    if (!x_on_device) {
        if ((rc = p->d_x.grow(x_bytes)) != 0) return rc;
        HIP_TRY(hipMemcpyAsync(p->d_x.get(), x, x_bytes, hipMemcpyHostToDevice, st));
        a.x = p->d_x.get();
    }
    a.y = y;
    a.labels = reinterpret_cast<long long*>(labels);
    if (!out_on_device) {
        if (y) {
            if ((rc = p->d_y.grow(nout * ysz)) != 0) return rc;
            a.y = p->d_y.get();
        }
        if (labels) {
            if ((rc = p->d_lab.grow(nout)) != 0) return rc;
            a.labels = p->d_lab.get();
        }
    }
    return 0;
}

template <class Args>
int rs_finish(const Args& a, void* y, size_t ysz, int64_t* labels, size_t nout, int x_on_device, int out_on_device, hipStream_t st)
{
    if (!out_on_device) {
        if (y) HIP_TRY(hipMemcpyAsync(y, a.y, nout * ysz, hipMemcpyDeviceToHost, st));
        if (labels) HIP_TRY(hipMemcpyAsync(labels, a.labels, nout * sizeof(long long), hipMemcpyDeviceToHost, st));
    }
    if (!out_on_device || !x_on_device) HIP_TRY(hipStreamSynchronize(st));
    return 0;
}

int rs_dif(hipStream_t st, double2* w, long long Mw, long long cnt, int M, const double2* tw, int twM)
{
    const int S = M < hssfsst::kRsBlock ? M : hssfsst::kRsBlock;
    const long long nb = cnt * (M / 2);
    for (int len = M; len > S; len >>= 1) {
        hipLaunchKernelGGL(hssfsst::resample_dif_pass_kernel, dim3(rs_grid(nb)), dim3(hssfsst::kRsThreads), 0, st, w, Mw, M, len, tw, twM, nb);
        if (int r = rs_launch_check("resample_dif_pass_kernel")) return r;
    }
    return 0;
}
int rs_dit(hipStream_t st, double2* w, long long Mw, long long cnt, int M, const double2* tw, int twM)
{
    const int S = M < hssfsst::kRsBlock ? M : hssfsst::kRsBlock;
    const long long nb = cnt * (M / 2);
    for (int len = 2 * S; len <= M; len <<= 1) {
        hipLaunchKernelGGL(hssfsst::resample_dit_pass_kernel, dim3(rs_grid(nb)), dim3(hssfsst::kRsThreads), 0, st, w, Mw, M, len, tw, twM, nb);
        if (int r = rs_launch_check("resample_dit_pass_kernel")) return r;
// ... 547 lines not shown
```

Before: 6.045 million.

## Replace gated fallback kernel launches with in-kernel rescue blocks for team16

The team16 persistent kernel previously needed follow-up gated fallback launches (canon fused or canon kernel, plus gated stats/normalize) that checked a device word and exited early when the team path succeeded. These are replaced by extra 'rescue' workgroups appended to the team16 grid. The rescue blocks wait until all team blocks report completion through a ring of counters, and recompute the signals themselves if an abort was signalled. This removes several launches from the common path, but adds spinning rescue blocks that occupy CUs and make the team kernel's completion logic more complex.

```diff
diff --git a/heart_sounds_segmentation_amd/csrc/fsst_canon128.hpp b/heart_sounds_segmentation_amd/csrc/fsst_canon128.hpp
--- a/heart_sounds_segmentation_amd/csrc/fsst_canon128.hpp
+++ b/heart_sounds_segmentation_amd/csrc/fsst_canon128.hpp
@@ -455,8 +455,6 @@
     long long xstride;
     Core128Regions reg;
     unsigned* status;
-    const unsigned* gate;
-    unsigned gate_val;
     const RaggedSignal* rsig;
     const int2* rchunk;
     int rnchunks;
@@ -482,7 +480,6 @@
     constexpr int ATAB = kCanonLdsTabFloats;
     constexpr int CTL = FUSED ? kCanonCtlFusedFloats : kCanonCtlFloats;
     extern __shared__ __attribute__((aligned(16))) float smem[];
-    if (p.gate != nullptr && *p.gate != p.gate_val) return;
     int n = p.n;
     const int lane = threadIdx.x & 63;
     const int wv = __builtin_amdgcn_readfirstlane(threadIdx.x >> 6);
diff --git a/heart_sounds_segmentation_amd/csrc/fsst_half.hpp b/heart_sounds_segmentation_amd/csrc/fsst_half.hpp
--- a/heart_sounds_segmentation_amd/csrc/fsst_half.hpp
+++ b/heart_sounds_segmentation_amd/csrc/fsst_half.hpp
@@ -16,11 +16,9 @@
 
 template <class OT>
 __global__ __launch_bounds__(256) void fsst_normalize_to_kernel(const float* in, OT* out, const float4* stats, const float* partials,
-                                                                int nblk, int fpp, int n, int K, int nsignals, int slices,
-                                                                const unsigned* gate = nullptr, unsigned gate_val = 0u)
+                                                                int nblk, int fpp, int n, int K, int nsignals, int slices)
 {
     static_assert(sizeof(OT) == 2, "2-byte output elements");
-    if (gate != nullptr && *gate != gate_val) return;
     __shared__ float4 st_sh;
     const int tid = threadIdx.x;
     const int C = 2 * K;
diff --git a/heart_sounds_segmentation_amd/csrc/fsst_kernels.hpp b/heart_sounds_segmentation_amd/csrc/fsst_kernels.hpp
--- a/heart_sounds_segmentation_amd/csrc/fsst_kernels.hpp
+++ b/heart_sounds_segmentation_amd/csrc/fsst_kernels.hpp
@@ -422,9 +422,8 @@
 }
 
 __global__ __launch_bounds__(64) void fsst_stats_kernel(const float* partials, float4* stats, int nparts, int fpp,
-                                                        int n, int K, const unsigned* gate = nullptr, unsigned gate_val = 0u)
-{
-    if (gate != nullptr && *gate != gate_val) return;
+                                                        int n, int K)
+{
     const long long b = blockIdx.x;
     const float4 st = signal_stats(partials + b * nparts * kPartFloats, nparts, fpp, n, K, threadIdx.x & 63);
     if (threadIdx.x == 0) stats[b] = st;
@@ -556,10 +555,8 @@
 }
 
 __global__ __launch_bounds__(256) void fsst_normalize_kernel(float* out, const float4* stats, const float* partials,
-                                                             int nblk, int fpp, int n, int K, int nsignals, int slices,
-                                                             const unsigned* gate = nullptr, unsigned gate_val = 0u)
-{
-    if (gate != nullptr && *gate != gate_val) return;
+                                                             int nblk, int fpp, int n, int K, int nsignals, int slices)
+{
     __shared__ float4 st_sh;
     const int tid = threadIdx.x;
     const int C = 2 * K;
diff --git a/heart_sounds_segmentation_amd/csrc/fsst_team16.hpp b/heart_sounds_segmentation_amd/csrc/fsst_team16.hpp
--- a/heart_sounds_segmentation_amd/csrc/fsst_team16.hpp
+++ b/heart_sounds_segmentation_amd/csrc/fsst_team16.hpp
@@ -52,6 +52,9 @@
     unsigned done_base;
     unsigned* host_done;
     double inv_total, inv_total1;
+    int rescue;
+    unsigned* out_count;
+    unsigned* next_count;
 };
 
 
@@ -84,6 +87,143 @@
     using w2 = unsigned __attribute__((ext_vector_type(2)));
     const w2 w = {__builtin_bit_cast(unsigned, __builtin_convertvector(lo, o2)), __builtin_bit_cast(unsigned, __builtin_convertvector(hi, o2))};
     __builtin_nontemporal_store(w, reinterpret_cast<w2*>(dst));
+}
+
+using t16_kparams = const __attribute__((address_space(4))) Team16Params;
+constexpr unsigned kT16RescueWaits = 4096u;
+
+template <int KLO, int KC, int WPB, class OT>
+__device__ __forceinline__ void team16_rescue(float* smem, int virt)
+{
+    constexpr int OB = static_cast<int>(sizeof(OT)), K = KC;
+    using C = CanonCfg<KLO, KC>;
+    t16_kparams* kp = (t16_kparams*)__builtin_amdgcn_kernarg_segment_ptr();
+    asm volatile("" : "+s"(kp), "+s"(virt));
+    int tid = threadIdx.x;
+    asm volatile("" : "+v"(tid));
+    const int lane = tid & 63, wv = __builtin_amdgcn_readfirstlane(tid >> 6);
+    constexpr int ATAB = kCanonLdsTabFloats, MS = t16_slots<KLO, KC>(), PSLOTS = t16_pslots<KLO, KC>();
+    float* atab = smem;
+    unsigned* verdict = reinterpret_cast<unsigned*>(smem + ATAB) + 5;
+    const unsigned* cls_lds = reinterpret_cast<const unsigned*>(smem + ATAB + 16);
+    const unsigned* ppk_lds = reinterpret_cast<const unsigned*>(smem + ATAB + 80);
+    float4* fin = reinterpret_cast<float4*>(smem + ATAB + 272 + 2 * MS);
+    float* part_lds = smem + ATAB + t16_ctl_base(MS);
+    float* wbase = smem + ATAB + t16_ctl_floats(PSLOTS, MS) + wv * C::wave_floats();
+    u2* xrec = reinterpret_cast<u2*>(wbase);
+    f2* own_base = reinterpret_cast<f2*>(wbase + 2 * kCanonRecs);
+    int* flag = reinterpret_cast<int*>(own_base + 16 * C::LD);
+    int* tq = flag + kCanonFlagWords;
+    const int team_grid = static_cast<int>(gridDim.x) - kp->rescue, r = virt - team_grid;
+    constexpr unsigned kHealthy = 1u, kGivenUp = 2u;
+    if (threadIdx.x == 0) {
+        const unsigned t0 = static_cast<unsigned>(wall_clock64());
+        const unsigned launch = kp->launch, bound = kp->spin_ticks * kT16RescueWaits;
+        unsigned v = kHealthy;
+        for (;;) {
+            const unsigned ab = __hip_atomic_load(kp->abort_word, __ATOMIC_RELAXED, __HIP_MEMORY_SCOPE_AGENT);
+            const unsigned out = __hip_atomic_load(kp->out_count, __ATOMIC_RELAXED, __HIP_MEMORY_SCOPE_AGENT);
+            if (ab == launch) { v = kGivenUp; break; }
+            if (out == static_cast<unsigned>(team_grid)) break;
+            if (static_cast<unsigned>(wall_clock64()) - t0 > bound) {
+                __hip_atomic_store((gu32*)(kp->status), 2u, __ATOMIC_RELAXED, __HIP_MEMORY_SCOPE_SYSTEM);
+                break;
+            }
+            __builtin_amdgcn_s_sleep(32);
+        }
+        __hip_atomic_store(verdict, v, __ATOMIC_RELAXED, __HIP_MEMORY_SCOPE_WORKGROUP);
+    }
+    __syncthreads();
+    if (__hip_atomic_load(verdict, __ATOMIC_RELAXED, __HIP_MEMORY_SCOPE_WORKGROUP) != kGivenUp) return;
+
+    auto KP = [&]() -> t16_kparams* { t16_kparams* q = kp; asm volatile("" : "+s"(q)); return q; };
+    f2 tiny = {1.0e-37f, 0.0f};
+    asm volatile("" : "+s"(tiny));
+    for (int sig = r; sig < KP()->nsig; sig += KP()->rescue) {
+        for (int pass = 0; pass < 2; ++pass) {
+            int ps = pass;
+            asm volatile("" : "+s"(ps));
+            for (int g = wv; g < ((KP()->ncols + 15) >> 4); g += WPB) {
+                int lane_o = lane;
+                asm volatile("" : "+v"(lane_o));
+                const int n = KP()->n;
+                const int cgg = g + (KP()->col0 >> 4), t0 = (cgg & ~3) * 16, tg = cgg * 16;
+                auto xsig = [&]() -> const float* {
+                    return KP()->x + static_cast<unsigned long long>(static_cast<unsigned>(sig)) * static_cast<unsigned>(KP()->xstride);
+                };
+                float sreg[3];
+                canon_fetch(xsig(), n, t0, lane_o, sreg);
+                const CanonTile tile = canon_land<true>(sreg, xrec, KP()->r2scale_s, KP()->inv_c, lane_o, t0, n);
+                canon_group<KLO, KC, 2, true>(xrec + (cgg & 3) * 16, atab, own_base, flag, tq, KP()->wtab, KP()->twtab, tile, tiny, lane_o,
+                                              xsig, n, tg, KP()->atab + kCanonAtabFloats);
+                const int ncols = KP()->ncols, nvalid = min(16, ncols - g * 16);
+                if (ps == 0) {
+                    f2 piv;
+                    const float w = canon_stats<KLO, KC>(own_base, nvalid, tile.inv, lane_o, piv);
+                    float* pe = part_lds + g * kT16PartFloats;
+                    if ((lane_o & 15) == 0) pe[lane_o >> 4] = w;
+                    if (lane_o == 0) { pe[4] = piv.x; pe[5] = piv.y; }
+                } else {
+                    const unsigned cofs = cls_lds[lane_o];
+                    const unsigned pk0 = ppk_lds[lane_o], pk1 = ppk_lds[64 + lane_o], pk2 = ppk_lds[128 + lane_o];
+                    unsigned obase = static_cast<unsigned>(reinterpret_cast<size_t>((lds_float*)reinterpret_cast<const float*>(own_base)));
+                    asm volatile("" : "+s"(obase));
+                    auto cell = [&](unsigned off) -> f2 {
+                        const lds_float* q = (const lds_float*)static_cast<size_t>(obase + off);
+                        return f2{q[0], q[2]};
+                    };
+                    const f2 lo0 = cell(pk0 & 0xffffu), hi0 = cell(pk0 >> 16), lo1 = cell(pk1 & 0xffffu), hi1 = cell(pk1 >> 16),
+                             lo2 = cell(pk2 & 0xffffu), hi2 = cell(pk2 >> 16);
+                    const f2 sc = {tile.inv, tile.inv};
+                    held_put<0>(lo0, sc); held_put<1>(hi0, sc); held_put<2>(lo1, sc); held_put<3>(hi1, sc); held_put<4>(lo2, sc); held_put<5>(hi2, sc);
+                    const char* tb = reinterpret_cast<const char*>(fin);
+                    const unsigned sig_bytes = static_cast<unsigned>(ncols) * (2 * K * OB);
+                    char* ob = reinterpret_cast<char*>(KP()->out) + static_cast<unsigned long long>(static_cast<unsigned>(sig)) * sig_bytes +
+                               static_cast<unsigned>(g * (16 * 2 * K * OB));
+                    const unsigned voff = static_cast<unsigned>(lane_o) * (4u * OB);
+                    const int lim = nvalid * (K >> 1);
+                    static_for<3>([&](auto I) {
+                        constexpr int i = decltype(I)::value;
+                        if (lane_o + 64 * i < lim) {
+                            const float4 tt = *reinterpret_cast<const float4*>(tb + ((cofs >> (8 * i)) & 0xffu));
+                            const f2 lo = held_zscore<2 * i>(f2{tt.x, tt.y});
+                            const f2 hi = held_zscore<2 * i + 1>(f2{tt.z, tt.w});
+                            if constexpr (OB == 4) __builtin_nontemporal_store(f4{lo.x, lo.y, hi.x, hi.y}, reinterpret_cast<f4*>(ob + (voff + 1024u * static_cast<unsigned>(i))));
+                            else team16_store4<OT>(ob + (voff + (256u * OB) * static_cast<unsigned>(i)), lo, hi);
+                        }
+                    });
+                }
+                wave_sync();
+            }
+            if (ps == 0) {
+                __syncthreads();
+                if (wv == 0) {
+                    int lane_r = lane;
+                    asm volatile("" : "+v"(lane_r));
+                    const int ncols = KP()->ncols, G = (ncols + 15) >> 4, nblocks = (G + kStatBlock - 1) / kStatBlock;
+                    const int q = lane_r & 3, h = q >> 1;
+                    double acc = 0.0;
+                    for (int blk = lane_r >> 2; blk < nblocks; blk += 16) {
+                        double sbk = 0.0;
+                        const int g1 = min(G, (blk + 1) * kStatBlock);
+                        for (int g = blk * kStatBlock; g < g1; ++g) {
+                            const float* pb = part_lds + g * kT16PartFloats;
+                            const double cnt = static_cast<double>(min(16, ncols - 16 * g)) * static_cast<double>(K);
+                            sbk += piece_moment(q, static_cast<double>(pb[2 * h]), static_cast<double>(pb[2 * h + 1]), static_cast<double>(pb[4 + h]), cnt);
+                        }
+                        acc += sbk;
+                    }
+                    const float4 st = stats_finish_lead(acc, KP()->inv_total, KP()->inv_total1, lane_r);
+                    if (lane == 0) {
+                        fin[0] = make_float4(st.x, st.y, st.x, st.y);
+                        fin[1] = make_float4(st.x, st.y, st.z, st.w);
+                        fin[2] = make_float4(st.z, st.w, st.z, st.w);
+                    }
+                }
+                __syncthreads();
+            }
+        }
+    }
 }
 
 template <int KLO, int KC, int WPB, int DEPTH, class OT = float>
@@ -124,7 +264,10 @@
     if (threadIdx.x < 16 && threadIdx.x != 2) next_q[threadIdx.x] = 0;
     for (int i = threadIdx.x; i < 2 * MS; i += 64 * WPB) ready[i] = 0u;
     if (threadIdx.x < 2 * PSLOTS) pcnt_lds[threadIdx.x] = 0;
-    if (threadIdx.x == 64) next_q[2] = static_cast<int>(arrived);
+    if (threadIdx.x == 64) {
+        next_q[2] = static_cast<int>(arrived);
+        if (arrived == 0u) __hip_atomic_store(p.next_count, 0u, __ATOMIC_RELAXED, __HIP_MEMORY_SCOPE_AGENT);
+    }
     if (wv == 0) {
         unsigned cofs = 0u;
 #pragma unroll
@@ -138,7 +281,7 @@
     }
     __syncthreads();
 
-    using kparams = const __attribute__((address_space(4))) Team16Params;
+    using kparams = t16_kparams;
     kparams* const kp_ = (kparams*)__builtin_amdgcn_kernarg_segment_ptr();
     auto P = [&]() -> kparams* { kparams* q = kp_; asm volatile("" : "+s"(q)); return q; };
 
@@ -160,10 +303,14 @@
 
     const int virt = __builtin_amdgcn_readfirstlane(next_q[2]);
     if (static_cast<unsigned>(virt) >= gridDim.x) { gave_up(); return; }
+    if (__builtin_expect(virt >= static_cast<int>(gridDim.x) - p.rescue, 0)) {
+        team16_rescue<KLO, KC, WPB, OT>(smem, virt);
+        asm volatile("s_endpgm" ::: "memory");
+    }
     const unsigned abort_seen = __hip_atomic_load(P()->abort_word, __ATOMIC_RELAXED, __HIP_MEMORY_SCOPE_AGENT);
     const int T = p.team, cpcs = p.cpc_shift, cpc = 1 << cpcs;
     const int member = virt & (T - 1), team = virt / T;
-    const int nteams = static_cast<int>(gridDim.x) / T;
+    const int nteams = (static_cast<int>(gridDim.x) - p.rescue) / T;
     const int nk = (p.nsig > team) ? (p.nsig - team + nteams - 1) / nteams : 0;
     const int nwork = nk << cpcs;
     const int ncols = p.ncols, cend = p.col0 + p.ncols;
@@ -499,6 +646,12 @@
             if (so == sl) { signal_statistics(ko_hs[sl]); emit_held(S, ko_hs[sl], g_hs[sl]); }
         });
     }
+    if (P()->rescue != 0) {
+        unsigned last = 0u;
+        if (lane == 0) last = __hip_atomic_fetch_add(next_q + 4, 1, __ATOMIC_RELAXED, __HIP_MEMORY_SCOPE_WORKGROUP) == WPB - 1 ? 1u : 0u;
+        if (__builtin_amdgcn_readfirstlane(last) != 0u && lane == 0)
+            __hip_atomic_fetch_add(P()->out_count, 1u, __ATOMIC_RELAXED, __HIP_MEMORY_SCOPE_AGENT);
+    }
     if (P()->host_done != nullptr) {
         __builtin_amdgcn_fence(__ATOMIC_RELEASE, "workgroup");
         unsigned last = 0u;
diff --git a/heart_sounds_segmentation_amd/csrc/hssfsst.hip b/heart_sounds_segmentation_amd/csrc/hssfsst.hip
--- a/heart_sounds_segmentation_amd/csrc/hssfsst.hip
+++ b/heart_sounds_segmentation_amd/csrc/hssfsst.hip
@@ -270,6 +270,7 @@
     DevBuf<unsigned long long> d_mail;
     unsigned team_seq = 0;
     DevBuf<unsigned> d_arrive; unsigned arrive_total = 0;
+    unsigned team_out_slot = 0;
     unsigned done_total = 0;
     unsigned team_launch = 0;
     volatile unsigned* h_fallback = nullptr; unsigned* d_fallback = nullptr;
@@ -337,14 +338,12 @@
     int zpref = HSSFSST_ZPATH_AUTO;
     bool host_waits = false;
     bool want_done_word = false;
-    const unsigned* gate = nullptr; unsigned gate_val = 0;
     unsigned team_launch = 0;
     unsigned flagged_launch = 0;
     bool fused = false;
     int zpath = 0;
     char kernel[sizeof(hssfsst_plan::last_kernel)] = "";
     bool timing = false;
-    bool timing_closed = false;
 };
 
 void name_kernel(char (&name)[sizeof(hssfsst_plan::last_kernel)], int waves, long long grid, const char* fmt, ...)
@@ -360,7 +359,7 @@
 void exec_report(hssfsst_plan* p, const ExecCtx& cx)
 {
     std::memcpy(p->last_kernel, cx.kernel, sizeof(p->last_kernel));
-    p->last_fused = (cx.fused || cx.team_launch != 0u) ? 1 : 0;
+    p->last_fused = cx.fused ? 1 : 0;
     p->last_zpath = cx.zpath;
 }
 
@@ -518,13 +517,15 @@
     return 0;
 }
 
+constexpr unsigned kTeamOutRing = 4;
 int ensure_team_words(hssfsst_plan* pl, hipStream_t st)
 {
     if (pl->d_arrive.get()) return 0;
-    if (int rc = pl->d_arrive.grow(4)) return rc;
-    HIP_TRY(hipMemsetAsync(pl->d_arrive.get(), 0, 4 * sizeof(unsigned), st));
+    if (int rc = pl->d_arrive.grow(4 + kTeamOutRing)) return rc;
+    HIP_TRY(hipMemsetAsync(pl->d_arrive.get(), 0, (4 + kTeamOutRing) * sizeof(unsigned), st));
     pl->arrive_total = 0;
     pl->done_total = 0;
+    pl->team_out_slot = 0;
     void* h = nullptr;
     HIP_TRY(hipHostMalloc(&h, 4 * sizeof(unsigned), hipHostMallocMapped));
     for (int i = 0; i < 4; ++i) static_cast<volatile unsigned*>(h)[i] = 0u;
@@ -572,7 +573,9 @@
     if (cpc < 4 && T > 1) return 0;
     int nteams = pl->team16_cus / T;
     if (batch < nteams) nteams = static_cast<int>(batch);
-    const int grid = nteams * T;
+    const int team_grid = nteams * T;
+    const int rescue = cx.host_waits ? 0 : static_cast<int>(std::min<int64_t>(batch, pl->team16_cus));
+    const int grid = team_grid + rescue;
     if ((batch + nteams - 1) / nteams > 65535) return 0;
     if (cp.xstride < 1 || cp.xstride > 0x7fffffffLL || batch > 0x7fffffffLL) return 0;
     const int held_pos = WPB * (DEPTH + 3);
@@ -613,6 +616,10 @@
     }
     tp.arrive = pl->d_arrive.get(); tp.arrive_base = pl->arrive_total;
     pl->arrive_total += static_cast<unsigned>(grid);
+    tp.rescue = rescue;
+    tp.out_count = pl->d_arrive.get() + 4 + pl->team_out_slot;
+    pl->team_out_slot = (pl->team_out_slot + 1u) % kTeamOutRing;
+    tp.next_count = pl->d_arrive.get() + 4 + pl->team_out_slot;
     if (cx.want_done_word && !force_fallback) {
         tp.done = pl->d_arrive.get() + 2; tp.done_base = pl->done_total; tp.host_done = pl->d_fallback + 2;
         pl->done_total += static_cast<unsigned>(grid);
@@ -654,7 +661,6 @@
     q.r2scale_s = pl->canon_r2s; q.inv_c = pl->canon_inv_c;
     q.n = cp.n; q.mode = cp.mode; q.nsig = cp.nsig; q.col0 = cp.col0; q.ncols = cp.ncols; q.xstride = cp.xstride; q.reg = cp.reg;
     q.status = cp.status;
-    q.gate = cx.gate; q.gate_val = cx.gate_val;
     return q;
 }
 
@@ -670,8 +676,7 @@
     int& slots = RAGGED ? pl->ragged_slots : pl->canon_slots;
     if (int rc = resident_blocks(pl, slots, kern, 64 * WPB, lds, false)) return rc;
     int64_t blocks = nchunks < slots ? nchunks : slots;
-    if (cx.gate != nullptr && blocks > 64) blocks = 64;
-    if (cx.gate == nullptr) name_kernel(cx.kernel, WPB, blocks, "fsst_canon_kernel<%d, %d, false%s>", KLO, KC, RAGGED ? ", ragged" : "");
+    name_kernel(cx.kernel, WPB, blocks, "fsst_canon_kernel<%d, %d, false%s>", KLO, KC, RAGGED ? ", ragged" : "");
     hssfsst::CanonParams q = canon_params(pl, cx, cp);
     if constexpr (RAGGED) { q.rsig = cp.rsig; q.rchunk = cp.rchunk; q.rnchunks = cp.rnchunks; }
     hipLaunchKernelGGL(kern, dim3(static_cast<unsigned>(blocks)), dim3(64 * WPB), lds, cx.st, q);
@@ -686,7 +691,6 @@
 template <int KLO, int KC>
 int launch_canon_fused_band(hssfsst_plan* pl, ExecCtx& cx, hssfsst::Core128Params cp, int64_t batch, int ngroups)
 {
-    const bool gated = cx.gate != nullptr;
     constexpr int WPB = 16, GPC = hssfsst::kCanonTileFrames / 16;
     if (ngroups > hssfsst::kFusedMaxGroups || (ngroups + GPC - 1) / GPC < hssfsst::kFusedMinChunks) return 0;
     constexpr size_t lds = (hssfsst::kCanonLdsTabFloats + hssfsst::kCanonCtlFusedFloats + static_cast<size_t>(WPB) * hssfsst::CanonCfg<KLO, KC>::wave_floats()) * sizeof(float);
@@ -699,11 +703,10 @@
     if (pl->fused_slots < 1) return 0;
     int64_t grid = pl->fused_slots;
     const int64_t rounds = (batch + grid - 1) / grid;
-    if (gated) grid = batch < 64 ? batch : 64;
-    else if (batch < grid || rounds * grid * 100 > batch * 112) return 0;
+    if (batch < grid || rounds * grid * 100 > batch * 112) return 0;
     if (int rcs = ensure_status(pl)) return rcs;
     cp.status = pl->d_status;
-    if (!gated) name_kernel(cx.kernel, WPB, grid, "fsst_canon_kernel<%d, %d, true>", KLO, KC);
+    name_kernel(cx.kernel, WPB, grid, "fsst_canon_kernel<%d, %d, true>", KLO, KC);
     hipLaunchKernelGGL(kern, dim3(static_cast<unsigned>(grid)), dim3(64 * WPB), lds, cx.st, canon_params(pl, cx, cp));
     HIP_TRY(hipGetLastError());
     return 1;
@@ -743,10 +746,6 @@
     if (int rc = plan_next_event(p, &evt)) return rc;
     HIP_TRY(hipEventRecord(evt, cx.st));
     return 0;
-}
-int timing_core_done(hssfsst_plan* p, const ExecCtx& cx)
-{
-    return cx.timing_closed ? 0 : timing_event(p, cx);
 }
 int timing_end(hssfsst_plan* p, const ExecCtx& cx, bool one_kernel)
 {
@@ -846,17 +845,8 @@
             });
             if (rc == 1) {
                 cx.zpath = 2;
-                if (int rce = timing_event(pl, cx)) return rce;
-                cx.timing_closed = cx.timing;
-                if (cx.host_waits) {
-                    cx.fused = true;
-                    return 0;
-                }
-                cx.gate = pl->d_arrive.get() + 1; cx.gate_val = cx.team_launch;
-                const int rc1 = half ? 0 : launch_canon_fused(pl, cx, cp, batch, ngroups);
-                if (rc1 < 0) return rc1;
-                if (rc1 == 1) { cx.fused = true; return 0; }
-                return launch_canon(pl, cx, cp, nchunks);
+                cx.fused = true;
+                return 0;
             }
             if (rc < 0) return rc;
         }
@@ -1549,7 +1539,7 @@
         default: rc = fail(HSSFSST_EUNSUPPORTED, "exec: unsupported radix %d", p->R);
     }
     if (rc != 0) return rc;
-    if ((rc = timing_core_done(p, cx)) != 0) return rc;
+    if ((rc = timing_event(p, cx)) != 0) return rc;
     if (p->mode == HSSFSST_MODE_STACK && !cx.fused) {
         float4* stats = reinterpret_cast<float4*>(p->d_stats.get());
         int64_t zgrid = 4096;
@@ -1562,17 +1552,15 @@
         const bool fused = slices == 1 && zgrid == batch && batch >= 512;
         if (!fused)
             hipLaunchKernelGGL(hssfsst::fsst_stats_kernel, dim3(static_cast<unsigned>(batch)), dim3(64), 0, st,
-                               cp.partials, stats, nblk, fpp, ncols, p->K, cx.gate, cx.gate_val);
+                               cp.partials, stats, nblk, fpp, ncols, p->K);
         if (half)
             half_dispatch(p, dout, [&](auto* o) {
                 hipLaunchKernelGGL(hssfsst::fsst_normalize_to_kernel<std::remove_pointer_t<decltype(o)>>, dim3(static_cast<unsigned>(zgrid)), dim3(256), 0, st,
-                                   kout, o, stats, fused ? cp.partials : nullptr, nblk, fpp, ncols, p->K, static_cast<int>(batch), slices,
-                                   cx.gate, cx.gate_val);
+                                   kout, o, stats, fused ? cp.partials : nullptr, nblk, fpp, ncols, p->K, static_cast<int>(batch), slices);
             });
         else
             hipLaunchKernelGGL(hssfsst::fsst_normalize_kernel, dim3(static_cast<unsigned>(zgrid)), dim3(256), 0, st,
-                               kout, stats, fused ? cp.partials : nullptr, nblk, fpp, ncols, p->K, static_cast<int>(batch), slices,
-                               cx.gate, cx.gate_val);
+                               kout, stats, fused ? cp.partials : nullptr, nblk, fpp, ncols, p->K, static_cast<int>(batch), slices);
         HIP_TRY(hipGetLastError());
     }
     exec_report(p, cx);
@@ -1760,7 +1748,7 @@
     else
         rc = launch_core128_plain<true>(p, cx, cp, p->rtab_nchunks, fast, canon);
     if (rc != 0) return rc;
-    if ((rc = timing_core_done(p, cx)) != 0) return rc;
+    if ((rc = timing_event(p, cx)) != 0) return rc;
     if (p->mode == HSSFSST_MODE_STACK) {
         float4* stats = reinterpret_cast<float4*>(p->d_stats.get());
         hipLaunchKernelGGL(hssfsst::fsst_ragged_stats_kernel, dim3(static_cast<unsigned>(batch)), dim3(64), 0, st, p->d_partials.get(), d_rsig, stats, p->K);
```

After: 5.960 million. 1.4% lower.
